# xmindflow/deformableLKA

Hardware: AMD Instinct MI355X
Metric: 3D D-LKA fwd+bwd volumes/sec (64x128x128, b2) (higher is better)
Workload: dtype f32; 1 GPU; 3D D-LKA Former Synapse 64x128x128 patch: fwd+bwd of its 21 D-LKA attention blocks (6x(32,32^3)+6x(64,16^3)+6x(128,8^3)+3x(256,4^3)) + grad all-reduce + SGD update; batch_per_gpu=2, global_batch=2, parallelism=dp1, block_params=15390693, hipgraph=True, weight_gradients_on_side_stream=True, allreduce_overlap=False, allreduce_split_block=0

## Files before the change

deformablelka_amd/_lib.py:

```python
from __future__ import annotations

import ctypes
import os
from ctypes import POINTER, c_char_p, c_int, c_int32, c_int64, c_size_t, c_void_p

import torch

_HERE = os.path.dirname(os.path.abspath(__file__))
LIB_PATH = os.path.join(_HERE, "_lib", "libdlka_hip.so")

DLKA_F32, DLKA_BF16, DLKA_F64 = 0, 1, 2
DLKA_TILES_MAX_T, DLKA_TILES_K_MAX = 64, 32
DLKA_TILES_IDENTITY, DLKA_TILES_SOFTMAX, DLKA_TILES_SIGMOID = 0, 1, 2
LKA3D_SYNAPSE, LKA3D_ACDC = 0, 1
DLKA_SEG_LOSS_K_MAX = 32
DLKA_SEG_LOSS_NNUNET, DLKA_SEG_LOSS_DICE2D = 0, 1
DLKA_LABEL_F32, DLKA_LABEL_I64 = 0, 1
DLKA_SD_K_MAX = 32
DLKA_SD_U8, DLKA_SD_I16, DLKA_SD_I32, DLKA_SD_I64 = 0, 1, 2, 3
DLKA_CC_K_MAX, DLKA_CC_IDS_MAX = 32, 64
DLKA_CC_SUMMARY = 1 + 2 * DLKA_CC_K_MAX
DLKA_RESAMPLE_SPLINE_PAD = 12
DLKA_SPLINE_REFLECT, DLKA_SPLINE_MIRROR = 0, 1
DLKA_AUG_I16 = 3
# ... 38 lines not shown
class SegLossDesc(ctypes.Structure):
    _fields_ = [("B", c_int32), ("K", c_int32), ("N", c_int64), ("dtype", c_int32), ("label_dtype", c_int32), ("mode", c_int32),
                ("batch_dice", c_int32), ("do_bg", c_int32), ("smooth", ctypes.c_float), ("weight_ce", ctypes.c_float),
                ("weight_dice", ctypes.c_float), ("class_weight", ctypes.c_float * DLKA_SEG_LOSS_K_MAX)]


class SurfaceDistDesc(ctypes.Structure):
    _fields_ = [("rank", c_int32), ("connectivity", c_int32), ("label_dtype", c_int32), ("K", c_int32), ("mask_mode", c_int32),
                ("ext", c_int64 * 3), ("spacing", ctypes.c_double * 3), ("class_id", c_int64 * DLKA_SD_K_MAX)]


class ConnCompDesc(ctypes.Structure):
    _fields_ = [("rank", c_int32), ("connectivity", c_int32), ("label_dtype", c_int32), ("K", c_int32), ("mask_mode", c_int32),
                ("n_ids", c_int32), ("has_min", c_int32), ("ext", c_int64 * 3), ("class_id", c_int64 * DLKA_CC_IDS_MAX),
                ("entry_of", c_int32 * DLKA_CC_IDS_MAX), ("min_count", c_int64 * DLKA_CC_K_MAX)]


class ResampleDesc(ctypes.Structure):
    _fields_ = [("C", c_int32), ("dtype", c_int32), ("taps", c_int32 * 3), ("in_", c_int64 * 3), ("out", c_int64 * 3)]


class AugmentDesc(ctypes.Structure):
    _fields_ = [("B", c_int32), ("C", c_int32), ("dtype", c_int32), ("order", c_int32), ("mode", c_int32), ("pad", c_int32),
                ("src", c_int64 * 3), ("out", c_int64 * 3), ("cval", ctypes.c_double)]


class PrepDesc(ctypes.Structure):
    _fields_ = [("rank", c_int32), ("C", c_int32), ("seg_channels", c_int32), ("nan_to_zero", c_int32), ("nonzero_label", c_int32),
                ("ext", c_int64 * 3), ("lo", c_int64 * 3), ("hi", c_int64 * 3)]


class Zoom2dDesc(ctypes.Structure):
    _fields_ = [("in_dtype", c_int32), ("out_dtype", c_int32), ("taps", c_int32), ("normalize", c_int32), ("N", c_int64),
                ("in_", c_int64 * 2), ("out", c_int64 * 2), ("mean", ctypes.c_float), ("std", ctypes.c_float)]


class OptimDesc(ctypes.Structure):
    _fields_ = [("n_tensors", c_int32), ("dtype", c_int32), ("nesterov", c_int32), ("has_momentum", c_int32), ("clip", c_int32),
                ("momentum", ctypes.c_float), ("weight_decay", ctypes.c_float), ("max_norm", ctypes.c_float), ("lr_index", c_int32)]


_G = POINTER(ConvGeom)
_SD = POINTER(SegLossDesc)
_SDD = POINTER(SurfaceDistDesc)
_CCD = POINTER(ConnCompDesc)
_RSD = POINTER(ResampleDesc)
_AGD = POINTER(AugmentDesc)
_PPD = POINTER(PrepDesc)
_ZMD = POINTER(Zoom2dDesc)
_OPD = POINTER(OptimDesc)
_PTRS, _I64S = POINTER(c_void_p), POINTER(c_int64)
SIGNATURES = {
    "dlka_abi_version": (c_int, []),
    "dlka_status_string": (c_char_p, [c_int]),
    "dlka_conv_out_size": (c_int, [c_int] * 5),
    "dlka_deform_conv3d_forward_workspace": (c_size_t, [_G, c_int]),
    "dlka_deform_conv3d_forward": (c_int, [c_void_p] * 6 + [c_size_t, _G, c_int, c_void_p]),
    "dlka_deform_conv3d_backward_workspace": (c_size_t, [_G, c_int]),
    "dlka_deform_conv3d_backward": (c_int, [c_void_p] * 9 + [c_size_t, _G, c_int, c_void_p]),
    "dlka_deform_conv3d_sample_index": (c_int, [c_void_p] * 3 + [_G, c_int, c_void_p]),
    "dlka_deform_conv3d_sample_index_path": (c_int, [c_void_p] * 3 + [_G, c_int, c_int, c_void_p]),
    "dlka_deform_conv2d_forward_workspace": (c_size_t, [_G, c_int]),
    "dlka_deform_conv2d_forward": (c_int, [c_void_p] * 6 + [c_size_t, _G, c_int, c_void_p]),
    "dlka_deform_conv2d_backward_workspace": (c_size_t, [_G, c_int]),
    "dlka_deform_conv2d_backward": (c_int, [c_void_p] * 9 + [c_size_t, _G, c_int, c_void_p]),
    "dlka_conv3d_forward_workspace": (c_size_t, [_G, c_int]),
    "dlka_conv3d_forward": (c_int, [c_void_p] * 5 + [c_size_t, _G, c_int, c_void_p]),
    "dlka_conv3d_backward_workspace": (c_size_t, [_G, c_int]),
    "dlka_conv3d_backward": (c_int, [c_void_p] * 7 + [c_size_t, _G, c_int, c_void_p]),
    "dlka_gelu_forward": (c_int, [c_void_p, c_void_p, c_int64, c_int, c_void_p]),
    "dlka_gelu_backward": (c_int, [c_void_p] * 3 + [c_int64, c_int, c_void_p]),
    "dlka_mul_forward": (c_int, [c_void_p] * 3 + [c_int64, c_int, c_void_p]),
    "dlka_mul_backward": (c_int, [c_void_p] * 5 + [c_int64, c_int, c_void_p]),
    "dlka_add_forward": (c_int, [c_void_p] * 3 + [c_int64, c_int, c_void_p]),
    "dlka_lka3d_saved_bytes": (c_size_t, [c_int] * 6),
    "dlka_lka3d_workspace_bytes": (c_size_t, [c_int] * 6),
    "dlka_lka3d_attention_forward": (c_int, [c_void_p, POINTER(Lka3dPtrs), c_void_p, c_void_p, c_size_t, c_void_p, c_size_t]
                                     + [c_int] * 6 + [c_void_p]),
    "dlka_lka3d_attention_backward": (c_int, [c_void_p, POINTER(Lka3dPtrs), c_void_p, c_void_p, c_size_t, c_void_p,
                                              POINTER(Lka3dPtrs), c_void_p, c_size_t] + [c_int] * 6 + [c_void_p]),
    "dlka_lka2d_saved_bytes": (c_size_t, [c_int] * 5),
    "dlka_lka2d_workspace_bytes": (c_size_t, [c_int] * 5),
    "dlka_lka2d_attention_forward": (c_int, [c_void_p, POINTER(Lka2dPtrs), c_void_p, c_void_p, c_size_t, c_void_p, c_size_t]
                                     + [c_int] * 5 + [c_void_p]),
    "dlka_lka2d_attention_backward": (c_int, [c_void_p, POINTER(Lka2dPtrs), c_void_p, c_void_p, c_size_t, c_void_p,
                                              POINTER(Lka2dPtrs), c_void_p, c_size_t] + [c_int] * 5 + [c_void_p]),
    "dlka_lka2d_force_general": (c_int, [c_int]),
    "dlka_lka2d_saved_offsets": (c_int, [c_int] * 5 + [POINTER(c_size_t), POINTER(c_int)]),
    "dlka_conv3d_cl_workspace": (c_size_t, [_G, c_int, c_int]),
    "dlka_conv3d_forward_cl": (c_int, [c_void_p] * 4 + [c_int, c_void_p, c_size_t, _G, c_int, c_void_p]),
    "dlka_conv3d_backward_cl": (c_int, [c_void_p] * 3 + [c_int] + [c_void_p] * 4 + [c_size_t, _G, c_int, c_void_p]),
    "dlka_deform_conv3d_cl_workspace": (c_size_t, [_G, c_int, c_int]),
    "dlka_deform_conv3d_forward_cl": (c_int, [c_void_p] * 6 + [c_size_t, _G, c_int, c_void_p]),
    "dlka_deform_conv3d_backward_cl": (c_int, [c_void_p] * 9 + [c_size_t, _G, c_int, c_void_p]),
    "dlka_ncdhw_to_ndhwc": (c_int, [c_void_p, c_void_p, c_int, c_int, c_int, c_int, c_void_p]),
    "dlka_ndhwc_to_ncdhw": (c_int, [c_void_p, c_void_p, c_int, c_int, c_int, c_int, c_void_p]),
    "dlka_lka3d_tokens_supported": (c_int, [c_int] * 6),
    "dlka_lka3d_tokens_saved_bytes": (c_size_t, [c_int] * 6),
    "dlka_lka3d_tokens_workspace_bytes": (c_size_t, [c_int] * 6),
    "dlka_lka3d_attention_tokens_forward": (c_int, [c_void_p, POINTER(Lka3dPtrs), c_void_p, c_void_p, c_size_t, c_void_p, c_size_t]
                                            + [c_int] * 6 + [c_void_p]),
    "dlka_lka3d_attention_tokens_forward_prepared": (c_int, [c_void_p, POINTER(Lka3dPtrs), c_void_p, c_void_p, c_size_t, c_void_p, c_size_t]
                                                     + [c_int] * 6 + [c_void_p]),
    "dlka_lka3d_tokens_prepare_plan_bytes": (c_size_t, [c_int]),
    "dlka_lka3d_tokens_prepare_plan": (c_int, [c_int, POINTER(Lka3dPtrs), POINTER(c_void_p), POINTER(c_size_t), POINTER(c_int), c_int, c_void_p, c_size_t]),
    "dlka_lka3d_tokens_prepare_run": (c_int, [c_void_p, c_void_p, c_int, c_void_p]),
    "dlka_lka3d_tokens_prepare_run_range": (c_int, [c_void_p, c_void_p, c_int, c_int, c_int, c_void_p]),
    "dlka_lka3d_tokens_partials_bytes_v": (c_size_t, [c_int] * 7),
    "dlka_wgrad_finalize_plan_bytes": (c_size_t, [c_int]),
    "dlka_wgrad_finalize_plan_init": (c_int, [c_void_p, c_size_t, c_int]),
    "dlka_lka3d_attention_tokens_backward_deferred_v": (c_int, [c_void_p, POINTER(Lka3dPtrs), c_void_p, c_void_p, c_size_t, c_void_p,
                                                               POINTER(Lka3dPtrs), c_void_p, c_size_t, c_void_p, c_size_t, c_void_p, c_int,
                                                               c_int, c_int, c_int, c_int, c_int, c_int, c_int, c_void_p]),
    "dlka_lka3d_attention_tokens_backward_phase_v": (c_int, [c_void_p, POINTER(Lka3dPtrs), c_void_p, c_void_p, c_size_t, c_void_p,
                                                            POINTER(Lka3dPtrs), c_void_p, c_size_t, c_void_p, c_size_t, c_void_p, c_int, c_int,
                                                            c_int, c_int, c_int, c_int, c_int, c_int, c_int, c_void_p]),
    "dlka_wgrad_finalize_plan_seal": (c_int, [c_void_p]),
    "dlka_wgrad_finalize_run_slot": (c_int, [c_void_p, c_int, c_void_p]),
    "dlka_wgrad_finalize_run": (c_int, [c_void_p, c_void_p, c_int, c_int, c_void_p]),
    "dlka_lka3d_attention_tokens_backward": (c_int, [c_void_p, POINTER(Lka3dPtrs), c_void_p, c_void_p, c_size_t, c_void_p,
                                                     POINTER(Lka3dPtrs), c_void_p, c_size_t] + [c_int] * 6 + [c_void_p]),
    "dlka_layernorm_tokens_forward": (c_int, [c_void_p, c_int] + [c_void_p] * 6 + [c_int] * 3 + [ctypes.c_float, c_int, c_void_p]),
    "dlka_layernorm_tokens_backward": (c_int, [c_void_p] * 9 + [c_int] * 4 + [c_void_p]),
    "dlka_scale_residual_forward": (c_int, [c_void_p] * 4 + [c_int64, c_int, c_int, c_void_p]),
    "dlka_scale_residual_backward": (c_int, [c_void_p] * 5 + [c_int64, c_int, c_int, c_void_p]),
    "dlka_batchnorm_cl_forward": (c_int, [c_void_p] * 5 + [c_int] + [c_void_p] * 2 + [c_int64, c_int, ctypes.c_float, ctypes.c_float, c_int, c_void_p]),
    "dlka_batchnorm_cl_backward": (c_int, [c_void_p] * 5 + [c_int] + [c_void_p] * 5 + [c_int64, c_int, ctypes.c_float, c_int, c_void_p]),
    "dlka_channel_scale": (c_int, [c_void_p] * 3 + [c_int, c_int64, c_int, c_int, c_void_p]),
    "dlka_batchnorm_planar_forward": (c_int, [c_void_p] * 6 + [c_int, c_int, c_int64, ctypes.c_float, c_void_p]),
    "dlka_batchnorm_planar_backward": (c_int, [c_void_p] * 8 + [c_int, c_int, c_int64, c_void_p]),
    "dlka_pointwise_planar_forward": (c_int, [c_void_p] * 4 + [c_int, c_int, c_int, c_int64, c_void_p]),
    "dlka_pointwise_planar_backward": (c_int, [c_void_p] * 6 + [c_int, c_int, c_int, c_int64, c_void_p]),
    "dlka_tblock3d_supported": (c_int, [c_int] * 6),
    "dlka_tblock3d_saved_bytes": (c_size_t, [c_int] * 6),
    "dlka_tblock3d_workspace_bytes": (c_size_t, [c_int] * 6),
    "dlka_tblock3d_forward": (c_int, [c_void_p, c_int, POINTER(TBlock3dPtrs), POINTER(Lka3dPtrs), c_void_p, c_int, c_void_p, c_void_p, c_void_p, c_size_t,
                                      c_void_p, c_size_t] + [c_int] * 5 + [ctypes.c_float, ctypes.c_float, c_int, c_void_p]),
    "dlka_tblock3d_backward": (c_int, [POINTER(TBlock3dPtrs), POINTER(Lka3dPtrs), c_void_p, c_int, c_void_p, c_void_p, c_void_p, c_size_t, c_void_p,
                                       POINTER(TBlock3dPtrs), POINTER(Lka3dPtrs), c_void_p, c_size_t] + [c_int] * 6 + [c_void_p]),
    "dlka_deform_conv2d_sample_index_path": (c_int, [c_void_p] * 3 + [_G, c_int, c_int, c_void_p]),
    "dlka_deform_dwconv2d_cl_workspace": (c_size_t, [_G, c_int, c_int]),
    "dlka_deform_dwconv2d_forward_cl": (c_int, [c_void_p] * 5 + [c_size_t, _G, c_int, c_void_p]),
    "dlka_deform_dwconv2d_backward_cl": (c_int, [c_void_p] * 8 + [c_size_t, _G, c_int, c_void_p]),
    "dlka_lka3d_force_wgrad_gather": (c_int, [c_int]),
    "dlka_fork_stats": (c_int, [c_int, POINTER(ctypes.c_int64), POINTER(ctypes.c_int64)]),
    "dlka_env_refresh": (None, []),
    "dlka_dwconv_lds_launch_count": (ctypes.c_long, []),
    "dlka_conv_brick_launch_count": (ctypes.c_long, []),
    "dlka_dwpair_launch_count": (ctypes.c_long, []),
    "dlka_pw_chain_launch_count": (ctypes.c_long, []),
    "dlka_dwconv_2p_launch_count": (ctypes.c_long, []),
    "dlka_conv_kw_launch_count": (ctypes.c_long, []),
    "dlka_conv_kw_applies": (c_int, [c_int] * 8),
    "dlka_lka3d_tokens_supported_v": (c_int, [c_int] * 7),
    "dlka_lka3d_tokens_saved_bytes_v": (c_size_t, [c_int] * 7),
    "dlka_lka3d_tokens_workspace_bytes_v": (c_size_t, [c_int] * 7),
    "dlka_lka3d_attention_tokens_forward_v": (c_int, [c_void_p, POINTER(Lka3dPtrs), c_void_p, c_void_p, c_size_t, c_void_p, c_size_t]
                                              + [c_int] * 7 + [c_void_p]),
    "dlka_lka3d_attention_tokens_backward_v": (c_int, [c_void_p, POINTER(Lka3dPtrs), c_void_p, c_void_p, c_size_t, c_void_p,
                                                       POINTER(Lka3dPtrs), c_void_p, c_size_t] + [c_int] * 7 + [c_void_p]),
    "dlka_lka3d_tokens_saved_offsets_v": (c_int, [c_int] * 7 + [POINTER(c_size_t)]),
    "dlka_tblock3d_saved_offsets_v": (c_int, [c_int] * 7 + [POINTER(c_size_t)]),
    "dlka_tblock3d_saved_activations_v": (c_int, [c_int] * 7 + [POINTER(c_size_t)]),
    "dlka_tblock3d_supported_v": (c_int, [c_int] * 7),
    "dlka_tblock3d_saved_bytes_v": (c_size_t, [c_int] * 7),
    "dlka_tblock3d_workspace_bytes_v": (c_size_t, [c_int] * 7),
    "dlka_tblock3d_forward_v": (c_int, [c_void_p, c_int, POINTER(TBlock3dPtrs), POINTER(Lka3dPtrs), c_void_p, c_int, c_void_p, c_void_p, c_void_p, c_size_t,
                                        c_void_p, c_size_t] + [c_int] * 5 + [ctypes.c_float, ctypes.c_float, c_int, c_int, c_void_p]),
    "dlka_tblock3d_backward_v": (c_int, [POINTER(TBlock3dPtrs), POINTER(Lka3dPtrs), c_void_p, c_int, c_void_p, c_void_p, c_void_p, c_size_t, c_void_p,
                                         POINTER(TBlock3dPtrs), POINTER(Lka3dPtrs), c_void_p, c_size_t] + [c_int] * 7 + [c_void_p]),
    "dlka_tblock3d_backward_phase_v": (c_int, [POINTER(TBlock3dPtrs), POINTER(Lka3dPtrs), c_void_p, c_int, c_void_p, c_void_p, c_void_p, c_size_t, c_void_p,
                                         POINTER(TBlock3dPtrs), POINTER(Lka3dPtrs), c_void_p, c_size_t] + [c_int] * 8 + [c_void_p]),
    "dlka_tiles_gather": (c_int, [c_void_p] + [c_int] * 4 + [POINTER(c_int), c_int, POINTER(c_int)] + [c_int] * 7 + [ctypes.c_float, c_void_p, c_void_p]),
    "dlka_tiles_blend": (c_int, [c_void_p, c_int, c_int, c_int, ctypes.c_float] + [c_void_p] * 3 + [c_int] * 3
                         + [POINTER(c_int), c_int, POINTER(c_int)] + [c_int] * 4 + [c_void_p]),
    "dlka_tiles_finalize": (c_int, [c_void_p] * 2 + [c_int] * 10 + [c_void_p] * 3),
    "dlka_tiles_launch_count": (ctypes.c_long, []),
    "dlka_seg_loss_workspace_bytes": (c_size_t, [_SD]),
    "dlka_seg_loss_forward": (c_int, [c_void_p, c_void_p, _SD, c_void_p, c_size_t] + [c_void_p] * 5),
    "dlka_seg_loss_backward": (c_int, [c_void_p, c_void_p, _SD] + [c_void_p] * 4),
    "dlka_seg_eval_counts": (c_int, [c_void_p, c_void_p, _SD, c_void_p, c_size_t, c_void_p, c_void_p]),
    "dlka_seg_loss_launch_count": (ctypes.c_long, []),
    "dlka_sd_stats_workspace_bytes": (c_size_t, [_SDD]),
    "dlka_sd_label_stats": (c_int, [c_void_p, c_void_p, _SDD, c_void_p, c_size_t, c_void_p, c_void_p]),
    "dlka_sd_distance_cells": (c_int64, [_SDD, POINTER(c_int64)]),
    "dlka_sd_distances": (c_int, [c_void_p, c_void_p, _SDD, POINTER(c_int64), c_void_p, c_size_t, c_void_p, c_int64, c_void_p]),
    "dlka_sd_launch_count": (ctypes.c_long, []),
    "dlka_cc_workspace_bytes": (c_size_t, [_CCD]),
    "dlka_cc_components": (c_int, [c_void_p, _CCD, c_void_p, c_size_t, c_void_p, c_void_p, c_void_p, c_void_p]),
    "dlka_cc_component_table": (c_int, [_CCD, c_void_p, c_size_t, c_int64, c_void_p, c_void_p, c_void_p]),
    "dlka_cc_launch_count": (ctypes.c_long, []),
    "dlka_resample_argmax": (c_int, [c_void_p, c_void_p, _RSD, c_void_p, c_void_p, c_void_p, c_void_p]),
    "dlka_resample_linear": (c_int, [c_void_p, c_void_p, _RSD, c_void_p, c_void_p, c_void_p]),
    "dlka_resample_labels": (c_int, [c_void_p, c_void_p, _RSD, c_void_p, c_void_p, c_int, c_void_p]),
    "dlka_resample_spline_eval": (c_int, [c_void_p, c_void_p, _RSD, c_void_p, c_void_p, c_void_p, c_void_p, c_int, c_void_p]),
    "dlka_resample_launch_count": (ctypes.c_long, []),
    "dlka_spline_pad": (c_int, [c_void_p, c_void_p, c_int, POINTER(c_int64), POINTER(c_int64), c_void_p]),
    "dlka_spline_prefilter": (c_int, [c_void_p, POINTER(c_int64), c_int, c_int, c_void_p]),
    "dlka_augment_spatial": (c_int, [c_void_p, c_void_p, c_void_p, _AGD, c_void_p, c_void_p, c_void_p]),
    "dlka_augment_spatial_labels": (c_int, [c_void_p, c_void_p, _AGD, c_void_p, c_void_p, c_void_p]),
    "dlka_augment_spatial2d": (c_int, [c_void_p, c_void_p, c_void_p, _AGD, c_void_p, c_void_p, c_void_p]),
    "dlka_augment_spatial2d_labels": (c_int, [c_void_p, c_void_p, _AGD, c_void_p, c_void_p, c_void_p]),
    "dlka_augment_gaussian": (c_int, [c_void_p, c_void_p, c_int, c_int64, POINTER(c_int64), c_int, c_void_p, c_void_p, c_void_p]),
    "dlka_augment_stats_workspace_bytes": (c_size_t, [c_int64, c_int64]),
    "dlka_augment_channel_stats": (c_int, [c_void_p, c_void_p, c_void_p, c_size_t, c_int, c_int64, c_int64, c_void_p]),
    "dlka_augment_pointwise": (c_int, [c_void_p, c_void_p, c_void_p, c_int, c_int64, c_int64, POINTER(c_int64)] + [c_void_p] * 5),
    "dlka_augment_launch_count": (ctypes.c_long, []),
    "dlka_prep_background": (c_int, [c_void_p, _PPD, c_void_p, c_void_p]),
    "dlka_prep_fill_workspace_bytes": (c_size_t, [_PPD]),
    "dlka_prep_fill_bbox": (c_int, [c_void_p, c_void_p, _PPD, c_void_p, c_size_t, c_void_p, c_void_p, c_void_p]),
    "dlka_prep_mask_bbox": (c_int, [c_void_p, _PPD, c_void_p, c_void_p]),
    "dlka_prep_crop": (c_int, [c_void_p, c_void_p, c_void_p, _PPD, c_void_p, c_void_p, c_void_p]),
    "dlka_prep_stats_workspace_bytes": (c_size_t, [_PPD]),
    "dlka_prep_channel_stats": (c_int, [c_void_p, c_void_p, _PPD, c_void_p, c_void_p, c_size_t, c_void_p]),
    "dlka_prep_normalize": (c_int, [c_void_p, c_void_p, _PPD, c_void_p, c_void_p, c_void_p]),
    "dlka_prep_launch_count": (ctypes.c_long, []),
    "dlka_zoom2d_spline": (c_int, [c_void_p, c_void_p, _ZMD, c_void_p, c_void_p, c_void_p]),
    "dlka_zoom2d_nearest": (c_int, [c_void_p, c_void_p, _ZMD, c_int, c_void_p, c_void_p]),
    "dlka_zoom2d_argmax": (c_int, [c_void_p, c_void_p, _ZMD, c_int, c_void_p, c_void_p]),
    "dlka_zoom2d_launch_count": (ctypes.c_long, []),
    "dlka_optim_workspace_bytes": (c_size_t, [_I64S, c_int64]),
    "dlka_optim_grad_norm": (c_int, [_PTRS, _I64S, c_int64, c_int, c_void_p, c_size_t, c_void_p, c_void_p]),
    "dlka_optim_scale": (c_int, [_PTRS, _I64S, c_int64, c_int, c_void_p, ctypes.c_float, c_void_p]),
    "dlka_optim_sgd_step": (c_int, [_PTRS, _PTRS, _PTRS, _I64S, _OPD, c_void_p, c_void_p, c_void_p]),
    "dlka_optim_launch_count": (ctypes.c_long, []),
    "dlka_trace_start": (c_int, [c_int, c_void_p]),
    "dlka_trace_mark": (c_int, [c_void_p]),
    "dlka_trace_stop": (c_int, []),
    "dlka_trace_count": (c_int, []),
    "dlka_trace_get": (c_int, [c_int, ctypes.c_char_p, c_size_t, POINTER(ctypes.c_float)]),
}


def bind(cdll: ctypes.CDLL) -> ctypes.CDLL:
    for name, (res, args) in SIGNATURES.items():
        fn = getattr(cdll, name)
        fn.restype = res
        fn.argtypes = args
    if cdll.dlka_abi_version() != 1:
        raise RuntimeError("libdlka ABI version mismatch")
    return cdll


_lib = None
_test_backend = False


def get_lib() -> ctypes.CDLL:
    global _lib
    if _lib is None:
        if not os.path.exists(LIB_PATH):
            raise RuntimeError(
                f"deformablelka_amd: {LIB_PATH} is missing. Build it with `python -c 'import __graft_entry__ as g; g.build()'` "
                "or `make -C deformablelka_amd/csrc` (hipcc, --offload-arch=gfx950). There is no CPU/PyTorch fallback.")
        _lib = bind(ctypes.CDLL(LIB_PATH))
    return _lib


def _set_backend_for_tests(cdll) -> None:
    global _lib, _test_backend
    _lib = bind(cdll) if cdll is not None else None
    _test_backend = cdll is not None


def check(rc: int, what: str) -> None:
    if rc != 0:
        msg = get_lib().dlka_status_string(rc).decode()
        raise RuntimeError(f"{what}: {msg} (dlka status {rc})")


def dtype_code(t: torch.Tensor, allow_f64: bool = False) -> int:
    if t.dtype == torch.float32:
        return DLKA_F32
    if t.dtype == torch.bfloat16:
        return DLKA_BF16
    if t.dtype == torch.float64 and allow_f64:
        return DLKA_F64
    raise RuntimeError(f"deformablelka_amd supports float32 and bfloat16 tensors (float64: the general deform_conv / conv3d operators only), got {t.dtype}")


def require_device(*tensors) -> None:
    for t in tensors:
        if t is None:
            continue
        if _test_backend:
            if t.device.type != "cpu":
                raise RuntimeError("test backend wants CPU tensors")
        elif not t.is_cuda:
            raise RuntimeError("deformablelka_amd: tensors must live on an AMD GPU (cuda/HIP device); "
                               "the operator is not implemented on the CPU")


def stream_ptr(t: torch.Tensor):
    if _test_backend:
        return None
    if t.device.index is not None and t.device.index != torch.cuda.current_device():
        raise RuntimeError(f"deformablelka_amd: tensor on {t.device} but the current device is cuda:{torch.cuda.current_device()} — "
                           f"call under torch.cuda.device({t.device.index})")
    return c_void_p(torch.cuda.current_stream(t.device).cuda_stream)


def ptr(t):
    return c_void_p(0) if t is None else c_void_p(t.data_ptr())


def scratch(nbytes: int, like: torch.Tensor) -> torch.Tensor:
# ... 2 lines not shown
```

deformablelka_amd/csrc/capi_lka3d_tokens.h:

```cpp
#pragma once
#include "cl_host.h"

namespace dlka {

inline SameConv block_conv(int B, int C, int Cout, int D, int H, int W, int k, int pad, int dil, int group, int act_bf16 = 0)
{
    SameConv s;
    s.act_bf16 = act_bf16;
    s.B = B; s.D = D; s.H = H; s.W = W; s.N = D * H * W; s.M = B * s.N; s.Cin = C; s.Cout = Cout; s.group = group;
    s.kd = s.kh = s.kw = k; s.pd = s.ph = s.pw = pad; s.dd = s.dh = s.dw = dil; s.K = k * k * k;
    return s;
}

struct DwPairCfg { int k0[3], p0[3], d0[3], k1[3], p1[3], d1[3]; };
inline bool dw_pair_cfg(int variant, int C, DwPairCfg &c)
{
    auto set = [](int *dst, int a, int b, int cc) { dst[0] = a; dst[1] = b; dst[2] = cc; };
    if (variant == DLKA_LKA3D_SYNAPSE) {
        set(c.k0, 5, 5, 5); set(c.p0, 2, 2, 2); set(c.d0, 1, 1, 1); set(c.k1, 7, 7, 7); set(c.p1, 9, 9, 9); set(c.d1, 3, 3, 3);
        return true;
    }
    if (variant != DLKA_LKA3D_ACDC) return false;
    if (C == 32 || C == 64) { set(c.k0, 5, 5, 5); set(c.p0, 2, 2, 2); set(c.d0, 1, 1, 1); set(c.k1, 5, 7, 7); set(c.p1, 6, 9, 9); set(c.d1, 3, 3, 3); }
    else if (C == 128) { set(c.k0, 5, 5, 5); set(c.p0, 2, 2, 2); set(c.d0, 1, 1, 1); set(c.k1, 3, 5, 5); set(c.p1, 1, 6, 6); set(c.d1, 1, 3, 3); }
    else if (C == 256) { set(c.k0, 3, 3, 3); set(c.p0, 1, 1, 1); set(c.d0, 1, 1, 1); set(c.k1, 3, 3, 3); set(c.p1, 1, 1, 1); set(c.d1, 1, 1, 1); }
    else return false;
    return true;
}
inline SameConv dw_conv(int B, int C, int D, int H, int W, const int *k, const int *p, const int *d, int act_bf16)
{
    SameConv s;
    s.act_bf16 = act_bf16;
    s.B = B; s.D = D; s.H = H; s.W = W; s.N = D * H * W; s.M = B * s.N; s.Cin = C; s.Cout = C; s.group = C;
    s.kd = k[0]; s.kh = k[1]; s.kw = k[2]; s.pd = p[0]; s.ph = p[1]; s.pw = p[2]; s.dd = d[0]; s.dh = d[1]; s.dw = d[2]; s.K = k[0] * k[1] * k[2];
    return s;
}

struct TokPartials { float *p2, *c1, *p1, *off, *dcn, *stage5, *stage7; };

struct TokGeoms {
    SameConv pw, dw5, dw7, offc, dcn;
    SameConv dw5_f, dw7_f, offc_f, pw_f;
    size_t E, Off, GOff;
    size_t SB;
    size_t part_bytes;
    TokGeoms(int B, int C, int D, int H, int W, int dtype = DLKA_F32, int variant = DLKA_LKA3D_SYNAPSE)
    {
        const int bf = dtype == DLKA_BF16 ? 1 : 0;
        SB = bf ? 2 : 4;
        DwPairCfg dc;
        if (!dw_pair_cfg(variant, C, dc)) dw_pair_cfg(DLKA_LKA3D_SYNAPSE, C, dc);
        pw = block_conv(B, C, C, D, H, W, 1, 0, 1, 1, bf);
        dw5 = dw_conv(B, C, D, H, W, dc.k0, dc.p0, dc.d0, bf);
        dw7 = dw_conv(B, C, D, H, W, dc.k1, dc.p1, dc.d1, bf);
        offc = block_conv(B, C, 81, D, H, W, 3, 1, 1, 1, bf);
        dcn = block_conv(B, C, C, D, H, W, 3, 1, 1, 1, bf);
        dw5_f = dw_conv(B, C, D, H, W, dc.k0, dc.p0, dc.d0, 0);
        dw7_f = dw_conv(B, C, D, H, W, dc.k1, dc.p1, dc.d1, 0);
        offc_f = block_conv(B, C, 81, D, H, W, 3, 1, 1, 1, 0);
        pw_f = block_conv(B, C, C, D, H, W, 1, 0, 1, 1, 0);
        E = (size_t)B * C * D * H * W;
        Off = (size_t)B * 81 * D * H * W;
        GOff = (size_t)B * 96 * D * H * W;
        part_bytes = carved_bytes([&](Carver &m) { carve_partials(m); });
    }
    size_t wp_floats() const
    {
        size_t m = dense_wp_floats(offc);
        if (dense_wp_floats(dcn) > m) m = dense_wp_floats(dcn);
        if ((size_t)dw7.K * dw7.Cin > m) m = (size_t)dw7.K * dw7.Cin;
        return m;
    }
    size_t scratch_floats() const { return deform_scratch_floats(dcn); }
    size_t blk_floats() const
    {
        const size_t a5 = cl_dwconv_blk_floats(dw5.B, dw5.Cin, dw5.D, dw5.H, dw5.W, dw5.dw), a7 = cl_dwconv_blk_floats(dw7.B, dw7.Cin, dw7.D, dw7.H, dw7.W, dw7.dw);
        return ((a5 > a7 ? a5 : a7) + 63) & ~(size_t)63;
    }
    size_t samp_capacity_floats() const
    {
        const size_t n = (size_t)dcn.K * dcn.M * dcn.Cin;
        return (n * SB < ((size_t)1 << 31)) ? n * SB / 4 : 0;
    }
    size_t pw_floats() const { return (size_t)pw.Cin * pw.Cin; }
    size_t offc_floats() const { return dense_wp_floats(offc); }
    size_t dcn_floats() const { return dense_wp_floats(dcn); }
    size_t dw5_floats() const { return (size_t)dw5.K * dw5.Cin; }
    size_t dw7_floats() const { return (size_t)dw7.K * dw7.Cin; }
    size_t prep_floats() const { return 6 * pw_floats() + 2 * offc_floats() + 3 * dcn_floats() + 2 * dw5_floats() + 2 * dw7_floats() + 17 * 64; }
    size_t part_pw() const { return (cl_wgrad_part_floats_mode(pw.M, 1, pw.Cin, pw.Cin, 0) + 63) & ~(size_t)63; }
    size_t part_off() const { return (cl_wgrad_part_floats_mode(pw.M, 27, 81, pw.Cin, 0) + 63) & ~(size_t)63; }
    size_t part_dcn() const { return (cl_wgrad_part_floats_mode(pw.M, 27, pw.Cin, pw.Cin, 1) + 63) & ~(size_t)63; }
    size_t stage_dw() const { return (size_t)(dw5.K + 1 + dw7.K + 1) * pw.Cin; }
    TokPartials carve_partials(Carver &pc) const
    {
        TokPartials P;
        P.p2 = (float *)pc.take(part_pw() * 4); P.c1 = (float *)pc.take(part_pw() * 4); P.p1 = (float *)pc.take(part_pw() * 4);
        P.off = (float *)pc.take(part_off() * 4);
        P.dcn = (float *)pc.take(part_dcn() * 4);
        P.stage5 = (float *)pc.take(stage_dw() * 4);
        P.stage7 = P.stage5 ? P.stage5 + (size_t)(dw5.K + 1) * pw.Cin : nullptr;
        return P;
    }
};

struct TokPrep {
    float *pw_f[3], *pw_b[3];
    float *off_f, *off_b, *dcn_f, *dcn_b, *dw5_f, *dw5_b, *dw7_f, *dw7_b;
    float *dcn_b16;
};

struct TokSaved {
    float *h, *a, *t1, *t, *off, *f, *g1;
    float *prep;
    float *m;
};
inline TokSaved carve_tok_saved(Carver &sv, const TokGeoms &G)
{
    const size_t act = G.E * G.SB;
    TokSaved S;
    S.h = (float *)sv.take(act); S.a = (float *)sv.take(act); S.t1 = (float *)sv.take(act); S.t = (float *)sv.take(act);
    S.off = (float *)sv.take(G.Off * 4);
    S.f = (float *)sv.take(act); S.g1 = (float *)sv.take(act);
    S.prep = (float *)sv.take(G.prep_floats() * 4);
    S.m = (float *)sv.take(act);
    return S;
}
inline size_t tok_saved_bytes(const TokGeoms &G) { return carved_bytes([&](Carver &m) { carve_tok_saved(m, G); }); }

inline void carve_tok_blk(Carver &cv, const TokGeoms &G, float *&blkA, float *&blkB)
{
    const bool want_blk = cl_dwconv_lds_mode() != 0;
    blkA = (float *)cv.take_opt(G.blk_floats() * 4, want_blk);
    blkB = (float *)cv.take_opt(G.blk_floats() * 4, want_blk && cv.got(blkA));
    if (!blkB) blkA = nullptr;
}

struct TokBwdWs {
    float *wp_reserve;
    float *part;
    float *gg1, *ga1, *gf, *gta, *gt, *gt1, *ga2, *gh;
    float *goff, *scratch;
    float *samp;
    float *blkA, *blkB;
    float *padt;
};
inline TokBwdWs carve_tok_bwd_ws(Carver &cv, const TokGeoms &G)
{
    TokBwdWs W;
    W.wp_reserve = (float *)cv.take(G.wp_floats() * 4);
    W.part = (float *)cv.take(G.part_bytes);
    float **grad[8] = {&W.gg1, &W.ga1, &W.gf, &W.gta, &W.gt, &W.gt1, &W.ga2, &W.gh};
    for (float **g : grad) *g = (float *)cv.take(G.E * 4);
    W.goff = (float *)cv.take(G.GOff * 4);
    W.scratch = (float *)cv.take(G.scratch_floats() * 4);
    W.samp = G.samp_capacity_floats() ? (float *)cv.take(G.samp_capacity_floats() * 4) : nullptr;
    carve_tok_blk(cv, G, W.blkA, W.blkB);
    const size_t pad = dense_wgrad_pad_bytes(G.offc);
    W.padt = (float *)cv.take_opt(pad, pad != 0);
    return W;
}

struct TokFwdWs {
    float *wp_reserve, *part_reserve, *gg1_reserve;
    float *a32, *t1_32, *t_32;
    float *blkA, *blkB;
};
inline TokFwdWs carve_tok_fwd_ws(Carver &cv, const TokGeoms &G)
{
    TokFwdWs W;
    W.wp_reserve = (float *)cv.take(G.wp_floats() * 4);
    W.part_reserve = (float *)cv.take(G.part_bytes);
    W.gg1_reserve = (float *)cv.take(G.E * 4);
    W.a32 = (float *)cv.take(G.E * 4); W.t1_32 = (float *)cv.take(G.E * 4); W.t_32 = (float *)cv.take(G.E * 4);
    carve_tok_blk(cv, G, W.blkA, W.blkB);
    return W;
}

struct TokWsTail {
    void *reserve;
    float *slab;
};
inline TokWsTail carve_tok_ws_tail(Carver &cv, const TokGeoms &G)
{
    cv.skip_to(carved_bytes([&](Carver &m) { carve_tok_bwd_ws(m, G); }));
    TokWsTail T;
    T.reserve = cv.take(4096);
    T.slab = deform_fwd_slab_floats(G.dcn) ? (float *)cv.take(deform_fwd_slab_floats(G.dcn) * 4) : nullptr;
    return T;
}
inline size_t tok_workspace_bytes(const TokGeoms &G)
{
    return carved_bytes([&](Carver &m) { carve_tok_fwd_ws(m, G); carve_tok_ws_tail(m, G); });
}

bool tokens_supported(int B, int C, int D, int H, int W, int variant = DLKA_LKA3D_SYNAPSE);
int carve_prep(const TokGeoms &G, float *base, TokPrep &t, const dlka_lka3d_params *p, hipStream_t st, bool fill, const ZeroBatch *zb = nullptr,
               PrepBatch *collect = nullptr, bool append = false);
constexpr int FIN_JOBS_PER_BLOCK = 8;
int tokens_forward_impl(const void *x_, const dlka_lka3d_params *p, void *y_, void *saved, size_t saved_bytes, void *workspace,
                        size_t workspace_bytes, int B, int C, int D, int H, int W, int dtype, void *stream, bool prepared,
                        int variant = DLKA_LKA3D_SYNAPSE, const float *x_f32 = nullptr);
int tokens_backward_impl(const void *x_, const dlka_lka3d_params *p, const void *gy_, const void *saved, size_t saved_bytes, void *gx_,
                         const dlka_lka3d_grads *gr, void *workspace, size_t workspace_bytes, int B, int C, int D, int H, int W, int dtype, int variant,
                         void *stream, void *partials, size_t partials_bytes, FinalizeJob *jobs_out, int *njobs_out, int phase = 0,
                         const FinalizeBatch *extra = nullptr);
}
```

deformablelka_amd/csrc/capi_lka3d_tokens.hip:

```cpp
#include "capi_lka3d_tokens.h"
#include "cl_fork.h"

using namespace dlka;

namespace dlka {

int carve_prep(const TokGeoms &G, float *base, TokPrep &t, const dlka_lka3d_params *p, hipStream_t st, bool fill, const ZeroBatch *zb,
               PrepBatch *collect, bool append)
{
    float *q = base;
    auto take = [&](size_t n) { float *r = q; q += (n + 63) & ~(size_t)63; return r; };
    for (int k = 0; k < 3; ++k) { t.pw_f[k] = take(G.pw_floats()); t.pw_b[k] = take(G.pw_floats()); }
    t.off_f = take(G.offc_floats()); t.off_b = take(G.offc_floats());
    t.dcn_f = take(G.dcn_floats()); t.dcn_b = take(G.dcn_floats());
    t.dw5_f = take(G.dw5_floats()); t.dw5_b = take(G.dw5_floats());
    t.dw7_f = take(G.dw7_floats()); t.dw7_b = take(G.dw7_floats());
    t.dcn_b16 = take(G.dcn_floats());
    if (!fill) return DLKA_OK;
    PrepBatch pb;
    if (collect && append) pb = *collect;
    else memset(&pb, 0, sizeof(pb));
    if (pb.njobs + 15 + (zb ? zb->n : 0) > PREP_MAX_JOBS) return DLKA_ERR_WORKSPACE;
    const int C = G.pw.Cin;
    const void *pw_w[3] = {p->proj_1_w, p->conv1_w, p->proj_2_w};
    for (int k = 0; k < 3; ++k) {
        add_job(pb, pw_w[k], t.pw_f[k], C, C, 1, C, C, 0);
        add_job(pb, pw_w[k], t.pw_b[k], C, C, 1, C, C, 1);
    }
    add_job(pb, p->offset_w, t.off_f, 81, C, 27, C, 96, split_mode_flag(use_split(G.offc_f, true)));
    add_job(pb, p->offset_w, t.off_b, 81, C, 27, 96, C, use_split(G.offc, false) ? 9 : 1);
    add_job(pb, p->deform_w, t.dcn_f, C, C, 27, C, C, (G.dcn.act_bf16 && deform_b16()) ? 8 : 0);
    add_job(pb, p->deform_w, t.dcn_b, C, C, 27, C, C, 2);
    if (deform_b16()) add_job(pb, p->deform_w, t.dcn_b16, C, C, 27, C, C, 2 | 8);
    add_job(pb, p->conv0_w, t.dw5_f, C, C, G.dw5.K, 0, 0, 3);
    add_job(pb, p->conv0_w, t.dw5_b, C, C, G.dw5.K, 0, 0, 4);
    add_job(pb, p->conv_spatial_w, t.dw7_f, C, C, G.dw7.K, 0, 0, 3);
    add_job(pb, p->conv_spatial_w, t.dw7_b, C, C, G.dw7.K, 0, 0, 4);
    if (zb && pb.njobs + zb->n > PREP_MAX_JOBS) return DLKA_ERR_WORKSPACE;
    if (zb)
        for (int r = 0; r < zb->n; ++r) {
            PrepJob &j = pb.j[pb.njobs++];
            memset(&j, 0, sizeof(j));
            j.dst = zb->p[r]; j.n = zb->cnt[r]; j.mode = 5;
            pb.total += j.n;
        }
    if (collect) { *collect = pb; return DLKA_OK; }
    return launch_cl_prep_batch(pb, st);
}

bool tokens_supported(int B, int C, int D, int H, int W, int variant)
{
    if (B <= 0 || D <= 0 || H <= 0 || W <= 0) return false;
    if (!(C == 32 || C == 64 || C == 128 || C == 256)) return false;
    if ((long)B * D * H * W > (1l << 28)) return false;
    DwPairCfg dc;
    if (!dw_pair_cfg(variant, C, dc)) return false;
    return dw_supported(dw_conv(B, C, D, H, W, dc.k0, dc.p0, dc.d0, 0)) && dw_supported(dw_conv(B, C, D, H, W, dc.k1, dc.p1, dc.d1, 0));
}

}

extern "C" {

int dlka_lka3d_tokens_supported_v(int B, int C, int D, int H, int W, int dtype, int variant)
{
    return ((dtype == DLKA_F32 || dtype == DLKA_BF16) && tokens_supported(B, C, D, H, W, variant)) ? 1 : 0;
}
int dlka_lka3d_tokens_supported(int B, int C, int D, int H, int W, int dtype) { return dlka_lka3d_tokens_supported_v(B, C, D, H, W, dtype, DLKA_LKA3D_SYNAPSE); }

size_t dlka_lka3d_tokens_saved_bytes_v(int B, int C, int D, int H, int W, int dtype, int variant)
{
    if (!dlka_lka3d_tokens_supported_v(B, C, D, H, W, dtype, variant)) return 0;
    return tok_saved_bytes(TokGeoms(B, C, D, H, W, dtype, variant));
}
size_t dlka_lka3d_tokens_saved_bytes(int B, int C, int D, int H, int W, int dtype) { return dlka_lka3d_tokens_saved_bytes_v(B, C, D, H, W, dtype, DLKA_LKA3D_SYNAPSE); }

size_t dlka_lka3d_tokens_workspace_bytes(int B, int C, int D, int H, int W, int dtype) { return dlka_lka3d_tokens_workspace_bytes_v(B, C, D, H, W, dtype, DLKA_LKA3D_SYNAPSE); }
size_t dlka_lka3d_tokens_workspace_bytes_v(int B, int C, int D, int H, int W, int dtype, int variant)
{
    if (!dlka_lka3d_tokens_supported_v(B, C, D, H, W, dtype, variant)) return 0;
    return tok_workspace_bytes(TokGeoms(B, C, D, H, W, dtype, variant));
}

}

int dlka::tokens_forward_impl(const void *x_, const dlka_lka3d_params *p, void *y_, void *saved, size_t saved_bytes, void *workspace,
                              size_t workspace_bytes, int B, int C, int D, int H, int W, int dtype, void *stream, bool prepared,
                              int variant, const float *x_f32)
{
    if (!x_ || !p || !y_ || !saved || !workspace) return DLKA_ERR_NULL;
    const void *const *pp = (const void *const *)p;
    for (size_t k = 0; k < sizeof(*p) / sizeof(void *); ++k) if (!pp[k]) return DLKA_ERR_NULL;
    if (!dlka_lka3d_tokens_supported_v(B, C, D, H, W, dtype, variant)) return DLKA_ERR_UNSUPPORTED;
    hipStream_t st = (hipStream_t)stream;
    TokGeoms G(B, C, D, H, W, dtype, variant);
    Carver sv(saved, saved_bytes), cv(workspace, workspace_bytes);
    const TokSaved S = carve_tok_saved(sv, G);
    const TokFwdWs Wf = carve_tok_fwd_ws(cv, G);
    if (!sv.ok() || !cv.ok()) return DLKA_ERR_WORKSPACE;
    TokWsTail Wt = {nullptr, nullptr};
    if (deform_fwd_slab_floats(G.dcn)) Wt = carve_tok_ws_tail(cv, G);
    if (!cv.ok()) return DLKA_ERR_WORKSPACE;
    float *h = S.h, *a = S.a, *t1 = S.t1, *t = S.t, *off = S.off, *f = S.f, *g1 = S.g1, *prep = S.prep, *m = S.m;
    float *a32 = Wf.a32, *t1_32 = Wf.t1_32, *t_32 = Wf.t_32, *blkA = Wf.blkA, *blkB = Wf.blkB, *slab = Wt.slab;
    const bool bf = dtype == DLKA_BF16;
    const float *x = (const float *)x_;
    float *y = (float *)y_;
    const float *N0 = nullptr;
    ZeroBatch zb;
    memset(&zb, 0, sizeof(zb));
    if (dense_forward_splits(G.offc_f, 0) > 1) zb.add(off, G.Off);
    if (dense_forward_splits(G.pw, 3) > 1) zb.add(y, G.E);
    TokPrep PW;
    const ZeroBatch *ride = nullptr;
    if (prepared) {
        DLKA_TRY(carve_prep(G, prep, PW, p, st, false));
        if (zb.n) ride = &zb;
    } else {
        DLKA_TRY(carve_prep(G, prep, PW, p, st, true, &zb));
    }
    if (bf && x_f32) {
        DLKA_TRY(dense_forward(G.pw_f, x_f32, N0, (const float *)p->proj_1_b, t_32, 0, PW.pw_f[0], 1, nullptr, a32, st, false, ride));
        ride = nullptr;
        DLKA_TRY(dense_forward(G.pw, x, N0, (const float *)p->proj_1_b, h, 0, PW.pw_f[0], 1, nullptr, a, st));
    } else
        DLKA_TRY(dense_forward(G.pw, x, N0, (const float *)p->proj_1_b, h, 0, PW.pw_f[0], 1, nullptr, a, st, false, ride, bf ? a32 : nullptr));
    const float *a_in = bf ? a32 : a;
    float *t1_out = bf ? t1_32 : t1, *t_out = bf ? t_32 : t;
    bool chained = false;
    DwBlk bk5, bk7;
    bk5.blk = blkA; bk5.blk_floats = G.blk_floats(); bk5.chain = &G.dw7_f; bk5.chain_blk = blkB; bk5.chained = &chained;
    const int pair = dw_pair(G.dw5_f, G.dw7_f, a_in, PW.dw5_f, (const float *)p->conv0_b, t1_out, bf ? t1 : nullptr, PW.dw7_f, (const float *)p->conv_spatial_b, t_out,
                             bf ? t : nullptr, nullptr, nullptr, st);
    if (pair != DLKA_ERR_UNSUPPORTED) DLKA_TRY(pair);
    else {
        DLKA_TRY(dw_forward(G.dw5_f, a_in, N0, (const float *)p->conv0_b, t1_out, PW.dw5_f, 0, st, nullptr, nullptr, bf ? t1 : nullptr, &bk5));
        bk7.blk = blkB; bk7.blk_floats = G.blk_floats(); bk7.in_blocked = chained;
        DLKA_TRY(dw_forward(G.dw7_f, t1_out, N0, (const float *)p->conv_spatial_b, t_out, PW.dw7_f, 0, st, nullptr, nullptr, bf ? t : nullptr, &bk7));
    }
    DLKA_TRY(dense_forward(G.offc_f, t_out, N0, (const float *)p->offset_b, off, 1, PW.off_f, 0, nullptr, nullptr, st, true));
    DLKA_TRY(deform_forward(G.dcn, t, off, N0, (const float *)p->deform_b, f, PW.dcn_f, st, slab));
    const int prc = pointwise_pair(G.pw, 0, f, PW.pw_f[1], (const float *)p->conv1_b, PW.pw_f[2], (const float *)p->proj_2_b, a, x, g1, m, y, st);
    if (prc != DLKA_ERR_UNSUPPORTED) return prc;
    DLKA_TRY(dense_forward(G.pw, f, N0, (const float *)p->conv1_b, g1, 0, PW.pw_f[1], 2, a, m, st));
    DLKA_TRY(dense_forward(G.pw, m, N0, (const float *)p->proj_2_b, y, 0, PW.pw_f[2], 3, x, nullptr, st, true));
    return DLKA_OK;
}

extern "C" {

int dlka_lka3d_attention_tokens_forward(const void *x, const dlka_lka3d_params *p, void *y, void *saved, size_t saved_bytes, void *workspace,
                                        size_t workspace_bytes, int B, int C, int D, int H, int W, int dtype, void *stream)
{
    return tokens_forward_impl(x, p, y, saved, saved_bytes, workspace, workspace_bytes, B, C, D, H, W, dtype, stream, false);
}

int dlka_lka3d_attention_tokens_forward_v(const void *x, const dlka_lka3d_params *p, void *y, void *saved, size_t saved_bytes, void *workspace,
                                          size_t workspace_bytes, int B, int C, int D, int H, int W, int dtype, int variant, void *stream)
{
    return tokens_forward_impl(x, p, y, saved, saved_bytes, workspace, workspace_bytes, B, C, D, H, W, dtype, stream, false, variant);
}

int dlka_lka3d_attention_tokens_forward_prepared(const void *x, const dlka_lka3d_params *p, void *y, void *saved, size_t saved_bytes, void *workspace,
                                                 size_t workspace_bytes, int B, int C, int D, int H, int W, int dtype, void *stream)
{
    return tokens_forward_impl(x, p, y, saved, saved_bytes, workspace, workspace_bytes, B, C, D, H, W, dtype, stream, true);
}

namespace {
constexpr int PLAN_JOBS_PER_BLOCK = 16;
struct PlanHeader { int njobs, nblocks, pad0, pad1; };
size_t plan_first_off() { return sizeof(PlanHeader); }
size_t plan_blkjob_off(int nb) { return sizeof(PlanHeader) + ((size_t)nb * PLAN_JOBS_PER_BLOCK + 1) * sizeof(int); }
size_t plan_jobs_off(int nb) { return align256(plan_blkjob_off(nb) + (size_t)(nb + 1) * sizeof(int)); }
}

size_t dlka_lka3d_tokens_prepare_plan_bytes(int nblocks)
{
    if (nblocks <= 0) return 0;
    return plan_jobs_off(nblocks) + (size_t)nblocks * PLAN_JOBS_PER_BLOCK * sizeof(PrepJob);
}

int dlka_lka3d_tokens_prepare_plan(int nblocks, const dlka_lka3d_params *params, void *const *saved, const size_t *saved_bytes, const int *dims5,
                                   int dtype, void *plan_host, size_t plan_bytes)
{
    if (!params || !saved || !saved_bytes || !dims5 || !plan_host) return DLKA_ERR_NULL;
    if (nblocks <= 0 || plan_bytes < dlka_lka3d_tokens_prepare_plan_bytes(nblocks)) return DLKA_ERR_WORKSPACE;
    unsigned char *base = (unsigned char *)plan_host;
    PlanHeader *hd = (PlanHeader *)base;
    int *first = (int *)(base + plan_first_off());
    PrepJob *jobs = (PrepJob *)(base + plan_jobs_off(nblocks));
    int *blkjob = (int *)(base + plan_blkjob_off(nblocks));
    int nj = 0, nb = 0;
    for (int k = 0; k < nblocks; ++k) {
        blkjob[k] = nj;
        const int B = dims5[5 * k], C = dims5[5 * k + 1], D = dims5[5 * k + 2], H = dims5[5 * k + 3], W = dims5[5 * k + 4];
        if (!dlka_lka3d_tokens_supported(B, C, D, H, W, dtype)) return DLKA_ERR_UNSUPPORTED;
        TokGeoms G(B, C, D, H, W, dtype);
        Carver sv(saved[k], saved_bytes[k]);
        const TokSaved S = carve_tok_saved(sv, G);
        if (!S.prep) return DLKA_ERR_WORKSPACE;
        TokPrep PW;
        PrepBatch pb;
        DLKA_TRY(carve_prep(G, S.prep, PW, &params[k], nullptr, true, nullptr, &pb));
        if (pb.njobs > PLAN_JOBS_PER_BLOCK) return DLKA_ERR_UNSUPPORTED;
        for (int j = 0; j < pb.njobs; ++j) {
            first[nj] = nb;
            jobs[nj] = pb.j[j];
            nb += cl_prep_table_blocks(pb.j[j]);
            ++nj;
        }
    }
    blkjob[nblocks] = nj;
    first[nj] = nb;
    hd->njobs = nj; hd->nblocks = nb; hd->pad0 = hd->pad1 = 0;
    return DLKA_OK;
}

int dlka_lka3d_tokens_prepare_run_range(const void *plan_device, const void *plan_host, int nblocks, int block_lo, int block_hi, void *stream)
{
    if (!plan_device || !plan_host) return DLKA_ERR_NULL;
    if (block_lo < 0 || block_hi > nblocks || block_lo >= block_hi) return DLKA_ERR_SHAPE;
    const unsigned char *hst = (const unsigned char *)plan_host;
    const int *first = (const int *)(hst + plan_first_off()), *blkjob = (const int *)(hst + plan_blkjob_off(nblocks));
    const int jlo = blkjob[block_lo], jhi = blkjob[block_hi];
    const unsigned char *dev = (const unsigned char *)plan_device;
    return launch_cl_prep_table((const PrepJob *)(dev + plan_jobs_off(nblocks)), (const int *)(dev + plan_first_off()), jlo, jhi, first[jhi] - first[jlo],
                                (hipStream_t)stream);
}

int dlka_lka3d_tokens_prepare_run(const void *plan_device, const void *plan_host, int nblocks, void *stream)
{
    return dlka_lka3d_tokens_prepare_run_range(plan_device, plan_host, nblocks, 0, nblocks, stream);
}

int dlka_lka3d_attention_tokens_backward(const void *x_, const dlka_lka3d_params *p, const void *gy_, const void *saved, size_t saved_bytes,
                                         void *gx_, const dlka_lka3d_grads *gr, void *workspace, size_t workspace_bytes, int B, int C,
                                         int D, int H, int W, int dtype, void *stream)
{
    return dlka_lka3d_attention_tokens_backward_v(x_, p, gy_, saved, saved_bytes, gx_, gr, workspace, workspace_bytes, B, C, D, H, W, dtype, DLKA_LKA3D_SYNAPSE, stream);
}

namespace {
struct FinPlanHeader { int nblocks, sealed, pad0, pad1; long total_blocks; long pad2; };
size_t fin_first_off() { return sizeof(FinPlanHeader); }
size_t fin_jobs_off(int nb) { return align256(sizeof(FinPlanHeader) + (size_t)(nb + 1) * sizeof(int)); }
}

size_t dlka_lka3d_tokens_partials_bytes_v(int B, int C, int D, int H, int W, int dtype, int variant)
{
    if (!dlka_lka3d_tokens_supported_v(B, C, D, H, W, dtype, variant)) return 0;
    return TokGeoms(B, C, D, H, W, dtype, variant).part_bytes;
}

size_t dlka_wgrad_finalize_plan_bytes(int nblocks)
{
    if (nblocks <= 0) return 0;
    return fin_jobs_off(nblocks) + (size_t)nblocks * FIN_JOBS_PER_BLOCK * sizeof(FinalizeJob);
}

int dlka_wgrad_finalize_plan_init(void *plan_host, size_t plan_bytes, int nblocks)
{
    if (!plan_host) return DLKA_ERR_NULL;
    if (nblocks <= 0 || plan_bytes < dlka_wgrad_finalize_plan_bytes(nblocks)) return DLKA_ERR_WORKSPACE;
    memset(plan_host, 0, dlka_wgrad_finalize_plan_bytes(nblocks));
    ((FinPlanHeader *)plan_host)->nblocks = nblocks;
    return DLKA_OK;
}

int dlka_lka3d_attention_tokens_backward_deferred_v(const void *x, const dlka_lka3d_params *p, const void *grad_y, const void *saved, size_t saved_bytes,
                                                    void *grad_x, const dlka_lka3d_grads *grads, void *workspace, size_t workspace_bytes, void *partials,
                                                    size_t partials_bytes, void *plan_host, int plan_slot, int B, int C, int D, int H, int W, int dtype,
                                                    int variant, void *stream)
{
    if (!partials) return DLKA_ERR_NULL;
    FinalizeJob jobs[FIN_JOBS_PER_BLOCK];
    int nj = 0;
    DLKA_TRY(tokens_backward_impl(x, p, grad_y, saved, saved_bytes, grad_x, grads, workspace, workspace_bytes, B, C, D, H, W, dtype, variant, stream, partials,
                                  partials_bytes, jobs, &nj));
    if (plan_host) {
        FinPlanHeader *hd = (FinPlanHeader *)plan_host;
        if (plan_slot < 0 || plan_slot >= hd->nblocks || hd->sealed) return DLKA_ERR_SHAPE;
        int *first = (int *)((unsigned char *)plan_host + fin_first_off());
        FinalizeJob *all = (FinalizeJob *)((unsigned char *)plan_host + fin_jobs_off(hd->nblocks));
        for (int j = 0; j < nj; ++j) all[plan_slot * FIN_JOBS_PER_BLOCK + j] = jobs[j];
        first[plan_slot] = nj;
    }
    return DLKA_OK;
}

int dlka_lka3d_attention_tokens_backward_phase_v(const void *x, const dlka_lka3d_params *p, const void *grad_y, const void *saved, size_t saved_bytes,
                                                 void *grad_x, const dlka_lka3d_grads *grads, void *workspace, size_t workspace_bytes, void *partials,
                                                 size_t partials_bytes, void *plan_host, int plan_slot, int phase, int B, int C, int D, int H, int W, int dtype,
                                                 int variant, void *stream)
{
    if (!partials) return DLKA_ERR_NULL;
    if (phase != 1 && phase != 2) return DLKA_ERR_SHAPE;
    FinalizeJob jobs[FIN_JOBS_PER_BLOCK];
    int nj = 0;
    DLKA_TRY(tokens_backward_impl(x, p, grad_y, saved, saved_bytes, grad_x, grads, workspace, workspace_bytes, B, C, D, H, W, dtype, variant, stream, partials,
                                  partials_bytes, jobs, &nj, phase));
    if (plan_host && phase == 2) {
        FinPlanHeader *hd = (FinPlanHeader *)plan_host;
        if (plan_slot < 0 || plan_slot >= hd->nblocks || hd->sealed) return DLKA_ERR_SHAPE;
        int *first = (int *)((unsigned char *)plan_host + fin_first_off());
        FinalizeJob *all = (FinalizeJob *)((unsigned char *)plan_host + fin_jobs_off(hd->nblocks));
        for (int j = 0; j < nj; ++j) all[plan_slot * FIN_JOBS_PER_BLOCK + j] = jobs[j];
        first[plan_slot] = nj;
    }
    return DLKA_OK;
}

int dlka_wgrad_finalize_run_slot(const void *plan_host, int plan_slot, void *stream)
{
    if (!plan_host) return DLKA_ERR_NULL;
    const FinPlanHeader *hd = (const FinPlanHeader *)plan_host;
    if (hd->sealed || plan_slot < 0 || plan_slot >= hd->nblocks) return DLKA_ERR_SHAPE;
    const int *first = (const int *)((const unsigned char *)plan_host + fin_first_off());
    const FinalizeJob *all = (const FinalizeJob *)((const unsigned char *)plan_host + fin_jobs_off(hd->nblocks));
    const int cnt = first[plan_slot];
    if (cnt <= 0 || cnt > FIN_JOBS_PER_BLOCK) return DLKA_ERR_SHAPE;
    FinalizeBatch fb;
    memset(&fb, 0, sizeof(fb));
    for (int j = 0; j < cnt; ++j) fb.j[j] = all[plan_slot * FIN_JOBS_PER_BLOCK + j];
    fb.njobs = cnt;
    return launch_cl_wgrad_finalize(fb, (hipStream_t)stream);
}

int dlka_wgrad_finalize_plan_seal(void *plan_host)
{
    if (!plan_host) return DLKA_ERR_NULL;
    FinPlanHeader *hd = (FinPlanHeader *)plan_host;
    if (hd->sealed) return DLKA_OK;
    const int nb = hd->nblocks;
    int *first = (int *)((unsigned char *)plan_host + fin_first_off());
    FinalizeJob *all = (FinalizeJob *)((unsigned char *)plan_host + fin_jobs_off(nb));
    int nj = 0;
    long blk = 0;
    for (int k = 0; k < nb; ++k) {
        const int cnt = first[k];
        if (cnt <= 0 || cnt > FIN_JOBS_PER_BLOCK) return DLKA_ERR_SHAPE;
        first[k] = nj;
        for (int j = 0; j < cnt; ++j) {
            FinalizeJob jb = all[k * FIN_JOBS_PER_BLOCK + j];
            jb.block0 = blk;
            blk += cl_wgrad_finalize_plan_job(jb);
            all[nj++] = jb;
        }
    }
    first[nb] = nj;
    hd->total_blocks = blk;
    hd->sealed = 1;
    return DLKA_OK;
}

int dlka_wgrad_finalize_run(const void *plan_device, const void *plan_host, int block_lo, int block_hi, void *stream)
{
    if (!plan_device || !plan_host) return DLKA_ERR_NULL;
    const FinPlanHeader *hd = (const FinPlanHeader *)plan_host;
    if (!hd->sealed || block_lo < 0 || block_hi > hd->nblocks || block_lo >= block_hi) return DLKA_ERR_SHAPE;
    const int *first = (const int *)((const unsigned char *)plan_host + fin_first_off());
    const FinalizeJob *all_h = (const FinalizeJob *)((const unsigned char *)plan_host + fin_jobs_off(hd->nblocks));
    const int jlo = first[block_lo], jhi = first[block_hi];
    const long b_lo = all_h[jlo].block0;
    const long b_hi = block_hi == hd->nblocks ? hd->total_blocks : all_h[jhi].block0;
    const FinalizeJob *all_d = (const FinalizeJob *)((const unsigned char *)plan_device + fin_jobs_off(hd->nblocks));
    return launch_cl_wgrad_finalize_table(all_d, jlo, jhi, b_hi - b_lo, (hipStream_t)stream);
}

int dlka_lka3d_attention_tokens_backward_v(const void *x_, const dlka_lka3d_params *p, const void *gy_, const void *saved, size_t saved_bytes,
                                           void *gx_, const dlka_lka3d_grads *gr, void *workspace, size_t workspace_bytes, int B, int C,
                                           int D, int H, int W, int dtype, int variant, void *stream)
{
    return tokens_backward_impl(x_, p, gy_, saved, saved_bytes, gx_, gr, workspace, workspace_bytes, B, C, D, H, W, dtype, variant, stream, nullptr, 0, nullptr,
                                nullptr);
}

}

int dlka::tokens_backward_impl(const void *x_, const dlka_lka3d_params *p, const void *gy_, const void *saved, size_t saved_bytes, void *gx_,
                         const dlka_lka3d_grads *gr, void *workspace, size_t workspace_bytes, int B, int C, int D, int H, int W, int dtype, int variant,
                         void *stream, void *partials, size_t partials_bytes, FinalizeJob *jobs_out, int *njobs_out, int phase, const FinalizeBatch *extra)
{
    if (!x_ || !p || !gy_ || !saved || !gx_ || !gr || !workspace) return DLKA_ERR_NULL;
    if (phase < 0 || phase > 2) return DLKA_ERR_SHAPE;
    const void *const *pp = (const void *const *)p;
    for (size_t k = 0; k < sizeof(*p) / sizeof(void *); ++k) if (!pp[k]) return DLKA_ERR_NULL;
    void *const *gp = (void *const *)gr;
    for (size_t k = 0; k < sizeof(*gr) / sizeof(void *); ++k) if (!gp[k]) return DLKA_ERR_NULL;
    if (!dlka_lka3d_tokens_supported_v(B, C, D, H, W, dtype, variant)) return DLKA_ERR_UNSUPPORTED;
    hipStream_t st = (hipStream_t)stream;
    TokGeoms G(B, C, D, H, W, dtype, variant);
    const bool bf = dtype == DLKA_BF16;
    Carver sv(saved, saved_bytes), cv(workspace, workspace_bytes);
    const TokSaved S = carve_tok_saved(sv, G);
    const TokBwdWs Wb = carve_tok_bwd_ws(cv, G);
    if (!sv.ok() || !cv.ok()) return DLKA_ERR_WORKSPACE;
    Carver pc(partials ? partials : Wb.part, partials ? partials_bytes : G.part_bytes);
    const TokPartials P = G.carve_partials(pc);
    if (!pc.ok()) return DLKA_ERR_WORKSPACE;
    const float *h = S.h, *a = S.a, *t1 = S.t1, *t = S.t, *off = S.off, *f = S.f, *g1 = S.g1, *m = S.m;
    float *prep = S.prep;
    float *gg1 = Wb.gg1, *ga1 = Wb.ga1, *gf = Wb.gf, *gta = Wb.gta, *gt = Wb.gt, *gt1 = Wb.gt1, *ga2 = Wb.ga2, *gh = Wb.gh;
    float *goff = Wb.goff, *scratch = Wb.scratch, *blkA = Wb.blkA, *blkB = Wb.blkB, *padt = Wb.padt;
    float *samp = wgrad_gather() ? nullptr : Wb.samp;
    const float *x = (const float *)x_, *gy = (const float *)gy_;
    float *gx = (float *)gx_;
    const float *N0 = nullptr;
    TokPrep PW;
    DLKA_TRY(carve_prep(G, prep, PW, p, st, false));
    float *part_p2 = P.p2, *part_c1 = P.c1, *part_p1 = P.p1, *part_off = P.off, *part_dcn = P.dcn, *stage5 = P.stage5, *stage7 = P.stage7;
    FinalizeBatch fb;
    memset(&fb, 0, sizeof(fb));

    const bool want_gx_fork = phase != 2 && gx_fork_wanted((long)G.dcn.M, phase);
    ForkLease lease(st, want_gx_fork);
    ZeroBatch zb;
    memset(&zb, 0, sizeof(zb));
    zb.add(stage5, G.stage_dw());
    zb.add(gta, G.E);
    int goff_cpad = 0;
    {
        DeformBwdArgs da;
        fill_deform_bwd(da, G.dcn);
        const bool fp32_goff = bf || getenv("DLKA_GOFF_PACKED") == nullptr;
        const bool sliced = cl_deform_goff_ccsplit(da) > 1;
        if (sliced) zb.add(goff, G.Off);
        else if (!fp32_goff && use_split(G.offc, false) == 2 && (G.offc.N & 15) == 0) goff_cpad = 96;
    }
    if (dense_backward_data_splits(G.pw, 0) > 1) zb.add(gf, G.E);
    if (dense_backward_data_splits(G.offc, 3) > 1) zb.add(bf ? ga2 : gt, G.E);
    if (dense_backward_data_splits(G.pw, 3) > 1) zb.add(gx, G.E);
    float *samp_max = (samp && !bf) ? samp + (size_t)G.dcn.K * G.dcn.M * G.dcn.Cin / 2 : nullptr;
    zb.add(samp_max, 1);
    if (zb.overflow) return DLKA_ERR_WORKSPACE;

#define DLKA_P1(call) do { if (phase != 2) DLKA_TRY(call); } while (0)
#define DLKA_P2(call) do { if (phase != 1) DLKA_TRY(call); } while (0)
    if (phase != 2) {
        const int prc = dense_backward_data_splits(G.pw, 0) > 1 ? DLKA_ERR_UNSUPPORTED
                                                                : pointwise_pair(G.pw, 1, gy, PW.pw_b[2], nullptr, PW.pw_b[1], nullptr, a, g1, gg1, ga1, gf, st, &zb);
        if (prc != DLKA_ERR_UNSUPPORTED) DLKA_TRY(prc);
        else {
            DLKA_TRY(dense_backward_data(G.pw, gy, 0, N0, gg1, PW.pw_b[2], 4, a, st, g1, ga1, false, false, false, nullptr, &zb));
            DLKA_TRY(dense_backward_data(G.pw, gg1, 0, N0, gf, PW.pw_b[1], 0, nullptr, st, nullptr, nullptr, true));
        }
    }
    if (!samp)
        DLKA_P2(deform_backward(G.dcn, t, off, N0, gf, nullptr, nullptr, (float *)gr->deform_w, (float *)gr->deform_b, PW.dcn_b, part_dcn, scratch, st,
                                &fb.j[fb.njobs++]));
    bool gx_forked = false;
    if (want_gx_fork && lease.ok()) {
        DLKA_TRY(lease.fork(1));
        DLKA_TRY(deform_backward(G.dcn, t, off, N0, gf, gta, nullptr, nullptr, nullptr, PW.dcn_b, nullptr, scratch, lease.stream(1), nullptr, true, false, 0, nullptr, PW.dcn_b16));
        gx_forked = true;
    }
    DLKA_P1(deform_backward(G.dcn, t, off, N0, gf, nullptr, goff, nullptr, nullptr, PW.dcn_b, nullptr, scratch, st, nullptr, false, true, goff_cpad, samp, PW.dcn_b16, samp_max != nullptr));
    if (samp)
        DLKA_P2(deform_backward(G.dcn, t, off, N0, gf, nullptr, nullptr, (float *)gr->deform_w, (float *)gr->deform_b, PW.dcn_b, part_dcn, scratch, st,
                                &fb.j[fb.njobs++], false, false, 0, samp));
    DLKA_P2(dense_backward_weight(G.offc, t, goff, 1, (float *)gr->offset_w, (float *)gr->offset_b, part_off, st, &fb.j[fb.njobs++], goff_cpad, padt));
    if (gx_forked) DLKA_TRY(lease.join(1));
    else
        DLKA_P1(deform_backward(G.dcn, t, off, N0, gf, gta, nullptr, nullptr, nullptr, PW.dcn_b, nullptr, scratch, st, nullptr, true, false, 0, nullptr, PW.dcn_b16));
    DLKA_P1(dense_backward_data(G.offc, goff, 1, N0, gt, PW.off_b, 3, gta, st, nullptr, nullptr, true, goff_cpad != 0, true, ga2));
    DLKA_P2(dw_backward_weight(G.dw7, t1, gt, (float *)gr->conv_spatial_w, (float *)gr->conv_spatial_b, stage7, st, &fb.j[fb.njobs++]));
    bool chained = false;
    DwBlk bk7, bk5;
    bk7.blk = blkA; bk7.blk_floats = G.blk_floats(); bk7.chain = &G.dw5; bk7.chain_blk = blkB; bk7.chained = &chained;
    int pair = DLKA_ERR_UNSUPPORTED;
    if (phase != 2) pair = dw_pair(G.dw7, G.dw5, gt, PW.dw7_b, nullptr, gt1, nullptr, PW.dw5_b, nullptr, gh, nullptr, h, ga1, st);
    if (pair != DLKA_ERR_UNSUPPORTED) DLKA_TRY(pair);
    else DLKA_P1(dw_forward(G.dw7, gt, N0, nullptr, gt1, PW.dw7_b, 1, st, nullptr, nullptr, nullptr, &bk7));
    DLKA_P2(dw_backward_weight(G.dw5, a, gt1, (float *)gr->conv0_w, (float *)gr->conv0_b, stage5, st, &fb.j[fb.njobs++]));
    bk5.blk = blkB; bk5.blk_floats = G.blk_floats(); bk5.in_blocked = chained;
    if (pair == DLKA_ERR_UNSUPPORTED) DLKA_P1(dw_forward(G.dw5, gt1, N0, nullptr, gh, PW.dw5_b, 1, st, h, ga1, nullptr, &bk5));
    if (phase != 1) {
        WgradArgs jobs[3];
        fill_pw_wgrad(jobs[0], G.pw, m, gy, part_p2);
        fill_pw_wgrad(jobs[1], G.pw, f, gg1, part_c1);
        fill_pw_wgrad(jobs[2], G.pw, x, gh, part_p1);
        float *const gws[3] = {(float *)gr->proj_2_w, (float *)gr->conv1_w, (float *)gr->proj_1_w};
        float *const gbs[3] = {(float *)gr->proj_2_b, (float *)gr->conv1_b, (float *)gr->proj_1_b};
        DLKA_TRY(launch_cl_wgrad_pw3(jobs, gws, gbs, st, &fb.j[fb.njobs]));
        fb.njobs += 3;
    }
    if (partials) {
        if (fb.njobs > FIN_JOBS_PER_BLOCK || !jobs_out || !njobs_out) return DLKA_ERR_UNSUPPORTED;
        for (int k = 0; k < fb.njobs; ++k) jobs_out[k] = fb.j[k];
        *njobs_out = fb.njobs;
    } else {
        if (phase != 0) return DLKA_ERR_UNSUPPORTED;
        if (extra) {
            if (fb.njobs + extra->njobs > (int)(sizeof(fb.j) / sizeof(fb.j[0]))) return DLKA_ERR_UNSUPPORTED;
            for (int k = 0; k < extra->njobs; ++k) fb.j[fb.njobs++] = extra->j[k];
        }
        DLKA_TRY(launch_cl_wgrad_finalize(fb, st));
    }
    DLKA_P1(dense_backward_data(G.pw, gh, 0, N0, gx, PW.pw_b[0], 3, gy, st, nullptr, nullptr, true));
#undef DLKA_P1
#undef DLKA_P2
    return DLKA_OK;
}

extern "C" {

int dlka_lka3d_tokens_saved_offsets_v(int B, int C, int D, int H, int W, int dtype, int variant, size_t *byte_offset)
{
    if (!byte_offset) return DLKA_ERR_NULL;
    if (!dlka_lka3d_tokens_supported_v(B, C, D, H, W, dtype, variant)) return DLKA_ERR_UNSUPPORTED;
    Carver sv = Carver::probing();
    *byte_offset = sv.offset_of(carve_tok_saved(sv, TokGeoms(B, C, D, H, W, dtype, variant)).off);
    return DLKA_OK;
}

}
```

deformablelka_amd/csrc/cl_args.h:

```cpp
#pragma once
#include "dlka_common.h"

namespace dlka {

struct ZeroBatch {
    int n;
    float *p[8];
    long cnt[8];
    unsigned block0[9];
    bool overflow;
    void add(float *ptr, size_t floats) { if (!ptr || !floats) return; if (n >= 8) { overflow = true; return; } p[n] = ptr; cnt[n] = (long)floats; ++n; }
};

__device__ __forceinline__ void zero_batch_block(const ZeroBatch &b, unsigned zb, int tid, int nthreads)
{
    if (zb >= b.block0[b.n]) return;
    int r = 0;
    while (r + 1 < b.n && zb >= b.block0[r + 1]) ++r;
    float *p = b.p[r];
    const long n = b.cnt[r], base = (long)(zb - b.block0[r]) * 4096;
    for (int k = tid; k < 1024; k += nthreads) {
        const long i = base + (long)k * 4;
        if (i + 3 < n) *reinterpret_cast<f32x4 *>(p + i) = f32x4{0.f, 0.f, 0.f, 0.f};
        else for (long j = i; j < n && j < base + 4096; ++j) p[j] = 0.f;
    }
}

struct IgemmArgs {
    const float *in;
    const float *off;
    const float *wp;
    const float *bias;
    const float *aux;
    const float *aux2;
    float *out;
    float *out2;
    float *out2_f32;
    int B, D, H, W, N, M;
    int Cin, CinReal, CinP, Cout, NP;
    int kd, kh, kw, pd, ph, pw, dd, dh, dw, K;
    int units_per_split;
    int split_bf16;
    int xcd_nx;
    int out_zeroed;
    int a_packed;
    int act_bf16;
    int aux_f32;
    ZeroBatch zero;
    int zero_xblocks;
    int epi;
};

struct PwPairArgs {
    const float *in, *wp1, *bias1, *wp2, *bias2, *a, *b;
    float *out1, *out1b, *out2;
    int M, C, bwd, act_bf16;
    ZeroBatch zero;
    int zero_blocks;
};

struct WgradArgs {
    const float *g;
    const float *in;
    const float *off;
    const float *samp;
    int samp_f16;
    int samp_b16mfma;
    float *part;
    float *bpart;
    int B, D, H, W, N, M;
    int Cin, Cout, CoutP;
    int kd, kh, kw, pd, ph, pw, dd, dh, dw, K;
    int rows_per_chunk;
    int act_bf16;
    int CT;
    int w16;
    int no_win3;
    int xcd_ny, xcd_nz, xcd_total;
    int g_cpad;
    const float *pad;
    int DP, HP, WP;
};

struct DwArgs {
    const float *in;
    const float *wp;
    const float *bias;
    float *out;
    float *out_lo;
    int xcd_nx;
    const float *gelu_x;
    const float *gelu_add;
    int B, D, H, W, C;
    int act_bf16;
    int kd, kh, pd, ph, pw, dd, dh;
    float *blk;
    size_t blk_floats;
    int in_blocked;
    float *out_blk;
    int out_blk_dil;
};

struct DwPairArgs {
    const float *in;
    const float *wpA, *wpB;
    const float *biasA, *biasB;
    float *outA, *outB;
    float *outA_lo, *outB_lo;
    const float *gelu_x, *gelu_add;
    int B, D, H, W, C;
    int kA, dA, pA, KA;
    int kB, dB, pB, KB;
    int act_bf16;
};

struct DwArgs2d {
    const float *in;
    const float *off;
    const float *wp;
    const float *g;
    float *out;
    float *out_lo;
    float *gx;
    float *goff;
    float *part;
    int B, H, W, C, kh, kw, ph, pw, dh, dw;
    int act_bf16;
};

struct DwWgradArgs {
    const float *g;
    const float *in;
    float *gwp;
    float *gb;
    int B, D, H, W, C;
    int kd, kh, pd, ph, pw, dd, dh;
    int rows_per_block;
    int act_bf16;
    int xcd_nx;
};

struct PrepJob {
    const float *src;
    float *dst;
    int Cout, Cin, K, KP, NP;
    int mode;
    long n;
};
constexpr int PREP_MAX_JOBS = 32;
struct PrepBatch {
    PrepJob j[PREP_MAX_JOBS];
    int njobs;
    long total;
    int first[PREP_MAX_JOBS + 1];
};

struct FinalizeJob {
    const float *part;
    const float *bpart;
    float *gw, *gb;
    int chunks, K, CoutP, Cout, Cin;
    int kind;
    int tr;
    long n;
    long block0;
};
struct FinalizeBatch {
    FinalizeJob j[12];
    int njobs;
    long nblocks;
};

struct DeformBwdArgs {
    const float *in;
    const float *off;
    const float *g;
    const float *wp;
    const float *wp16;
    float *gx;
    float *goff;
    float *samp;
    int B, D, H, W, N, M;
    int C, Cout, CoutP;
    int kd, kh, kw, pd, ph, pw, dd, dh, dw, K;
    int cc_per_block;
    int xcd_nx;
    int gx_zeroed;
    int goff_zeroed;
    int act_bf16;
    int samp_f16;
    int samp_max_zeroed;
    int goff_cpad;
};

}
```

deformablelka_amd/csrc/cl_conv_kw.hip:

```cpp
#include <stdlib.h>

#include <atomic>

#include "cl_arow.h"
#include "dlka_kernels.h"

namespace dlka {

std::atomic<long> g_conv_kw_launches{0};

template <int AMODE, int OMODE, int SPLIT, int KW, int NT, typename T>
__global__ __launch_bounds__(64 * KW) void cl_conv_kw_kernel(IgemmArgs p)
{
    constexpr bool A16 = AMODE == 0 && sizeof(T) == 2;
    constexpr int UF = SPLIT == 3 ? 48 : 32;
    constexpr int NB = 2 * SPLIT * NT;
    constexpr int RS = 65;
    constexpr bool LF = AMODE == 0 && sizeof(T) == 4;
    constexpr int AROW = 36;
    constexpr int WSM = (LF && 32 * AROW > 16 * RS) ? 32 * AROW : 16 * RS;
    __shared__ __attribute__((aligned(16))) float Red[KW][WSM];
    const int tid = threadIdx.x, lane = tid & 63, wave = tid >> 6;
    const int i = lane & 31, h = lane >> 5;
    const int mbase = blockIdx.x * 32;
    const int m = mbase + i;
    const bool row_ok = m < p.M;
    const int b = row_ok ? m / p.N : 0;
    const int v = row_ok ? m - b * p.N : 0;
    const int w0 = v % p.W, h0 = (v / p.W) % p.H, d0 = v / (p.W * p.H);
    const int n0 = blockIdx.z * (32 * NT);

    f32x16 acc[NT];
#pragma unroll
    for (int t = 0; t < NT; ++t)
#pragma unroll
        for (int r = 0; r < 16; ++r) acc[t][r] = 0.f;

    const int nchunk = p.CinP / 32;
    const int units = p.K * nchunk;
    const int ups = (units + KW - 1) / KW;
    const int unit_lo = wave * ups;
    const int unit_hi = min(units, unit_lo + ups);
    const BufRsrc rin = make_rsrc(p.in, AMODE == 2 ? (size_t)p.B * p.CinReal * p.N * 4 : (size_t)p.M * p.Cin * sizeof(T));
    const BufRsrc rw = make_rsrc(p.wp, (size_t)units * UF * p.NP * 4);
    const unsigned unit_bytes = (unsigned)(UF * p.NP) * 4u, seg_bytes = (unsigned)p.NP * 16u;
    const unsigned blane = (unsigned)(h * p.NP + n0 + i) * 16u;

    ARow<AMODE, T> arow;
    float abuf[2][16];
    f32x4 bbuf[2][NB];
    const int rg = lane >> 3, pc = lane & 7;
    unsigned lf_ro[4] = {DLKA_OOB, DLKA_OOB, DLKA_OOB, DLKA_OOB};
    int lf_tap = -1;
    auto issue = [&](int unit, float *ad, f32x4 *bd) {
        int ck;
        const int tap = divmod_fast(unit, nchunk, ck);
        if (LF) {
            if (tap != lf_tap) {
                lf_tap = tap;
                int ti, tj, tk;
                tap_decode(tap, p.kw, p.kh, ti, tj, tk);
                const int zd = d0 + ti * p.dd - p.pd, zh = h0 + tj * p.dh - p.ph, zw = w0 + tk * p.dw - p.pw;
                const bool ok = row_ok & ((unsigned)zd < (unsigned)p.D) & ((unsigned)zh < (unsigned)p.H) & ((unsigned)zw < (unsigned)p.W);
                const unsigned mine = !ok ? DLKA_OOB : (unsigned)((b * p.N + (zd * p.H + zh) * p.W + zw) * p.Cin) * 4u;
#pragma unroll
                for (int e = 0; e < 4; ++e) lf_ro[e] = (unsigned)__shfl((int)mine, 8 * e + rg);
            }
            const unsigned cb = (unsigned)(ck * 32 + 4 * pc) * 4u;
#pragma unroll
            for (int e = 0; e < 4; ++e) {
                const f32x4 t = buf_load_f32x4(rin, lf_ro[e] == DLKA_OOB ? DLKA_OOB : lf_ro[e] + cb);
                ad[4 * e] = t[0]; ad[4 * e + 1] = t[1]; ad[4 * e + 2] = t[2]; ad[4 * e + 3] = t[3];
            }
        } else
        arow.fetch(p, rin, tap, ck, h, row_ok, b, v, d0, h0, w0, ad);
        const unsigned ub = (unsigned)unit * unit_bytes + blane;
#pragma unroll
        for (int part = 0; part < SPLIT; ++part)
#pragma unroll
            for (int mf = 0; mf < 2; ++mf)
#pragma unroll
                for (int t = 0; t < NT; ++t) bd[(part * 2 + mf) * NT + t] = buf_load_f32x4(rw, ub + (unsigned)((part * 2 + mf) * 2) * seg_bytes + (unsigned)t * 512u);
    };
    auto compute = [&](const float *a_raw, const f32x4 *b_cur) {
        float a_lf[16];
        if (LF) {
            float *At = Red[wave];
            wave_sync();
#pragma unroll
            for (int e = 0; e < 4; ++e) *reinterpret_cast<f32x4 *>(At + (8 * e + rg) * AROW + 4 * pc) = f32x4{a_raw[4 * e], a_raw[4 * e + 1], a_raw[4 * e + 2], a_raw[4 * e + 3]};
            wave_sync();
#pragma unroll
            for (int e = 0; e < 4; ++e) {
                const f32x4 t = *reinterpret_cast<const f32x4 *>(At + i * AROW + 16 * h + 4 * e);
                a_lf[4 * e] = t[0]; a_lf[4 * e + 1] = t[1]; a_lf[4 * e + 2] = t[2]; a_lf[4 * e + 3] = t[3];
            }
        }
        const float *a_cur = LF ? a_lf : a_raw;
#pragma unroll
        for (int mf = 0; mf < 2; ++mf) {
            if (SPLIT == 3) {
                bf16x8 ahi, amid, alo;
                split3_bf16x8(a_cur + 8 * mf, ahi, amid, alo);
#pragma unroll
                for (int t = 0; t < NT; ++t) {
                    const bf16x8 bhi = __builtin_bit_cast(bf16x8, b_cur[(0 * 2 + mf) * NT + t]), bmid = __builtin_bit_cast(bf16x8, b_cur[(1 * 2 + mf) * NT + t]),
                                 blo = __builtin_bit_cast(bf16x8, b_cur[(2 * 2 + mf) * NT + t]);
                    acc[t] = mfma_32x32x16_bf16(alo, bhi, acc[t]);
                    acc[t] = mfma_32x32x16_bf16(ahi, blo, acc[t]);
                    acc[t] = mfma_32x32x16_bf16(amid, bmid, acc[t]);
                    acc[t] = mfma_32x32x16_bf16(amid, bhi, acc[t]);
                    acc[t] = mfma_32x32x16_bf16(ahi, bmid, acc[t]);
                    acc[t] = mfma_32x32x16_bf16(ahi, bhi, acc[t]);
                }
            } else {
                bf16x8 ahi, alo;
                if (A16) ahi = alo = bf16x8_from_words(a_cur + 4 * mf);
                else if (AMODE == 2 && p.a_packed) unpack_split2x8(a_cur + 8 * mf, ahi, alo);
                else split_bf16x8(a_cur + 8 * mf, ahi, alo);
#pragma unroll
                for (int t = 0; t < NT; ++t) {
                    const bf16x8 bhi = __builtin_bit_cast(bf16x8, b_cur[(0 * 2 + mf) * NT + t]), blo = __builtin_bit_cast(bf16x8, b_cur[(1 * 2 + mf) * NT + t]);
                    if (!A16) acc[t] = mfma_32x32x16_bf16(alo, bhi, acc[t]);
                    acc[t] = mfma_32x32x16_bf16(ahi, blo, acc[t]);
                    acc[t] = mfma_32x32x16_bf16(ahi, bhi, acc[t]);
                }
            }
        }
    };
    if (unit_lo < unit_hi) issue(unit_lo, abuf[0], bbuf[0]);
    for (int unit = unit_lo; unit < unit_hi; unit += 2) {
        if (unit + 1 < unit_hi) issue(unit + 1, abuf[1], bbuf[1]);
        compute(abuf[0], bbuf[0]);
        if (unit + 1 < unit_hi) {
            if (unit + 2 < unit_hi) issue(unit + 2, abuf[0], bbuf[0]);
            compute(abuf[1], bbuf[1]);
        }
    }

    float *mine = Red[wave];
    wave_sync();
#pragma unroll
    for (int t = 0; t < NT; ++t) {
        if (t) __syncthreads();
#pragma unroll
        for (int r = 0; r < 16; ++r) mine[r * RS + lane] = acc[t][r];
        __syncthreads();
        for (int e = tid; e < 32 * 32; e += 64 * KW) {
            const int row = OMODE == 1 ? (e & 31) : (e >> 5), col = OMODE == 1 ? (e >> 5) : (e & 31);
            const int hh = (row >> 2) & 1, rr = (row & 3) + 4 * (row >> 3);
            float val = 0.f;
#pragma unroll
            for (int w = 0; w < KW; ++w) val += Red[w][rr * RS + col + 32 * hh];
            const int mr = mbase + row, n = n0 + 32 * t + col;
            if (mr >= p.M || n >= p.Cout) continue;
            if (p.bias) val += p.bias[n];
            if (OMODE == 1) {
                const int bb = mr / p.N, vv = mr - bb * p.N;
                p.out[((long)bb * p.Cout + n) * p.N + vv] = val;
            } else {
                const long o = (long)mr * p.Cout + n;
                if (p.epi == 3) val += (sizeof(T) == 2 && p.aux_f32) ? p.aux[o] : act_load1(reinterpret_cast<const T *>(p.aux), o);
                act_store1(reinterpret_cast<T *>(p.out), o, val);
            }
        }
    }
}

bool cl_conv_kw_applies(int amode, int omode, int split_bf16, int K, int epi, int NP, bool act_bf16, bool volume)
{
    static const bool off = [] { const char *e = getenv("DLKA_CONV_KW"); return e && e[0] == '0'; }();
    if (off || !volume || K <= 1 || (epi != 0 && epi != 3) || NP % 32) return false;
    if (epi == 3 && omode == 1) return false;
    if (act_bf16) return split_bf16 == 2 && ((amode == 0 && omode == 1) || (amode == 2 && omode == 0));
    if (split_bf16 == 3) return amode == 0 && (omode == 0 || omode == 1);
    if (split_bf16 == 2) return (amode == 0 && (omode == 0 || omode == 1)) || (amode == 2 && omode == 0);
    return false;
}

int launch_cl_conv_kw(int amode, int omode, const IgemmArgs &a, hipStream_t st)
{
    if (!cl_conv_kw_applies(amode, omode, a.split_bf16, a.K, a.epi, a.NP, a.act_bf16 != 0, a.D > 1)) return DLKA_ERR_UNSUPPORTED;
    if ((long)a.K * (a.CinP / 32) * (a.split_bf16 == 3 ? 48 : 32) * a.NP * 4 >= (1l << 31)) return DLKA_ERR_UNSUPPORTED;
    const int nt_total = a.NP / 32, row_tiles = cdiv(a.M, 32);
    int nt = 1;
    for (int c = 4; c > 1; --c)
        if (nt_total % c == 0 && (long)row_tiles * (nt_total / c) * 4 >= 2048) { nt = c; break; }
    const int tiles = row_tiles * (nt_total / nt);
    const int kw = (nt > 1 || tiles * 4 >= 1024) ? 4 : 8;
    dim3 grid(row_tiles, 1, nt_total / nt), block(64 * kw);
    auto go = [&](auto am, auto om, auto sp, auto t) {
        dispatch_int<4, 1, 2, 3>(nt, [&](auto n) { dispatch_bool(kw == 8, [&](auto w8) {
            if constexpr (!DLKA_V(w8) || DLKA_V(n) == 1) {
                auto k = cl_conv_kw_kernel<DLKA_V(am), DLKA_V(om), DLKA_V(sp), DLKA_V(w8) ? 8 : 4, DLKA_V(n), DLKA_T(t)>;
                DLKA_LAUNCH(k, grid, block, 0, st, a);
            }
        }); });
    };
    constexpr int_c<0> c0; constexpr int_c<1> c1; constexpr int_c<2> c2; constexpr int_c<3> c3;
    if (a.act_bf16) {
        if (amode == 0) go(c0, c1, c2, type_tag<bf16_t>{});
        else go(c2, c0, c2, type_tag<bf16_t>{});
    } else if (a.split_bf16 == 3) {
        if (omode == 1) go(c0, c1, c3, type_tag<float>{});
        else go(c0, c0, c3, type_tag<float>{});
    } else {
        if (amode == 0 && omode == 0) go(c0, c0, c2, type_tag<float>{});
        else if (amode == 0) go(c0, c1, c2, type_tag<float>{});
        else go(c2, c0, c2, type_tag<float>{});
    }
    DLKA_CHECK_LAUNCH();
    g_conv_kw_launches.fetch_add(1, std::memory_order_relaxed);
    return DLKA_OK;
}

}

extern "C" long dlka_conv_kw_launch_count(void) { return dlka::g_conv_kw_launches.load(std::memory_order_relaxed); }
extern "C" int dlka_conv_kw_applies(int amode, int omode, int split_bf16, int K, int epi, int NP, int act_bf16, int volume)
{
    return dlka::cl_conv_kw_applies(amode, omode, split_bf16, K, epi, NP, act_bf16 != 0, volume != 0) ? 1 : 0;
}
```

deformablelka_amd/csrc/cl_host.h:

```cpp
#pragma once
#include <stdint.h>
#include <stdlib.h>

#include "cl_args.h"
#include "dlka_kernels.h"

namespace dlka {

inline size_t align256(size_t n) { return (n + 255) & ~(size_t)255; }

struct Carver {
    uintptr_t base;
    size_t cap, used;
    bool measure;
    Carver(const void *p, size_t n) : base((uintptr_t)p), cap(n), used(0), measure(false) {}
    static Carver measuring() { Carver c(nullptr, ~(size_t)0); c.measure = true; return c; }
    static Carver probing() { return Carver((const void *)(uintptr_t)256, ~(size_t)0 >> 1); }
    void *take(size_t n)
    {
        n = align256(n);
        if (measure) { used += n; return nullptr; }
        if (!base || used + n > cap) { used = cap + 1; return nullptr; }
        void *r = (void *)(base + used);
        used += n;
        return r;
    }
    void *take_opt(size_t n, bool want)
    {
        n = align256(n);
        if (!want) return nullptr;
        if (measure) { used += n; return nullptr; }
        if (!base || used > cap || used + n > cap) return nullptr;
        void *r = (void *)(base + used);
        used += n;
        return r;
    }
    bool got(const void *p) const { return measure || p != nullptr; }
    void skip_to(size_t n)
    {
        if (!measure && n > cap) used = cap + 1;
        else if (n > used) used = n;
    }
    size_t offset_of(const void *field) const { return (size_t)((uintptr_t)field - base); }
    bool ok() const { return used <= cap; }
};

template <typename Carve>
size_t carved_bytes(Carve carve)
{
    Carver m = Carver::measuring();
    carve(m);
    return m.used;
}

#define DLKA_TRY(expr)                  \
    do {                                \
        int rc_ = (expr);               \
        if (rc_ != DLKA_OK) return rc_; \
    } while (0)

struct SameConv {
    int B, D, H, W, N, M, Cin, Cout, group;
    int kd, kh, kw, pd, ph, pw, dd, dh, dw, K;
    int act_bf16;
};

struct ForkEnv {
    bool gx_rows_set;
    long gx_rows;
    int lka2d_fork;
    bool wgrad_pad;
    bool dwpair;
    bool prep_tiled;
};
ForkEnv fork_env();

struct DwBlk {
    float *blk = nullptr;
    size_t blk_floats = 0;
    bool in_blocked = false;
    const SameConv *chain = nullptr;
    float *chain_blk = nullptr;
    bool *chained = nullptr;
};

int make_same_conv(const dlka_conv_geom *c, SameConv &s);
bool nt_ok(int np);
bool is_depthwise(const SameConv &s);
bool dw_supported(const SameConv &s);
bool dense_fwd_supported(const SameConv &s);
int use_split(const SameConv &s, bool forward);
inline int split_mode_flag(int terms) { return terms == 3 ? 16 : (terms == 2 ? 8 : 0); }
int dense_forward_splits(const SameConv &s, int epi);
int dense_backward_data_splits(const SameConv &s, int epi, int gout_planar = -1);
int dense_forward(const SameConv &s, const float *x, const float *w, const float *bias, float *out, int out_planar, float *wp,
                  int epi, const float *aux, float *out2, hipStream_t st, bool zeroed = false, const ZeroBatch *ride = nullptr, float *out2_f32 = nullptr);
int dense_backward_data(const SameConv &s, const float *gout, int gout_planar, const float *w, float *gx, float *wp, int epi,
                        const float *aux, hipStream_t st, const float *aux2 = nullptr, float *out2 = nullptr, bool zeroed = false, bool g_packed = false,
                        bool aux_f32 = false, float *acc32 = nullptr, const ZeroBatch *ride = nullptr);
size_t dense_wp_floats(const SameConv &s);
size_t dense_wgrad_pad_bytes(const SameConv &s);
int dense_backward_weight(const SameConv &s, const float *x, const float *gout, int gout_planar, float *gw, float *gb, float *part, hipStream_t st,
                          FinalizeJob *defer = nullptr, int g_cpad = 0, float *padbuf = nullptr);
void fill_pw_wgrad(WgradArgs &a, const SameConv &s, const float *x, const float *gout, float *part);
int dw_forward(const SameConv &s, const float *x, const float *w, const float *bias, float *out, float *wp, int flip, hipStream_t st,
               const float *gelu_x = nullptr, const float *gelu_add = nullptr, float *out_lo = nullptr, const DwBlk *bk = nullptr);
int dw_pair(const SameConv &sa, const SameConv &sb, const float *x, const float *wpA, const float *biasA, float *outA, float *outA_lo, const float *wpB, const float *biasB,
            float *outB, float *outB_lo, const float *gelu_x, const float *gelu_add, hipStream_t st);
int dw_backward_weight(const SameConv &s, const float *x, const float *gout, float *gw, float *gb, float *gwp, hipStream_t st, FinalizeJob *defer = nullptr);
bool deform_b16();
bool deform_supported(const SameConv &s);
size_t deform_fwd_slab_floats(const SameConv &s);
int deform_forward(const SameConv &s, const float *x, const float *off, const float *w, const float *bias, float *out, float *wp, hipStream_t st,
                   float *slab = nullptr, bool b16_cores = true);
void fill_deform_bwd(DeformBwdArgs &a, const SameConv &s);
size_t deform_scratch_floats(const SameConv &s);
int deform_backward(const SameConv &s, const float *x, const float *off, const float *w, const float *gout, float *gx, float *goff,
                    float *gw, float *gb, float *wp, float *part, float *scratch, hipStream_t st, FinalizeJob *defer = nullptr, bool gx_zeroed = false,
                    bool goff_zeroed = false, int goff_cpad = 0, float *samp = nullptr, const float *wp16 = nullptr, bool samp_max_zeroed = false);
int pointwise_pair(const SameConv &s, int bwd, const float *in, const float *wp1, const float *bias1, const float *wp2, const float *bias2,
                   const float *a, const float *b, float *out1, float *out1b, float *out2, hipStream_t st, const ZeroBatch *ride = nullptr);
bool wgrad_gather();
void add_job(PrepBatch &pb, const void *src, float *dst, int Cout, int Cin, int K, int KP, int NP, int mode);
}
```

deformablelka_amd/csrc/cl_host_ops.hip:

```cpp
#include <atomic>
#include <mutex>

#include "cl_host.h"

namespace dlka {

int make_same_conv(const dlka_conv_geom *c, SameConv &s)
{
    if (!c) return DLKA_ERR_NULL;
    if (c->B <= 0 || c->C <= 0 || c->D <= 0 || c->H <= 0 || c->W <= 0 || c->Cout <= 0) return DLKA_ERR_SHAPE;
    if (c->kd <= 0 || c->kh <= 0 || c->kw <= 0 || c->dd <= 0 || c->dh <= 0 || c->dw <= 0) return DLKA_ERR_SHAPE;
    if (c->group <= 0 || c->C % c->group || c->Cout % c->group) return DLKA_ERR_GROUP;
    if (c->sd != 1 || c->sh != 1 || c->sw != 1) return DLKA_ERR_UNSUPPORTED;
    if (dlka_conv_out_size(c->D, c->pd, c->dd, c->kd, 1) != c->D || dlka_conv_out_size(c->H, c->ph, c->dh, c->kh, 1) != c->H ||
        dlka_conv_out_size(c->W, c->pw, c->dw, c->kw, 1) != c->W)
        return DLKA_ERR_UNSUPPORTED;
    const long N = (long)c->D * c->H * c->W;
    if (N > (1l << 30) || (long)c->B * N > (1l << 30)) return DLKA_ERR_SHAPE;
    s.B = c->B; s.D = c->D; s.H = c->H; s.W = c->W; s.N = (int)N; s.M = (int)(c->B * N);
    s.Cin = c->C; s.Cout = c->Cout; s.group = c->group;
    s.kd = c->kd; s.kh = c->kh; s.kw = c->kw; s.pd = c->pd; s.ph = c->ph; s.pw = c->pw;
    s.dd = c->dd; s.dh = c->dh; s.dw = c->dw; s.K = c->kd * c->kh * c->kw;
    s.act_bf16 = 0;
    return DLKA_OK;
}

bool nt_ok(int np) { const int nt = np / 32; return nt == 1 || nt == 2 || nt == 3 || nt == 4 || nt == 8; }
bool is_depthwise(const SameConv &s) { return s.group == s.Cin && s.Cin == s.Cout; }
bool dw_supported(const SameConv &s)
{
    const bool kshape = (s.kw == 5 && s.dw == 1) || (s.kw == 7 && s.dw == 3) || (s.kw == 3 && s.dw == 1) || (s.kw == 5 && s.dw == 3) ||
                        (s.kw == 7 && s.dw == 1);
    const int cpb = s.Cin < 256 ? s.Cin : 256;
    return kshape && s.Cin % 32 == 0 && 256 % cpb == 0 && s.Cin % cpb == 0;
}
bool dense_fwd_supported(const SameConv &s) { return s.group == 1 && s.Cin % 32 == 0 && nt_ok(round_up(s.Cout, 32)); }

int use_split(const SameConv &s, bool forward)
{
    static const bool exact = getenv("DLKA_EXACT_FP32") != nullptr;
    static const int fwd = getenv("DLKA_SPLIT_FORWARD") ? atoi(getenv("DLKA_SPLIT_FORWARD")) : 3;
    if (s.act_bf16) return s.K > 1 ? 2 : 0;
    if (exact || s.K <= 1) return 0;
    if (!forward) return 2;
    return (fwd == 2 || fwd == 3) ? fwd : 0;
}

template <class Args> static void copy_geom(Args &a, const SameConv &s)
{
    a.B = s.B; a.D = s.D; a.H = s.H; a.W = s.W; a.N = s.N; a.M = s.M;
    a.kd = s.kd; a.kh = s.kh; a.kw = s.kw; a.pd = s.pd; a.ph = s.ph; a.pw = s.pw; a.dd = s.dd; a.dh = s.dh; a.dw = s.dw; a.K = s.K;
}

static void fill_igemm(IgemmArgs &a, const SameConv &s)
{
    memset(&a, 0, sizeof(a));
    copy_geom(a, s);
    a.act_bf16 = s.act_bf16;
}

static int deform_forward_splits(const SameConv &s) { return cl_igemm_pick_splits(s.M, s.K * (s.Cin / 32), 0, s.K); }
int dense_forward_splits(const SameConv &s, int epi)
{
    const int sp = cl_igemm_pick_splits(s.M, s.K * (s.Cin / 32), epi, s.K);
    if (sp > 1 && cl_conv_kw_applies(0, s.act_bf16 ? 1 : 0, use_split(s, true), s.K, epi, round_up(s.Cout, 32), s.act_bf16 != 0, s.D > 1)) return 1;
    return sp;
}
int dense_backward_data_splits(const SameConv &s, int epi, int gout_planar)
{
    const int sp = cl_igemm_pick_splits(s.M, s.K * (round_up(s.Cout, 32) / 32), epi, s.K);
    const int amode = gout_planar < 0 ? (s.act_bf16 ? 2 : 0) : (gout_planar ? 2 : 0);
    if (sp > 1 && cl_conv_kw_applies(amode, 0, use_split(s, false), s.K, epi, s.Cin, s.act_bf16 != 0, s.D > 1)) return 1;
    return sp;
}

int dense_forward(const SameConv &s, const float *x, const float *w, const float *bias, float *out, int out_planar, float *wp,
                  int epi, const float *aux, float *out2, hipStream_t st, bool zeroed, const ZeroBatch *ride, float *out2_f32)
{
    const int NP = round_up(s.Cout, 32);
    const int split = use_split(s, true);
    if (w) DLKA_TRY(launch_cl_prep_weight(w, wp, s.Cout, s.Cin, s.K, s.Cin, NP, split_mode_flag(split), st));
    IgemmArgs a;
    fill_igemm(a, s);
    a.split_bf16 = split;
    a.in = x; a.wp = wp; a.bias = bias; a.out = out; a.out2 = out2; a.aux = aux; a.epi = epi; a.out_zeroed = zeroed ? 1 : 0;
    a.Cin = s.Cin; a.CinReal = s.Cin; a.CinP = s.Cin; a.Cout = s.Cout; a.NP = NP;
    if (ride) a.zero = *ride;
    int splits = dense_forward_splits(s, epi);
    if (out_planar && cl_conv_brick3_supported(a)) splits = 1;
    if (out2_f32) {
        if (!(s.act_bf16 && epi == 1 && s.K == 1 && splits == 1 && !split && !out_planar)) return DLKA_ERR_UNSUPPORTED;
        a.out2_f32 = out2_f32;
    }
    return launch_cl_igemm(0, out_planar ? 1 : 0, a, splits, st);
}

int dense_backward_data(const SameConv &s, const float *gout, int gout_planar, const float *w, float *gx, float *wp, int epi,
                        const float *aux, hipStream_t st, const float *aux2, float *out2, bool zeroed, bool g_packed,
                        bool aux_f32, float *acc32, const ZeroBatch *ride)
{
    const int KP = round_up(s.Cout, 32), NP = s.Cin;
    if (!(nt_ok(NP) || NP == 192 || NP == 384) || s.Cin % 32) return DLKA_ERR_UNSUPPORTED;
    if (!gout_planar && s.Cout % 32) return DLKA_ERR_UNSUPPORTED;
    const int split = use_split(s, false);
    if (w) DLKA_TRY(launch_cl_prep_weight(w, wp, s.Cout, s.Cin, s.K, KP, NP, 1 | split_mode_flag(split), st));
    IgemmArgs a;
    fill_igemm(a, s);
    a.split_bf16 = split;
    a.pd = s.dd * (s.kd - 1) - s.pd; a.ph = s.dh * (s.kh - 1) - s.ph; a.pw = s.dw * (s.kw - 1) - s.pw;
    a.in = gout; a.wp = wp; a.bias = nullptr; a.out = gx; a.aux = aux; a.aux2 = aux2; a.out2 = out2; a.epi = epi; a.out_zeroed = zeroed ? 1 : 0;
    a.Cin = s.Cout; a.CinReal = s.Cout; a.CinP = KP; a.Cout = s.Cin; a.NP = NP;
    if (g_packed) {
        if (!gout_planar || split != 2) return DLKA_ERR_UNSUPPORTED;
        a.a_packed = 1; a.CinReal = KP;
    }
    a.aux_f32 = aux_f32 ? 1 : 0;
    if (ride) a.zero = *ride;
    int splits = dense_backward_data_splits(s, epi, gout_planar);
    const int bsplit = gout_planar ? cl_conv_brick_split(a) : 0;
    bool brick_only = false;
    if (bsplit == 1) splits = 1;
    else if (bsplit > 1 && splits <= 1) { splits = 2; brick_only = true; }
    if (s.act_bf16 && splits > 1) {
        if (!acc32) return DLKA_ERR_WORKSPACE;
        if (brick_only) DLKA_TRY(launch_zero(acc32, (size_t)s.M * s.Cin * 4, st));
        a.out = acc32; a.out_zeroed = 1;
        DLKA_TRY(launch_cl_igemm(gout_planar ? 2 : 0, 0, a, splits, st));
        return launch_cast_from_f32<bf16_t>(acc32, reinterpret_cast<bf16_t *>(gx), (long)s.M * s.Cin, st);
    }
    if (brick_only) {
        DLKA_TRY(launch_zero(gx, (size_t)s.M * s.Cin * 4, st));
        a.out_zeroed = 1;
    }
    return launch_cl_igemm(gout_planar ? 2 : 0, 0, a, splits, st);
}

size_t dense_wp_floats(const SameConv &s) { return (size_t)s.K * round_up(s.Cin, 32) * round_up(s.Cout, 32) * (s.K > 1 ? 3 : 2) / 2; }

static std::mutex g_fork_env_mu;
static ForkEnv g_fork_env;
static std::atomic<int> g_fork_env_loaded{0};
static void fork_env_load()
{
    std::lock_guard<std::mutex> lk(g_fork_env_mu);
    ForkEnv e;
    const char *r = getenv("DLKA_GX_FORK_MIN_ROWS");
    e.gx_rows_set = r != nullptr;
    e.gx_rows = r ? atol(r) : 0;
    const char *f = getenv("DLKA_LKA2D_FORK");
    e.lka2d_fork = !f ? 2 : f[0] == '0' ? 0 : f[0] == '1' ? 1 : 2;
    auto off = [](const char *name) { const char *v = getenv(name); return v && v[0] == '0'; };
    e.wgrad_pad = !off("DLKA_WGRAD_PAD");
    e.dwpair = !off("DLKA_DWPAIR");
    e.prep_tiled = !off("DLKA_PREP_TILED");
    g_fork_env = e;
    g_fork_env_loaded.store(1, std::memory_order_release);
}
ForkEnv fork_env()
{
    if (!g_fork_env_loaded.load(std::memory_order_acquire)) fork_env_load();
    std::lock_guard<std::mutex> lk(g_fork_env_mu);
    return g_fork_env;
}

size_t dense_wgrad_pad_bytes(const SameConv &s)
{
    if (!fork_env().wgrad_pad || s.K <= 1 || s.group != 1) return 0;
    const size_t n = cl_wgrad_pad_bytes(s.B, s.D, s.H, s.W, s.Cin, s.kd, s.kh, s.kw, s.dd, s.dh, s.dw, s.act_bf16);
    return n < ((size_t)1 << 31) ? align256(n) : 0;
}
int dense_backward_weight(const SameConv &s, const float *x, const float *gout, int gout_planar, float *gw, float *gb, float *part, hipStream_t st,
                          FinalizeJob *defer, int g_cpad, float *padbuf)
{
    if (s.Cin % 32) return DLKA_ERR_UNSUPPORTED;
    if (s.K != 1 && s.K > 7 * 64) return DLKA_ERR_UNSUPPORTED;
    WgradArgs a;
    memset(&a, 0, sizeof(a));
    a.g = gout; a.in = x; a.part = part;
    copy_geom(a, s);
    a.Cin = s.Cin; a.Cout = s.Cout;
    if (s.K == 1 && gout_planar) return DLKA_ERR_UNSUPPORTED;
    if (g_cpad && (!gout_planar || s.K == 1)) return DLKA_ERR_UNSUPPORTED;
    a.g_cpad = g_cpad;
    a.act_bf16 = s.act_bf16;
    a.pad = (padbuf && gout_planar && !g_cpad && dense_wgrad_pad_bytes(s)) ? padbuf : nullptr;
    return launch_cl_wgrad<float>(0, gout_planar ? 1 : 0, a, gw, gb, st, defer);
}

void fill_pw_wgrad(WgradArgs &a, const SameConv &s, const float *x, const float *gout, float *part)
{
    memset(&a, 0, sizeof(a));
    a.g = gout; a.in = x; a.part = part;
    copy_geom(a, s);
    a.Cin = s.Cin; a.Cout = s.Cout;
    a.act_bf16 = s.act_bf16;
}

static void fill_dw_args(DwArgs &a, const SameConv &s, int flip)
{
    memset(&a, 0, sizeof(a));
    a.B = s.B; a.D = s.D; a.H = s.H; a.W = s.W; a.C = s.Cin;
    a.act_bf16 = s.act_bf16; a.xcd_nx = 0;
    a.kd = s.kd; a.kh = s.kh; a.dd = s.dd; a.dh = s.dh;
    if (flip) { a.pd = s.dd * (s.kd - 1) - s.pd; a.ph = s.dh * (s.kh - 1) - s.ph; a.pw = s.dw * (s.kw - 1) - s.pw; }
    else { a.pd = s.pd; a.ph = s.ph; a.pw = s.pw; }
}

int dw_forward(const SameConv &s, const float *x, const float *w, const float *bias, float *out, float *wp, int flip, hipStream_t st,
               const float *gelu_x, const float *gelu_add, float *out_lo, const DwBlk *bk)
{
    if (w) DLKA_TRY(launch_cl_dw_prep_weight(w, wp, s.Cin, s.K, flip, st));
    if (out_lo && s.act_bf16) return DLKA_ERR_UNSUPPORTED;
    DwArgs a;
    fill_dw_args(a, s, flip);
    a.in = x; a.wp = wp; a.bias = bias; a.out = out; a.out_lo = out_lo; a.gelu_x = gelu_x; a.gelu_add = gelu_add;
    if (bk && bk->blk) {
        a.blk = bk->blk; a.blk_floats = bk->blk_floats; a.in_blocked = bk->in_blocked ? 1 : 0;
        if (bk->chained) *bk->chained = false;
        if (bk->chain && bk->chain_blk && cl_dwconv_lds_selected(a, s.kw, s.dw)) {
            DwArgs n;
            fill_dw_args(n, *bk->chain, flip);
            n.blk = bk->chain_blk; n.blk_floats = bk->blk_floats;
            if (cl_dwconv_lds_selected(n, bk->chain->kw, bk->chain->dw)) {
                a.out_blk = bk->chain_blk; a.out_blk_dil = bk->chain->dw;
                if (bk->chained) *bk->chained = true;
            }
        }
    }
    return launch_cl_dwconv(a, s.kw, s.dw, st);
}

static int dwpair_mode()
{
    return fork_env().dwpair ? 1 : 0;
}

int dw_pair(const SameConv &sa, const SameConv &sb, const float *x, const float *wpA, const float *biasA, float *outA, float *outA_lo, const float *wpB, const float *biasB,
            float *outB, float *outB_lo, const float *gelu_x, const float *gelu_add, hipStream_t st)
{
    if (!dwpair_mode()) return DLKA_ERR_UNSUPPORTED;
    auto cubic = [](const SameConv &s) { return s.kd == s.kw && s.kh == s.kw && s.dd == s.dw && s.dh == s.dw && s.pd == s.pw && s.ph == s.pw; };
    if (!cubic(sa) || !cubic(sb) || sa.act_bf16 != sb.act_bf16 || sa.Cin != sb.Cin) return DLKA_ERR_UNSUPPORTED;
    DwPairArgs a;
    memset(&a, 0, sizeof(a));
    a.in = x; a.wpA = wpA; a.wpB = wpB; a.biasA = biasA; a.biasB = biasB; a.outA = outA; a.outB = outB; a.outA_lo = outA_lo; a.outB_lo = outB_lo;
    a.gelu_x = gelu_x; a.gelu_add = gelu_add;
    a.B = sa.B; a.D = sa.D; a.H = sa.H; a.W = sa.W; a.C = sa.Cin;
    a.kA = sa.kw; a.dA = sa.dw; a.pA = sa.pw; a.KA = sa.K;
    a.kB = sb.kw; a.dB = sb.dw; a.pB = sb.pw; a.KB = sb.K;
    a.act_bf16 = sa.act_bf16;
    return launch_cl_dwpair_small(a, st);
}

int dw_backward_weight(const SameConv &s, const float *x, const float *gout, float *gw, float *gb, float *gwp, hipStream_t st, FinalizeJob *defer)
{
    DwWgradArgs a;
    memset(&a, 0, sizeof(a));
    a.g = gout; a.in = x; a.gwp = gwp; a.gb = defer ? gwp + (size_t)s.K * s.Cin : gb;
    a.B = s.B; a.D = s.D; a.H = s.H; a.W = s.W; a.C = s.Cin;
    a.kd = s.kd; a.kh = s.kh; a.pd = s.pd; a.ph = s.ph; a.pw = s.pw; a.dd = s.dd; a.dh = s.dh;
    a.act_bf16 = s.act_bf16;
    if (defer) {
        DLKA_TRY(launch_cl_dwconv_wgrad(a, s.kw, s.dw, st, false));
        memset(defer, 0, sizeof(*defer));
        defer->part = gwp; defer->gw = gw; defer->gb = gb; defer->K = s.K; defer->Cin = s.Cin; defer->kind = 1; defer->chunks = 1;
        defer->n = (long)s.K * s.Cin + s.Cin;
        return DLKA_OK;
    }
    DLKA_TRY(launch_cl_dwconv_wgrad(a, s.kw, s.dw, st));
    return launch_cl_dw_unprep<float>(gwp, gw, s.Cin, s.K, st);
}

bool deform_b16()
{
    static const bool on = [] { const char *e = getenv("DLKA_DEFORM_B16"); return !(e && e[0] == '0') && getenv("DLKA_EXACT_FP32") == nullptr; }();
    return on;
}

bool deform_supported(const SameConv &s) { return s.group == 1 && s.Cin % 32 == 0 && s.Cout % 32 == 0 && nt_ok(s.Cout) && nt_ok(s.Cin); }

static int deform_fwd_actual_splits(const SameConv &s) { return cl_deform_fwd_actual_splits(s.K, s.Cin, deform_forward_splits(s)); }
size_t deform_fwd_slab_floats(const SameConv &s)
{
    const int sp = deform_fwd_actual_splits(s);
    return sp > 1 ? (size_t)sp * s.M * s.Cout : 0;
}
int deform_forward(const SameConv &s, const float *x, const float *off, const float *w, const float *bias, float *out, float *wp, hipStream_t st,
                   float *slab, bool b16_cores)
{
    const int b16 = (s.act_bf16 && b16_cores && deform_b16()) ? 1 : 0;
    if (w) DLKA_TRY(launch_cl_prep_weight(w, wp, s.Cout, s.Cin, s.K, s.Cin, s.Cout, b16 ? 8 : 0, st));
    IgemmArgs a;
    fill_igemm(a, s);
    a.split_bf16 = b16 ? 2 : 0;
    a.in = x; a.off = off; a.wp = wp; a.bias = bias; a.out = out; a.epi = 0; a.out_zeroed = 0;
    a.Cin = s.Cin; a.CinReal = s.Cin; a.CinP = s.Cin; a.Cout = s.Cout; a.NP = s.Cout;
    const int splits = deform_fwd_actual_splits(s);
    if (splits > 1) {
        if (!slab) return DLKA_ERR_WORKSPACE;
        a.out = slab;
        const int rc = launch_cl_deform_fwd(a, splits, st);
        if (rc == DLKA_OK) return launch_cl_slab_reduce(slab, splits, (long)s.M * s.Cout, out, s.act_bf16, st);
        if (rc != DLKA_ERR_UNSUPPORTED || s.act_bf16) return rc;
        a.out = out;
        return launch_cl_igemm(1, 0, a, splits, st);
    }
    const int rc = launch_cl_deform_fwd(a, 1, st);
    if (rc != DLKA_ERR_UNSUPPORTED || s.act_bf16) return rc;
    return launch_cl_igemm(1, 0, a, 1, st);
}

void fill_deform_bwd(DeformBwdArgs &a, const SameConv &s)
{
    memset(&a, 0, sizeof(a));
    copy_geom(a, s);
    a.C = s.Cin; a.Cout = s.Cout; a.CoutP = s.Cout;
    a.act_bf16 = s.act_bf16;
}

size_t deform_scratch_floats(const SameConv &s)
{
    DeformBwdArgs a;
    fill_deform_bwd(a, s);
    return cl_deform_bwd2_scratch_floats(a);
}

static bool samp_f16(const SameConv &s)
{
    static const bool on = [] { const char *e = getenv("DLKA_SAMP_F16"); return !(e && e[0] == '0') && getenv("DLKA_EXACT_FP32") == nullptr; }();
    return on && !s.act_bf16;
}

int deform_backward(const SameConv &s, const float *x, const float *off, const float *w, const float *gout, float *gx, float *goff,
                    float *gw, float *gb, float *wp, float *part, float *scratch, hipStream_t st, FinalizeJob *defer, bool gx_zeroed,
                    bool goff_zeroed, int goff_cpad, float *samp, const float *wp16, bool samp_max_zeroed)
{
    if (gx || goff) {
        if (w) DLKA_TRY(launch_cl_prep_weight(w, wp, s.Cout, s.Cin, s.K, s.Cout, s.Cin, 2, st));
        DeformBwdArgs a;
        fill_deform_bwd(a, s);
        a.in = x; a.off = off; a.g = gout; a.wp = wp; a.gx = gx; a.goff = goff; a.gx_zeroed = gx_zeroed ? 1 : 0; a.goff_zeroed = goff_zeroed ? 1 : 0; a.goff_cpad = goff_cpad;
        a.samp = goff ? samp : nullptr;
        a.samp_f16 = (a.samp && samp_f16(s)) ? 1 : 0;
        a.samp_max_zeroed = samp_max_zeroed ? 1 : 0;
        a.wp16 = deform_b16() ? wp16 : nullptr;
        DLKA_TRY(launch_cl_deform_bwd2(a, scratch, st));
    }
    if (gw) {
        WgradArgs a;
        memset(&a, 0, sizeof(a));
        a.g = gout; a.in = x; a.off = off; a.part = part; a.samp = samp;
        a.samp_f16 = (samp && samp_f16(s)) ? 1 : 0;
        {
            static const bool b16 = [] { const char *e = getenv("DLKA_SAMP_B16MFMA"); return !(e && e[0] == '0'); }();
            a.samp_b16mfma = (a.samp_f16 && b16) ? 1 : 0;
        }
        copy_geom(a, s);
        a.Cin = s.Cin; a.Cout = s.Cout;
        a.act_bf16 = s.act_bf16;
        DLKA_TRY(launch_cl_wgrad<float>(1, 0, a, gw, gb, st, defer));
    } else if (gb) {
        if (s.act_bf16) return DLKA_ERR_UNSUPPORTED;
        DLKA_TRY(launch_cl_colsum(gout, gb, s.M, s.Cout, st));
    }
    return DLKA_OK;
}

int pointwise_pair(const SameConv &s, int bwd, const float *in, const float *wp1, const float *bias1, const float *wp2, const float *bias2,
                   const float *a, const float *b, float *out1, float *out1b, float *out2, hipStream_t st, const ZeroBatch *ride)
{
    const bool unfused = getenv("DLKA_PW_UNFUSED") != nullptr;
    if (unfused || s.Cin != s.Cout || s.K != 1) return DLKA_ERR_UNSUPPORTED;
    PwPairArgs pa;
    memset(&pa, 0, sizeof(pa));
    pa.in = in; pa.wp1 = wp1; pa.bias1 = bias1; pa.wp2 = wp2; pa.bias2 = bias2; pa.a = a; pa.b = b;
    pa.out1 = out1; pa.out1b = out1b; pa.out2 = out2; pa.M = s.M; pa.C = s.Cin; pa.bwd = bwd; pa.act_bf16 = s.act_bf16;
    if (ride) pa.zero = *ride;
    return s.Cin == 32 ? launch_cl_pointwise_pair(pa, st) : launch_cl_pointwise_chain(pa, st);
}

static std::atomic<int> g_wgrad_gather{-1};
bool wgrad_gather()
{
    int v = g_wgrad_gather.load(std::memory_order_acquire);
    if (v < 0) {
        int want = getenv("DLKA_WGRAD_GATHER") != nullptr ? 1 : 0;
        if (g_wgrad_gather.compare_exchange_strong(v, want, std::memory_order_acq_rel)) v = want;
    }
    return v != 0;
}

void add_job(PrepBatch &pb, const void *src, float *dst, int Cout, int Cin, int K, int KP, int NP, int mode)
{
    PrepJob &j = pb.j[pb.njobs++];
    j.src = (const float *)src; j.dst = dst; j.Cout = Cout; j.Cin = Cin; j.K = K; j.KP = KP; j.NP = NP; j.mode = mode;
    if (!fork_env().prep_tiled && (mode & 7) <= 2) j.mode |= 32;
    j.n = (mode == 3 || mode == 4) ? (long)Cin * K : (long)K * KP * NP;
    pb.total += j.n;
}

}

using namespace dlka;

extern "C" {

void dlka_env_refresh(void)
{
    fork_env_load();
}

int dlka_lka3d_force_wgrad_gather(int on)
{
    const int old = wgrad_gather() ? 1 : 0;
    g_wgrad_gather.store(on ? 1 : 0, std::memory_order_release);
    return old;
}

}
```

deformablelka_amd/csrc/dlka_kernels.h:

```cpp
#pragma once
#include "cl_args.h"
#include "dlka_common.h"

namespace dlka {

int deform_pick_cob(int Og);
int deform_fwd_wt_floats(const Geom &g);
template <typename T>
int launch_relayout_weight(const T *w, float *wt, int group, int Og, int Cg, int K, int OgP, hipStream_t st);
template <typename T, int NOFF>
int launch_deform_fwd(const T *x, const T *off, const T *w, const T *bias, T *out, float *wt, const Geom &g, hipStream_t st);
template <typename T, int NOFF>
int launch_deform_bwd_input_offset(const T *x, const T *off, const float *wt, int OgP, const T *gout,
                                   float *gx32, T *goff, const Geom &g, hipStream_t st);
template <typename T, int NOFF>
int launch_deform_bwd_weight(const T *x, const T *off, const T *gout, float *gw32, const Geom &g, hipStream_t st);
template <typename T>
int launch_bias_grad(const T *gout, T *gb, int B, int Cout, int No, hipStream_t st);
template <typename T>
int launch_cast_from_f32(const float *src, T *dst, long n, hipStream_t st);
template <typename T>
int launch_sample_index(const T *off, int32_t *idx, uint8_t *mask, const Geom &g, int path, hipStream_t st);
template <typename T>
int launch_sample_index2(const T *off, int32_t *idx, uint8_t *mask, const Geom &g, int path, hipStream_t st);

template <int NOFF> int launch_deform_fwd_f64(const double *x, const double *off, const double *w, const double *bias, double *out, const Geom &g, hipStream_t st);
template <int NOFF> int launch_deform_bwd_f64(const double *x, const double *off, const double *w, const double *gout, double *gx, double *goff, double *gw, double *gb,
                                              const Geom &g, hipStream_t st);
int launch_conv_fwd_f64(const double *x, const double *w, const double *bias, double *out, const Geom &g, hipStream_t st);
int launch_conv_bwd_f64(const double *x, const double *w, const double *gout, double *gx, double *gw, double *gb, const Geom &g, hipStream_t st);

int conv_fwd_wt_floats(const Geom &g);
int conv_bwd_wb_floats(const Geom &g);
template <typename T>
int launch_conv_fwd(const T *x, const T *w, const T *bias, T *out, float *wt, const Geom &g, hipStream_t st);
template <typename T>
int launch_conv_bwd_data(const T *gout, const T *w, T *gx, float *wb, const Geom &g, hipStream_t st);
size_t conv_bwd_weight_part_floats(const Geom &g, size_t elem_bytes);
template <typename T>
int launch_conv_bwd_weight(const T *x, const T *gout, float *gw32, const Geom &g, hipStream_t st, float *part = nullptr);

int launch_zero(void *ptr, size_t bytes, hipStream_t st);
struct ZeroBatch;
int launch_zero_batch(ZeroBatch &b, hipStream_t st);
template <typename T> int launch_gelu_fwd(const T *x, T *y, long n, hipStream_t st);
template <typename T> int launch_gelu_bwd(const T *x, const T *gy, T *gx, long n, hipStream_t st);
template <typename T> int launch_mul_fwd(const T *a, const T *b, T *y, long n, hipStream_t st);
template <typename T> int launch_mul_bwd(const T *a, const T *b, const T *gy, T *ga, T *gb, long n, hipStream_t st);
template <typename T> int launch_add_fwd(const T *a, const T *b, T *y, long n, hipStream_t st);
template <typename T> int launch_gelu_bwd_sum(const T *x, const T *g1, const T *g2, T *gx, long n, hipStream_t st);

int launch_cl_prep_weight(const float *w, float *wp, int Cout, int Cin, int K, int KP, int NP, int mode, hipStream_t st);
int launch_cl_prep_batch(const PrepBatch &b, hipStream_t st);
int cl_prep_table_blocks(const PrepJob &j);
int launch_cl_prep_table(const PrepJob *jobs_dev, const int *first_dev, int job_lo, int job_hi, int nblocks, hipStream_t st);
int cl_igemm_pick_splits(int M, int units, int epi, int K);
int launch_cl_pointwise(const IgemmArgs &a, hipStream_t st);
int launch_cl_pointwise_pair(const PwPairArgs &a, hipStream_t st);
int launch_cl_pointwise_chain(const PwPairArgs &a, hipStream_t st);
int launch_cl_conv_wave(int amode, int omode, const IgemmArgs &a, int splits, hipStream_t st);
bool cl_conv_kw_applies(int amode, int omode, int split_bf16, int K, int epi, int NP, bool act_bf16, bool volume);
int launch_cl_conv_kw(int amode, int omode, const IgemmArgs &a, hipStream_t st);
bool cl_conv_brick_supported(const IgemmArgs &a);
int cl_conv_brick_split(const IgemmArgs &a);
bool cl_conv_brick3_supported(const IgemmArgs &a);
int launch_cl_conv_brick3(const IgemmArgs &a, hipStream_t st);
int launch_cl_conv_brick(const IgemmArgs &a, hipStream_t st);
int launch_cl_igemm(int amode, int omode, IgemmArgs a, int splits, hipStream_t st);
int launch_cl_deform_fwd(IgemmArgs a, int splits, hipStream_t st);
int cl_deform_fwd_actual_splits(int K, int CinP, int splits);
int launch_cl_slab_reduce(const float *slab, int S, long n, void *out, int out_bf16, hipStream_t st);
int cl_wgrad_pick_chunks(int M, int K, int Cout, int Cin, int amode);
size_t cl_wgrad_part_floats(int M, int K, int Cout, int Cin);
size_t cl_wgrad_pad_bytes(int B, int D, int H, int W, int Cin, int kd, int kh, int kw, int dd, int dh, int dw, int act_bf16);
template <typename T> int launch_cl_wgrad(int amode, int gmode, WgradArgs a, T *gw, T *gb, hipStream_t st, FinalizeJob *defer = nullptr);
size_t cl_wgrad_part_floats_mode(int M, int K, int Cout, int Cin, int amode);
int launch_cl_wgrad_finalize(FinalizeBatch &b, hipStream_t st);
int launch_pl_bn_forward(const float *x, const float *w, const float *b, float *stats, float *y, float *scratch, int B, int C, long N, float eps, hipStream_t st);
int launch_pl_bn_backward(const float *g, const float *x, const float *w, const float *stats, float *gx, float *gw, float *gb, float *scratch, int B, int C,
                          long N, hipStream_t st);
int launch_pl_pw_forward(const float *x, const float *w, const float *bias, float *y, int B, int CI, int CO, long N, hipStream_t st);
int launch_pl_pw_backward(const float *x, const float *w, const float *g, float *gx, float *gw, float *gb, int B, int CI, int CO, long N, hipStream_t st);
long cl_wgrad_finalize_plan_job(FinalizeJob &j);
int launch_cl_wgrad_finalize_table(const FinalizeJob *jobs_device, int job_lo, int job_hi, long nblocks, hipStream_t st);
int launch_cl_wgrad_pw3(const WgradArgs *jobs, float *const *gw, float *const *gb, hipStream_t st, FinalizeJob *defer);
int launch_cl_colsum(const float *g, float *gb32, int M, int Cout, hipStream_t st);
int launch_cl_dw_prep_weight(const float *w, float *wp, int C, int K, int flip, hipStream_t st);
int launch_cl_dwconv(const DwArgs &a, int kw, int dil_w, hipStream_t st);
bool cl_dwpair_small_supported(const DwPairArgs &a);
int launch_cl_dwpair_small(const DwPairArgs &a, hipStream_t st);
int launch_cl_dwconv_lds(const DwArgs &a, int kw, int dil_w, hipStream_t st);
bool cl_dwconv_lds_selected(const DwArgs &a, int kw, int dil_w);
int cl_dwconv_lds_mode();
size_t cl_dwconv_blk_floats(int B, int C, int D, int H, int W, int dil);
int launch_cl_dwconv_wgrad(DwWgradArgs a, int kw, int dil_w, hipStream_t st, bool zero_init = true);
template <typename T> int launch_cl_dw_unprep(const float *gwp, T *gw, int C, int K, hipStream_t st);
int launch_cl_transpose(const float *src, float *dst, int B, int C, int N, int to_cl, hipStream_t st, int bf16 = 0);
size_t cl_deform_bwd2_scratch_floats(const DeformBwdArgs &a);
int launch_cl_deform_bwd2(const DeformBwdArgs &a, float *scratch, hipStream_t st);
int cl_deform_goff_ccsplit(const DeformBwdArgs &a);

int cl_ddw2d_supported(int C);
size_t cl_ddw2d_part_floats(int M, int K, int C);
int launch_cl_ddw2d_fwd(const DwArgs2d &d, hipStream_t st);
int launch_cl_ddw2d_bwd(const DwArgs2d &d, float *gw, hipStream_t st, hipStream_t gx_st = nullptr);
int lka2d_cl_supported(int B, int C, int H, int W, int dtype);
size_t lka2d_cl_saved_bytes(int B, int C, int H, int W, int dtype);
int lka2d_cl_saved_offsets(int B, int C, int H, int W, int dtype, size_t byte_offsets[2], int *elem_bytes);
size_t lka2d_cl_workspace_bytes(int B, int C, int H, int W, int dtype);
int lka2d_cl_forward(const void *x, const dlka_lka2d_params *p, void *y, void *saved, size_t saved_bytes, void *workspace, size_t workspace_bytes, int B,
                     int C, int H, int W, int dtype, hipStream_t st);
int lka2d_cl_backward(const void *x, const dlka_lka2d_params *p, const void *gy, const void *saved, size_t saved_bytes, void *gx, const dlka_lka2d_grads *gr,
                      void *workspace, size_t workspace_bytes, int B, int C, int H, int W, int dtype, hipStream_t st);

int launch_cl_layernorm_fwd(const float *x, int x_planar, const float *pos, const float *w, const float *b, float *xt, float *xn, float *stats, int B, int N,
                            int C, float eps, hipStream_t st, int lo = 0, float *xn32 = nullptr);
int launch_cl_layernorm_bwd(const float *g, const float *g_res, const float *xt, const float *stats, const float *w, float *gxt, float *gw, float *gb,
                            float *gpos, int B, int N, int C, hipStream_t st, bool zeroed = false, int lo = 0);
int launch_cl_scale_residual_fwd(const float *xt, const float *e, const float *gamma, float *out, long M, int C, hipStream_t st, int lo = 0);
int launch_cl_scale_residual_bwd(const float *g, const float *e, const float *gamma, float *ge, float *ggamma, long M, int C, hipStream_t st, bool zeroed = false, int lo = 0);
int launch_cl_bn_stats(const float *x, float *sums, float *stats, long M, int C, float eps, hipStream_t st, bool zeroed = false, float *det_part = nullptr, size_t det_floats = 0);
int launch_cl_bn_apply(const float *x, const float *res, const float *w, const float *b, const float *stats, const float *mask, float *y, long M, long N, int C,
                       float slope, hipStream_t st);
int launch_cl_bn_bwd(const float *g, const float *gmask, const float *x, const float *y, const float *w, const float *stats, float *sums, float *gx, float *gres,
                     const float *gres_add, float *gw, float *gb, long M, long N, int C, float slope, int training, hipStream_t st, bool zeroed = false);
int launch_cl_channel_scale(const float *x, const float *mask, float *y, int B, long N, int C, hipStream_t st);

}
```

deformablelka_amd/ops.py:

```python
from __future__ import annotations

import ctypes
import math
from ctypes import byref
from typing import Optional, Sequence, Tuple

import numpy as np
import torch

from . import _lib as L


def _triple(v) -> Tuple[int, int, int]:
    if isinstance(v, int):
        return (v, v, v)
    v = tuple(int(x) for x in v)
    if len(v) != 3:
        raise ValueError(f"expected an int or a 3-tuple, got {v}")
    return v


def _pair(v) -> Tuple[int, int]:
    if isinstance(v, int):
        return (v, v)
# ... 321 lines not shown
    Cout = weight.shape[0]
    y = torch.empty((B, Cout) + tuple(x.shape[2:]), dtype=torch.float32, device=x.device)
    L.check(L.get_lib().dlka_pointwise_planar_forward(L.ptr(x), L.ptr(weight), L.ptr(bias), L.ptr(y), B, Cin, Cout, x[0, 0].numel(), L.stream_ptr(x)),
            "pointwise_planar_forward")
    return y


def pointwise_planar_backward(x, weight, g, need=(True, True, True)):
    L.require_device(x, weight, g)
    B, Cin = x.shape[:2]
    Cout = weight.shape[0]
    gx = torch.empty_like(x) if need[0] else None
    gw = torch.empty_like(weight) if need[1] else None
    gb = torch.empty(Cout, dtype=torch.float32, device=x.device) if (need[1] and need[2]) else None
    if need[0] or need[1]:
        L.check(L.get_lib().dlka_pointwise_planar_backward(L.ptr(x), L.ptr(weight), L.ptr(g), L.ptr(gx), L.ptr(gw), L.ptr(gb), B, Cin, Cout, x[0, 0].numel(),
                                                           L.stream_ptr(x)), "pointwise_planar_backward")
    if need[2] and gb is None:
        gb = g.sum(dim=[0] + list(range(2, g.dim())))
    return gx, gw, gb


def _ptr_struct(cls, fields, tensors):
    st = cls()
    for n, t in zip(fields, tensors):
        setattr(st, n, t.data_ptr())
    return st


def lka3d_attention_forward(x, params: Sequence[torch.Tensor]):
    L.require_device(x, *params)
    x = x.contiguous()
    params = [t.contiguous() for t in params]
    B, C, D, H, W = (int(v) for v in x.shape)
    lib = L.get_lib()
    dt = L.dtype_code(x)
    sb, wb = lib.dlka_lka3d_saved_bytes(B, C, D, H, W, dt), lib.dlka_lka3d_workspace_bytes(B, C, D, H, W, dt)
    if sb == 0:
        L.check(-4, "lka3d_attention_forward")
    saved, ws = L.scratch(sb, x), L.scratch(wb, x)
    y = torch.empty_like(x)
    ps = _ptr_struct(L.Lka3dPtrs, L.LKA3D_FIELDS, params)
    rc = lib.dlka_lka3d_attention_forward(L.ptr(x), byref(ps), L.ptr(y), L.ptr(saved), sb, L.ptr(ws), wb, B, C, D, H, W, dt,
                                          L.stream_ptr(x))
    L.check(rc, "lka3d_attention_forward")
    return y, saved


def lka3d_attention_backward(x, params, grad_y, saved):
    L.require_device(x, grad_y, saved, *params)
    x, grad_y = x.contiguous(), grad_y.contiguous()
    params = [t.contiguous() for t in params]
    B, C, D, H, W = (int(v) for v in x.shape)
    lib = L.get_lib()
    dt = L.dtype_code(x)
    wb = lib.dlka_lka3d_workspace_bytes(B, C, D, H, W, dt)
    ws = L.scratch(wb, x)
    gx = torch.empty_like(x)
    grads = [torch.empty_like(t) for t in params]
    ps = _ptr_struct(L.Lka3dPtrs, L.LKA3D_FIELDS, params)
    gs = _ptr_struct(L.Lka3dPtrs, L.LKA3D_FIELDS, grads)
    rc = lib.dlka_lka3d_attention_backward(L.ptr(x), byref(ps), L.ptr(grad_y), L.ptr(saved), saved.numel(), L.ptr(gx), byref(gs),
                                           L.ptr(ws), wb, B, C, D, H, W, dt, L.stream_ptr(x))
    L.check(rc, "lka3d_attention_backward")
    return gx, grads


def lka2d_bf16_supported(C: int) -> bool:
    return C % 32 == 0 and C // 32 in (1, 2, 3, 4, 6, 8, 12)


def _lka2d_params(x, params):
    if x.dtype == torch.bfloat16:
        if not lka2d_bf16_supported(int(x.shape[1])):
            raise RuntimeError(f"deformable_LKA_Attention with bfloat16 activations needs C / 32 in {{1,2,3,4,6,8,12}}, got C={int(x.shape[1])}")
        return [_fp32_param(t) for t in params]
    return [t.contiguous() for t in params]


def lka2d_attention_forward(x, params: Sequence[torch.Tensor]):
    L.require_device(x, *params)
    x = x.contiguous()
    params = _lka2d_params(x, params)
    B, C, H, W = (int(v) for v in x.shape)
    lib = L.get_lib()
    dt = L.dtype_code(x)
    sb, wb = lib.dlka_lka2d_saved_bytes(B, C, H, W, dt), lib.dlka_lka2d_workspace_bytes(B, C, H, W, dt)
    if sb == 0:
        L.check(-4, "lka2d_attention_forward")
    saved, ws = L.scratch(sb, x), L.scratch(wb, x)
    y = torch.empty_like(x)
    ps = _ptr_struct(L.Lka2dPtrs, L.LKA2D_FIELDS, params)
    rc = lib.dlka_lka2d_attention_forward(L.ptr(x), byref(ps), L.ptr(y), L.ptr(saved), sb, L.ptr(ws), wb, B, C, H, W, dt,
                                          L.stream_ptr(x))
    L.check(rc, "lka2d_attention_forward")
    return y, saved


def lka2d_saved_offsets(saved, x):
    B, C, H, W = (int(v) for v in x.shape)
    lib = L.get_lib()
    offs = (ctypes.c_size_t * 2)()
    eb = ctypes.c_int(0)
    L.check(lib.dlka_lka2d_saved_offsets(B, C, H, W, L.dtype_code(x), offs, byref(eb)), "lka2d_saved_offsets")
    dt = torch.float32 if eb.value == 4 else torch.bfloat16
    out = []
    for o, ch in zip(offs, (50, 98)):
        n = B * ch * H * W * eb.value
        out.append(saved[int(o):int(o) + n].view(dt).view(B, ch, H, W))
    return out


def lka2d_attention_backward(x, params, grad_y, saved):
    L.require_device(x, grad_y, saved, *params)
    x, grad_y = x.contiguous(), grad_y.to(x.dtype).contiguous()
    params = _lka2d_params(x, params)
    B, C, H, W = (int(v) for v in x.shape)
    lib = L.get_lib()
    dt = L.dtype_code(x)
    wb = lib.dlka_lka2d_workspace_bytes(B, C, H, W, dt)
    ws = L.scratch(wb, x)
    gx = torch.empty_like(x)
    grads = [torch.empty_like(t) for t in params]
    ps = _ptr_struct(L.Lka2dPtrs, L.LKA2D_FIELDS, params)
    gs = _ptr_struct(L.Lka2dPtrs, L.LKA2D_FIELDS, grads)
    rc = lib.dlka_lka2d_attention_backward(L.ptr(x), byref(ps), L.ptr(grad_y), L.ptr(saved), saved.numel(), L.ptr(gx), byref(gs),
                                           L.ptr(ws), wb, B, C, H, W, dt, L.stream_ptr(x))
    L.check(rc, "lka2d_attention_backward")
    return gx, grads


def _geom_cl(x_shape, cout, k, p, d, group, dg=1):
    B, D, H, W, C = (int(v) for v in x_shape)
    return L.ConvGeom(B, C, D, H, W, int(cout), *k, 1, 1, 1, *p, *d, int(group), int(dg), 64)


def conv3d_forward_cl(x, weight, bias=None, padding=0, dilation=1, groups=1, out_planar=False):
    L.require_device(x, weight, bias)
    p, d = _triple(padding), _triple(dilation)
    x, weight = x.contiguous(), weight.contiguous()
    bias = None if bias is None else bias.contiguous()
    g = _geom_cl(x.shape, weight.shape[0], tuple(weight.shape[2:5]), p, d, groups)
    lib = L.get_lib()
    dt = L.dtype_code(x)
    B, D, H, W, _ = x.shape
    shape = (B, g.Cout, D, H, W) if out_planar else (B, D, H, W, g.Cout)
    out = torch.empty(shape, dtype=x.dtype, device=x.device)
    wsb = lib.dlka_conv3d_cl_workspace(byref(g), dt, 0)
    ws = L.scratch(wsb, x)
    rc = lib.dlka_conv3d_forward_cl(L.ptr(x), L.ptr(weight), L.ptr(bias), L.ptr(out), int(out_planar), L.ptr(ws), wsb, byref(g), dt,
                                    L.stream_ptr(x))
    L.check(rc, "conv3d_forward_cl")
    return out


def conv3d_backward_cl(x, weight, grad_out, padding=0, dilation=1, groups=1, grad_out_planar=False, need=(True, True, True)):
    L.require_device(x, weight, grad_out)
    p, d = _triple(padding), _triple(dilation)
    x, weight, grad_out = x.contiguous(), weight.contiguous(), grad_out.contiguous()
    g = _geom_cl(x.shape, weight.shape[0], tuple(weight.shape[2:5]), p, d, groups)
    lib = L.get_lib()
    dt = L.dtype_code(x)
    if not any(need):
        return None, None, None
    gi = torch.empty_like(x) if need[0] else None
    gw = torch.empty_like(weight) if need[1] else None
    gb = torch.empty((g.Cout,), dtype=x.dtype, device=x.device) if need[2] else None
    wsb = lib.dlka_conv3d_cl_workspace(byref(g), dt, 1)
    ws = L.scratch(wsb, x)
    rc = lib.dlka_conv3d_backward_cl(L.ptr(x), L.ptr(weight), L.ptr(grad_out), int(grad_out_planar), L.ptr(gi), L.ptr(gw), L.ptr(gb),
                                     L.ptr(ws), wsb, byref(g), dt, L.stream_ptr(x))
    L.check(rc, "conv3d_backward_cl")
    return gi, gw, gb


def deform_cl_grad_dtype(x):
    return torch.float32 if x.dtype == torch.bfloat16 else x.dtype


def _deform_cl_fp32_operands(x, **named):
    for name, t in named.items():
        if t is not None and t.dtype != (torch.float32 if x.dtype == torch.bfloat16 else x.dtype):
            raise RuntimeError(f"channels-last deformable conv: {name} must be float32 (bfloat16 is the storage of x / out / grad_out only); got {t.dtype}")


def deform_conv3d_forward_cl(x, offset, weight, bias, padding=1, dilation=1):
    L.require_device(x, offset, weight, bias)
    _deform_cl_fp32_operands(x, offset=offset, weight=weight, bias=bias)
    p, d = _triple(padding), _triple(dilation)
    x, offset, weight, bias = x.contiguous(), offset.contiguous(), weight.contiguous(), bias.contiguous()
    g = _geom_cl(x.shape, weight.shape[0], tuple(weight.shape[2:5]), p, d, 1)
    lib = L.get_lib()
    dt = L.dtype_code(x)
    B, D, H, W, _ = x.shape
    out = torch.empty((B, D, H, W, g.Cout), dtype=x.dtype, device=x.device)
    wsb = lib.dlka_deform_conv3d_cl_workspace(byref(g), dt, 0)
    ws = L.scratch(wsb, x)
    rc = lib.dlka_deform_conv3d_forward_cl(L.ptr(x), L.ptr(offset), L.ptr(weight), L.ptr(bias), L.ptr(out), L.ptr(ws), wsb, byref(g), dt,
                                           L.stream_ptr(x))
    L.check(rc, "deform_conv3d_forward_cl")
    return out


def deform_conv3d_backward_cl(x, offset, weight, grad_out, padding=1, dilation=1, need=(True, True, True, True)):
    L.require_device(x, offset, weight, grad_out)
    _deform_cl_fp32_operands(x, offset=offset, weight=weight)
    if grad_out.dtype != x.dtype:
        raise RuntimeError(f"channels-last deformable conv: grad_out must have x's dtype ({x.dtype}), got {grad_out.dtype}")
    p, d = _triple(padding), _triple(dilation)
    x, offset, weight, grad_out = x.contiguous(), offset.contiguous(), weight.contiguous(), grad_out.contiguous()
    g = _geom_cl(x.shape, weight.shape[0], tuple(weight.shape[2:5]), p, d, 1)
    lib = L.get_lib()
    dt = L.dtype_code(x)
    if not any(need):
        return None, None, None, None
    gdt = deform_cl_grad_dtype(x)
    gi = torch.empty(x.shape, dtype=gdt, device=x.device) if need[0] else None
    go = torch.empty(offset.shape, dtype=gdt, device=x.device) if need[1] else None
    gw = torch.empty(weight.shape, dtype=gdt, device=x.device) if need[2] else None
    gb = torch.empty((g.Cout,), dtype=gdt, device=x.device) if need[3] else None
    wsb = lib.dlka_deform_conv3d_cl_workspace(byref(g), dt, 1)
    ws = L.scratch(wsb, x)
    rc = lib.dlka_deform_conv3d_backward_cl(L.ptr(x), L.ptr(offset), L.ptr(weight), L.ptr(grad_out), L.ptr(gi), L.ptr(go), L.ptr(gw),
                                            L.ptr(gb), L.ptr(ws), wsb, byref(g), dt, L.stream_ptr(x))
    L.check(rc, "deform_conv3d_backward_cl")
    return gi, go, gw, gb


def lka3d_tokens_supported(x, B, C, D, H, W, variant=0) -> bool:
    dt = x if isinstance(x, torch.dtype) else x.dtype
    if dt not in (torch.float32, torch.bfloat16):
        return False
    return bool(L.get_lib().dlka_lka3d_tokens_supported_v(B, C, D, H, W, L.DLKA_F32 if dt == torch.float32 else L.DLKA_BF16, int(variant)))


def autocast_activation_dtype(x):
    try:
        on = torch.is_autocast_enabled(x.device.type)
        dt = torch.get_autocast_dtype(x.device.type) if on else None
    except (TypeError, RuntimeError):
        return x.dtype
    return torch.bfloat16 if (on and dt == torch.bfloat16 and x.dtype in (torch.float32, torch.bfloat16)) else x.dtype



def _fp32_param(t):
    if t.dtype != torch.float32:
        raise RuntimeError(f"the token-layout D-LKA block keeps its parameters in float32 (bf16 is an ACTIVATION dtype); got {t.dtype}")
    return t.contiguous()


def lka3d_attention_tokens_forward(x, params, dims, variant=0):
    L.require_device(x, *params)
    x = x.contiguous()
    params = [_fp32_param(t) for t in params]
    B, N, C = (int(v) for v in x.shape)
    D, H, W = (int(v) for v in dims)
    assert N == D * H * W
    lib = L.get_lib()
    dt = L.dtype_code(x)
    v = int(variant)
    sb, wb = lib.dlka_lka3d_tokens_saved_bytes_v(B, C, D, H, W, dt, v), lib.dlka_lka3d_tokens_workspace_bytes_v(B, C, D, H, W, dt, v)
    if sb == 0:
        L.check(-8, "lka3d_attention_tokens_forward")
    saved, ws = L.scratch(sb, x), L.scratch(wb, x)
    y = torch.empty_like(x)
    ps = _ptr_struct(L.Lka3dPtrs, L.LKA3D_FIELDS, params)
    rc = lib.dlka_lka3d_attention_tokens_forward_v(L.ptr(x), byref(ps), L.ptr(y), L.ptr(saved), sb, L.ptr(ws), wb, B, C, D, H, W, dt, v,
                                                   L.stream_ptr(x))
    L.check(rc, "lka3d_attention_tokens_forward")
    return y, saved


def lka3d_tokens_saved_offsets(saved, B, C, dims, act_dtype=torch.float32, variant=0):
    D, H, W = (int(v) for v in dims)
    off = ctypes.c_size_t(0)
    dt = L.DLKA_F32 if act_dtype == torch.float32 else L.DLKA_BF16
    lib = L.get_lib()
    if lib.dlka_lka3d_tokens_saved_offsets_v(B, C, D, H, W, dt, int(variant), byref(off)) != 0:
        sb = 4 if act_dtype == torch.float32 else 2
        off = ctypes.c_size_t(4 * ((B * C * D * H * W * sb + 255) & ~255))
    o = int(off.value)
    return saved[o:o + B * 81 * D * H * W * 4].view(torch.float32).view(B, 81, D, H, W)


def tblock3d_saved_offsets(saved, B, C, dims, variant=0, lka_bf16=False):
    D, H, W = (int(v) for v in dims)
    off = ctypes.c_size_t(0)
    L.check(L.get_lib().dlka_tblock3d_saved_offsets_v(B, C, D, H, W, L.DLKA_BF16 if lka_bf16 else L.DLKA_F32, int(variant), byref(off)), "tblock3d_saved_offsets")
    o = int(off.value)
    return saved[o:o + B * 81 * D * H * W * 4].view(torch.float32).view(B, 81, D, H, W)


def tblock3d_saved_activation_signs(saved, B, C, dims, variant=0, lka_bf16=False):
    D, H, W = (int(v) for v in dims)
    offs = (ctypes.c_size_t * 2)()
    L.check(L.get_lib().dlka_tblock3d_saved_activations_v(B, C, D, H, W, L.DLKA_BF16 if lka_bf16 else L.DLKA_F32, int(variant), offs), "tblock3d_saved_activations")
    n = B * D * H * W * C
    a1 = saved[int(offs[0]):int(offs[0]) + n * 4].view(torch.float32).view(B, D * H * W, C)
    rd = saved[int(offs[1]):int(offs[1]) + n * 4].view(torch.float32).view(B, D * H * W, C)
    return a1 > 0, rd > 0, rd != 0


def lka3d_attention_tokens_backward(x, params, grad_y, saved, dims, variant=0, side_stream=None):
    L.require_device(x, grad_y, saved, *params)
    x, grad_y = x.contiguous(), grad_y.to(x.dtype).contiguous()
# ... 1029 lines not shown
```

include/dlka.h:

```cpp
#ifndef DLKA_H_
#define DLKA_H_

#include <stddef.h>
#include <stdint.h>

#ifdef __cplusplus
extern "C" {
#endif

#define DLKA_ABI_VERSION 1

typedef enum dlka_status {
    DLKA_OK = 0,
    DLKA_ERR_NULL = -1,
    DLKA_ERR_GROUP = -2,
    DLKA_ERR_DEFORM_GROUP = -3,
    DLKA_ERR_SHAPE = -4,
    DLKA_ERR_IM2COL_STEP = -5,
    DLKA_ERR_DTYPE = -6,
    DLKA_ERR_WORKSPACE = -7,
    DLKA_ERR_UNSUPPORTED = -8,
    DLKA_ERR_LAUNCH = -9
} dlka_status;

// ... 93 lines not shown
    const void *conv0_offset_w, *conv0_offset_b;
    const void *conv0_w;
    const void *conv_spatial_offset_w, *conv_spatial_offset_b;
    const void *conv_spatial_w;
    const void *conv1_w, *conv1_b;
    const void *proj_2_w, *proj_2_b;
} dlka_lka2d_params;

typedef struct dlka_lka2d_grads {
    void *proj_1_w, *proj_1_b, *conv0_offset_w, *conv0_offset_b, *conv0_w,
         *conv_spatial_offset_w, *conv_spatial_offset_b, *conv_spatial_w, *conv1_w, *conv1_b, *proj_2_w, *proj_2_b;
} dlka_lka2d_grads;

size_t dlka_lka2d_saved_bytes(int B, int C, int H, int W, int dtype);
size_t dlka_lka2d_workspace_bytes(int B, int C, int H, int W, int dtype);
int dlka_lka2d_attention_forward(const void *x, const dlka_lka2d_params *p, void *y,
                                 void *saved, size_t saved_bytes, void *workspace, size_t workspace_bytes,
                                 int B, int C, int H, int W, int dtype, void *stream);
int dlka_lka2d_force_general(int on);
int dlka_lka2d_saved_offsets(int B, int C, int H, int W, int dtype, size_t byte_offsets[2], int *elem_bytes);
int dlka_lka2d_attention_backward(const void *x, const dlka_lka2d_params *p, const void *grad_y,
                                  const void *saved, size_t saved_bytes,
                                  void *grad_x, const dlka_lka2d_grads *grads,
                                  void *workspace, size_t workspace_bytes,
                                  int B, int C, int H, int W, int dtype, void *stream);



size_t dlka_conv3d_cl_workspace(const dlka_conv_geom *g, int dtype, int backward);
int dlka_conv3d_forward_cl(const void *x, const void *weight, const void *bias, void *out, int out_planar,
                           void *workspace, size_t workspace_bytes, const dlka_conv_geom *g, int dtype, void *stream);
int dlka_conv3d_backward_cl(const void *x, const void *weight, const void *grad_out, int grad_out_planar,
                            void *grad_x, void *grad_weight, void *grad_bias,
                            void *workspace, size_t workspace_bytes, const dlka_conv_geom *g, int dtype, void *stream);

size_t dlka_deform_conv3d_cl_workspace(const dlka_conv_geom *g, int dtype, int backward);
int dlka_deform_conv3d_forward_cl(const void *x, const void *offset, const void *weight, const void *bias, void *out,
                                  void *workspace, size_t workspace_bytes, const dlka_conv_geom *g, int dtype, void *stream);
int dlka_deform_conv3d_backward_cl(const void *x, const void *offset, const void *weight, const void *grad_out,
                                   void *grad_x, void *grad_offset, void *grad_weight, void *grad_bias,
                                   void *workspace, size_t workspace_bytes, const dlka_conv_geom *g, int dtype, void *stream);

int dlka_ncdhw_to_ndhwc(const void *src, void *dst, int B, int C, int N, int dtype, void *stream);
int dlka_ndhwc_to_ncdhw(const void *src, void *dst, int B, int C, int N, int dtype, void *stream);

int    dlka_lka3d_tokens_supported(int B, int C, int D, int H, int W, int dtype);
size_t dlka_lka3d_tokens_saved_bytes(int B, int C, int D, int H, int W, int dtype);
size_t dlka_lka3d_tokens_workspace_bytes(int B, int C, int D, int H, int W, int dtype);
int dlka_lka3d_attention_tokens_forward(const void *x, const dlka_lka3d_params *p, void *y,
                                        void *saved, size_t saved_bytes, void *workspace, size_t workspace_bytes,
                                        int B, int C, int D, int H, int W, int dtype, void *stream);
size_t dlka_lka3d_tokens_prepare_plan_bytes(int nblocks);
int dlka_lka3d_tokens_prepare_plan(int nblocks, const dlka_lka3d_params *params, void *const *saved, const size_t *saved_bytes,
                                   const int *dims5, int dtype, void *plan_host, size_t plan_bytes);
int dlka_lka3d_tokens_prepare_run(const void *plan_device, const void *plan_host, int nblocks, void *stream);
int dlka_lka3d_tokens_prepare_run_range(const void *plan_device, const void *plan_host, int nblocks, int block_lo, int block_hi, void *stream);
int dlka_lka3d_attention_tokens_forward_prepared(const void *x, const dlka_lka3d_params *p, void *y,
                                                 void *saved, size_t saved_bytes, void *workspace, size_t workspace_bytes,
                                                 int B, int C, int D, int H, int W, int dtype, void *stream);
int dlka_lka3d_attention_tokens_backward(const void *x, const dlka_lka3d_params *p, const void *grad_y,
                                         const void *saved, size_t saved_bytes,
                                         void *grad_x, const dlka_lka3d_grads *grads,
                                         void *workspace, size_t workspace_bytes,
                                         int B, int C, int D, int H, int W, int dtype, void *stream);
size_t dlka_lka3d_tokens_partials_bytes_v(int B, int C, int D, int H, int W, int dtype, int variant);
size_t dlka_wgrad_finalize_plan_bytes(int nblocks);
int dlka_wgrad_finalize_plan_init(void *plan_host, size_t plan_bytes, int nblocks);
int dlka_lka3d_attention_tokens_backward_deferred_v(const void *x, const dlka_lka3d_params *p, const void *grad_y,
                                                    const void *saved, size_t saved_bytes,
                                                    void *grad_x, const dlka_lka3d_grads *grads,
                                                    void *workspace, size_t workspace_bytes,
                                                    void *partials, size_t partials_bytes, void *plan_host, int plan_slot,
                                                    int B, int C, int D, int H, int W, int dtype, int variant, void *stream);
int dlka_lka3d_attention_tokens_backward_phase_v(const void *x, const dlka_lka3d_params *p, const void *grad_y,
                                                 const void *saved, size_t saved_bytes,
                                                 void *grad_x, const dlka_lka3d_grads *grads,
                                                 void *workspace, size_t workspace_bytes,
                                                 void *partials, size_t partials_bytes, void *plan_host, int plan_slot, int phase,
                                                 int B, int C, int D, int H, int W, int dtype, int variant, void *stream);
int dlka_wgrad_finalize_run_slot(const void *plan_host, int plan_slot, void *stream);
int dlka_wgrad_finalize_plan_seal(void *plan_host);
int dlka_wgrad_finalize_run(const void *plan_device, const void *plan_host, int block_lo, int block_hi, void *stream);


int dlka_layernorm_tokens_forward(const void *x, int x_planar, const void *pos, const void *w, const void *b, void *xt, void *xn,
                                  void *stats, int B, int N, int C, float eps, int dtype, void *stream);
int dlka_layernorm_tokens_backward(const void *g_xn, const void *g_res, const void *xt, const void *stats, const void *w, void *gxt,
                                   void *gw, void *gb, void *gpos, int B, int N, int C, int dtype, void *stream);
int dlka_scale_residual_forward(const void *xt, const void *e, const void *gamma, void *out, int64_t M, int C, int dtype, void *stream);
int dlka_scale_residual_backward(const void *g, const void *e, const void *gamma, void *ge, void *ggamma, int64_t M, int C, int dtype,
                                 void *stream);
int dlka_batchnorm_cl_forward(const void *x, const void *res, const void *w, const void *b, void *stats, int training, void *y,
                              void *scratch, int64_t M, int C, float eps, float slope, int dtype, void *stream);
int dlka_batchnorm_cl_backward(const void *g, const void *x, const void *y, const void *w, const void *stats, int training, void *gx,
                               void *gres, void *gw, void *gb, void *scratch, int64_t M, int C, float slope, int dtype, void *stream);
int dlka_channel_scale(const void *x, const void *mask, void *y, int B, int64_t N, int C, int dtype, void *stream);

int dlka_batchnorm_planar_forward(const void *x, const void *w, const void *b, void *stats, void *y, void *scratch,
                                  int B, int C, int64_t N, float eps, void *stream);
int dlka_batchnorm_planar_backward(const void *g, const void *x, const void *w, const void *stats, void *gx, void *gw, void *gb,
                                   void *scratch, int B, int C, int64_t N, void *stream);
int dlka_pointwise_planar_forward(const void *x, const void *w, const void *bias, void *y, int B, int Cin, int Cout, int64_t N, void *stream);
int dlka_pointwise_planar_backward(const void *x, const void *w, const void *g, void *gx, void *gw, void *gb,
                                   int B, int Cin, int Cout, int64_t N, void *stream);

typedef struct dlka_tblock3d_params {
    const void *norm_w, *norm_b;
    const void *gamma;
    const void *pos_embed;
    const void *conv51_conv1_w, *conv51_conv2_w;
    const void *conv51_norm1_w, *conv51_norm1_b;
    const void *conv51_norm2_w, *conv51_norm2_b;
    const void *conv8_w, *conv8_b;
} dlka_tblock3d_params;

typedef struct dlka_tblock3d_grads {
    void *norm_w, *norm_b, *gamma, *pos_embed, *conv51_conv1_w, *conv51_conv2_w, *conv51_norm1_w, *conv51_norm1_b,
         *conv51_norm2_w, *conv51_norm2_b, *conv8_w, *conv8_b;
} dlka_tblock3d_grads;

int dlka_tblock3d_supported(int B, int C, int D, int H, int W, int dtype);
size_t dlka_tblock3d_saved_bytes(int B, int C, int D, int H, int W, int dtype);
size_t dlka_tblock3d_workspace_bytes(int B, int C, int D, int H, int W, int dtype);
int dlka_tblock3d_forward(const void *x, int x_planar, const dlka_tblock3d_params *p, const dlka_lka3d_params *lka,
                          const void *drop_mask, int training, void *bn_stats, void *y,
                          void *saved, size_t saved_bytes, void *workspace, size_t workspace_bytes,
                          int B, int C, int D, int H, int W, float ln_eps, float bn_eps, int dtype, void *stream);
int dlka_tblock3d_backward(const dlka_tblock3d_params *p, const dlka_lka3d_params *lka, const void *drop_mask, int training,
                           const void *bn_stats, const void *grad_y, const void *saved, size_t saved_bytes, void *grad_x,
                           const dlka_tblock3d_grads *grads, const dlka_lka3d_grads *lka_grads,
                           void *workspace, size_t workspace_bytes, int B, int C, int D, int H, int W, int dtype, void *stream);

int dlka_deform_conv2d_sample_index_path(const void *offset, int32_t *idx, uint8_t *mask,
                                         const dlka_conv_geom *g, int dtype, int path, void *stream);

size_t dlka_deform_dwconv2d_cl_workspace(const dlka_conv_geom *g, int dtype, int backward);
int dlka_deform_dwconv2d_forward_cl(const void *x, const void *offset, const void *weight, void *out,
                                    void *workspace, size_t workspace_bytes, const dlka_conv_geom *g, int dtype, void *stream);
int dlka_deform_dwconv2d_backward_cl(const void *x, const void *offset, const void *weight, const void *grad_out,
                                     void *grad_x, void *grad_offset, void *grad_weight,
                                     void *workspace, size_t workspace_bytes, const dlka_conv_geom *g, int dtype, void *stream);

typedef enum dlka_lka3d_variant { DLKA_LKA3D_SYNAPSE = 0, DLKA_LKA3D_ACDC = 1 } dlka_lka3d_variant;
int    dlka_lka3d_tokens_supported_v(int B, int C, int D, int H, int W, int dtype, int variant);
size_t dlka_lka3d_tokens_saved_bytes_v(int B, int C, int D, int H, int W, int dtype, int variant);
int dlka_lka3d_force_wgrad_gather(int on);
int  dlka_fork_stats(int device, int64_t *contexts, int64_t *leases);
void dlka_env_refresh(void);
long dlka_dwconv_lds_launch_count(void);
long dlka_conv_brick_launch_count(void);
long dlka_dwpair_launch_count(void);
long dlka_pw_chain_launch_count(void);
long dlka_conv_kw_launch_count(void);
int dlka_conv_kw_applies(int amode, int omode, int split_bf16, int K, int epi, int NP, int act_bf16, int volume);
long dlka_dwconv_2p_launch_count(void);
size_t dlka_lka3d_tokens_workspace_bytes_v(int B, int C, int D, int H, int W, int dtype, int variant);
int dlka_lka3d_attention_tokens_forward_v(const void *x, const dlka_lka3d_params *p, void *y, void *saved, size_t saved_bytes,
                                          void *workspace, size_t workspace_bytes, int B, int C, int D, int H, int W, int dtype, int variant, void *stream);
int dlka_lka3d_attention_tokens_backward_v(const void *x, const dlka_lka3d_params *p, const void *grad_y, const void *saved, size_t saved_bytes,
                                           void *grad_x, const dlka_lka3d_grads *grads, void *workspace, size_t workspace_bytes,
                                           int B, int C, int D, int H, int W, int dtype, int variant, void *stream);
int    dlka_tblock3d_supported_v(int B, int C, int D, int H, int W, int dtype, int variant);
size_t dlka_tblock3d_saved_bytes_v(int B, int C, int D, int H, int W, int dtype, int variant);
int dlka_lka3d_tokens_saved_offsets_v(int B, int C, int D, int H, int W, int dtype, int variant, size_t *byte_offset);
int dlka_tblock3d_saved_offsets_v(int B, int C, int D, int H, int W, int dtype, int variant, size_t *byte_offset);
int dlka_tblock3d_saved_activations_v(int B, int C, int D, int H, int W, int dtype, int variant, size_t byte_offsets[2]);
size_t dlka_tblock3d_workspace_bytes_v(int B, int C, int D, int H, int W, int dtype, int variant);
int dlka_tblock3d_forward_v(const void *x, int x_planar, const dlka_tblock3d_params *p, const dlka_lka3d_params *lka,
                            const void *drop_mask, int training, void *bn_stats, void *y, void *saved, size_t saved_bytes,
                            void *workspace, size_t workspace_bytes, int B, int C, int D, int H, int W, float ln_eps, float bn_eps,
                            int dtype, int variant, void *stream);
int dlka_tblock3d_backward_v(const dlka_tblock3d_params *p, const dlka_lka3d_params *lka, const void *drop_mask, int training,
                             const void *bn_stats, const void *grad_y, const void *saved, size_t saved_bytes, void *grad_x,
                             const dlka_tblock3d_grads *grads, const dlka_lka3d_grads *lka_grads,
                             void *workspace, size_t workspace_bytes, int B, int C, int D, int H, int W, int dtype, int variant, void *stream);
int dlka_tblock3d_backward_phase_v(const dlka_tblock3d_params *p, const dlka_lka3d_params *lka, const void *drop_mask, int training, const void *bn_stats,
                                   const void *grad_y, const void *saved, size_t saved_bytes, void *grad_x, const dlka_tblock3d_grads *grads,
                                   const dlka_lka3d_grads *lka_grads, void *workspace, size_t workspace_bytes, int B, int C, int D, int H, int W, int dtype,
                                   int variant, int phase, void *stream);

#define DLKA_TILES_MAX_T 64
#define DLKA_TILES_K_MAX 32
#define DLKA_TILES_IDENTITY 0
#define DLKA_TILES_SOFTMAX 1
#define DLKA_TILES_SIGMOID 2
int dlka_tiles_gather(const float *x, int C, int X, int Y, int Z, const int *origins, int T, const int *masks, int M, int pd, int ph,
                      int pw, int pad_x, int pad_y, int pad_z, float pad_value, float *out, void *stream);
int dlka_tiles_blend(const void *logits, int dtype, int K, int nonlin, float mirror_scale, const float *gauss, float *score,
                     float *weight, int Xp, int Yp, int Zp, const int *origins, int T, const int *masks, int M, int pd, int ph, int pw,
                     void *stream);
int dlka_tiles_finalize(const float *score, const float *weight, int K, int Xp, int Yp, int Zp, int pad_x, int pad_y, int pad_z, int X,
                        int Y, int Z, float *probs, int64_t *seg, void *stream);
long dlka_tiles_launch_count(void);

#define DLKA_SEG_LOSS_K_MAX 32
#define DLKA_SEG_LOSS_NNUNET 0
#define DLKA_SEG_LOSS_DICE2D 1
#define DLKA_LABEL_F32 0
#define DLKA_LABEL_I64 1
typedef struct dlka_seg_loss_desc {
    int32_t B, K;
    int64_t N;
    int32_t dtype, label_dtype, mode, batch_dice, do_bg;
    float smooth, weight_ce, weight_dice;
    float class_weight[DLKA_SEG_LOSS_K_MAX];
} dlka_seg_loss_desc;
size_t dlka_seg_loss_workspace_bytes(const dlka_seg_loss_desc *d);
int dlka_seg_loss_forward(const void *logits, const void *labels, const dlka_seg_loss_desc *d, void *workspace, size_t workspace_bytes,
                          float *loss, float *dc, float *stats, float *coef, void *stream);
int dlka_seg_loss_backward(const void *logits, const void *labels, const dlka_seg_loss_desc *d, const float *coef, const float *grad_output,
                           void *grad_logits, void *stream);
int dlka_seg_eval_counts(const void *logits, const void *labels, const dlka_seg_loss_desc *d, void *workspace, size_t workspace_bytes,
                         int64_t *counts, void *stream);
long dlka_seg_loss_launch_count(void);

#define DLKA_SD_K_MAX 32
#define DLKA_SD_U8 0
#define DLKA_SD_I16 1
#define DLKA_SD_I32 2
#define DLKA_SD_I64 3
typedef struct dlka_sd_desc {
    int32_t rank, connectivity, label_dtype, K, mask_mode;
    int64_t ext[3];
    double spacing[3];
    int64_t class_id[DLKA_SD_K_MAX];
} dlka_sd_desc;
size_t dlka_sd_stats_workspace_bytes(const dlka_sd_desc *d);
int dlka_sd_label_stats(const void *prediction, const void *label, const dlka_sd_desc *d, void *workspace, size_t workspace_bytes,
                        int64_t *stats, void *stream);
int64_t dlka_sd_distance_cells(const dlka_sd_desc *d, const int64_t *boxes);
int dlka_sd_distances(const void *prediction, const void *label, const dlka_sd_desc *d, const int64_t *boxes, void *workspace,
                      size_t workspace_bytes, double *sqdist, int64_t sqdist_cells, void *stream);
long dlka_sd_launch_count(void);

#define DLKA_CC_K_MAX 32
#define DLKA_CC_IDS_MAX 64
#define DLKA_CC_SUMMARY (1 + 2 * DLKA_CC_K_MAX)
typedef struct dlka_cc_desc {
    int32_t rank, connectivity, label_dtype, K, mask_mode, n_ids, has_min;
    int64_t ext[3];
    int64_t class_id[DLKA_CC_IDS_MAX];
    int32_t entry_of[DLKA_CC_IDS_MAX];
    int64_t min_count[DLKA_CC_K_MAX];
} dlka_cc_desc;
size_t dlka_cc_workspace_bytes(const dlka_cc_desc *d);
int dlka_cc_components(const void *image, const dlka_cc_desc *d, void *workspace, size_t workspace_bytes, int32_t *labels, void *filtered,
                       int32_t *summary, void *stream);
int dlka_cc_component_table(const dlka_cc_desc *d, const void *workspace, size_t workspace_bytes, int64_t capacity, int64_t *sizes,
                            int32_t *owner, void *stream);
long dlka_cc_launch_count(void);

typedef struct dlka_resample_desc {
    int32_t C, dtype;
    int32_t taps[3];
    int64_t in[3], out[3];
} dlka_resample_desc;
int dlka_resample_argmax(const void *x, uint8_t *labels, const dlka_resample_desc *d, const int32_t *idx, const double *w,
                         const int32_t *region_class, void *stream);
int dlka_resample_linear(const void *x, void *y, const dlka_resample_desc *d, const int32_t *idx, const double *w, void *stream);
int dlka_resample_labels(const int32_t *seg, int32_t *out, const dlka_resample_desc *d, const int32_t *idx, const double *w, int strict,
                         void *stream);
int dlka_resample_spline_eval(const double *coef, double *y, const dlka_resample_desc *d, const int32_t *start, const double *w4,
                              const double *lo, const double *hi, int clip_axis, void *stream);
long dlka_resample_launch_count(void);

#define DLKA_RESAMPLE_SPLINE_PAD 12
#define DLKA_SPLINE_REFLECT 0
#define DLKA_SPLINE_MIRROR 1
int dlka_spline_pad(const void *x, double *padded, int dtype, const int64_t *in, const int64_t *pad, void *stream);
int dlka_spline_prefilter(double *coef, const int64_t *ext, int axis, int boundary, void *stream);

#define DLKA_AUG_I16 3
#define DLKA_AUG_CONSTANT 0
#define DLKA_AUG_NEAREST 1
#define DLKA_AUG_RADIUS_MAX 32
#define DLKA_AUG_OPS_MAX 4
enum {
    DLKA_AUG_OP_NONE = 0,
    DLKA_AUG_OP_NOISE = 1,
    DLKA_AUG_OP_SCALE_ADD = 2,
    DLKA_AUG_OP_CONTRAST = 3,
    DLKA_AUG_OP_GAMMA = 4,
    DLKA_AUG_OP_RETAIN = 5,
    DLKA_AUG_OP_REPLACE = 6
};
typedef struct dlka_augment_desc {
    int32_t B, C, dtype, order, mode, pad;
    int64_t src[3], out[3];
    double cval;
} dlka_augment_desc;
int dlka_augment_spatial(const void *x, const double *coef, void *y, const dlka_augment_desc *d, const double *maps, const int32_t *plain,
                         void *stream);
int dlka_augment_spatial_labels(const int32_t *seg, int32_t *out, const dlka_augment_desc *d, const double *maps, const int32_t *plain,
                                void *stream);
int dlka_augment_spatial2d(const void *x, const double *coef, void *y, const dlka_augment_desc *d, const double *maps, const int32_t *plain,
                           void *stream);
int dlka_augment_spatial2d_labels(const int32_t *seg, int32_t *out, const dlka_augment_desc *d, const double *maps, const int32_t *plain,
                                  void *stream);
int dlka_augment_gaussian(const void *x, void *y, int dtype, int64_t channels, const int64_t *ext, int axis, const int32_t *radius,
                          const double *weights, void *stream);
size_t dlka_augment_stats_workspace_bytes(int64_t channels, int64_t cells);
int dlka_augment_channel_stats(const void *x, double *stats, void *workspace, size_t workspace_bytes, int dtype, int64_t channels,
                               int64_t cells, void *stream);
int dlka_augment_pointwise(const void *x, const void *noise, void *y, int dtype, int64_t B, int64_t C, const int64_t *ext, const double *ops,
                           const double *stats0, const double *stats1, const int32_t *flip, void *stream);
long dlka_augment_launch_count(void);
// ... 61 lines not shown
```

Measured before the change: 212.5 volumes/s.

## Add split-K with ticketed last-block reduction to the kw conv kernel

Adds a split-K mode to the cl_conv_kw implicit-GEMM kernel for small-tile cases. Each slice along grid.y writes partials to a slab, and the last block to arrive (tracked by an atomic ticket) reduces them and applies the epilogue. It is wired into the offset-conv forward and backward-data paths of the 3D LKA token blocks, reusing the weight-prep reserve as slab and ticket space. The aim is more parallelism on the small deep-stage volumes, at the cost of extra slab traffic, ticket zeroing and a serial final reduction.

After: 214.0 volumes/s (median of 6 runs). No clear change (+0.7%).

```diff
diff --git a/deformablelka_amd/_lib.py b/deformablelka_amd/_lib.py
--- a/deformablelka_amd/_lib.py
+++ b/deformablelka_amd/_lib.py
@@ -214,6 +214,10 @@
     "dlka_dwconv_2p_launch_count": (ctypes.c_long, []),
     "dlka_conv_kw_launch_count": (ctypes.c_long, []),
     "dlka_conv_kw_applies": (c_int, [c_int] * 8),
+    "dlka_conv_kw_force_ks": (c_int, [c_int]),
+    "dlka_conv_kw_last_ks": (c_int, []),
+    "dlka_conv_kw_pick_ks": (c_int, [c_int] * 3),
+    "dlka_conv3d_kw_split_run": (c_int, [c_int] + [c_void_p] * 6 + [c_size_t, c_void_p, c_size_t, _G, c_int, c_int, c_void_p]),
     "dlka_lka3d_tokens_supported_v": (c_int, [c_int] * 7),
     "dlka_lka3d_tokens_saved_bytes_v": (c_size_t, [c_int] * 7),
     "dlka_lka3d_tokens_workspace_bytes_v": (c_size_t, [c_int] * 7),
diff --git a/deformablelka_amd/csrc/capi_lka3d_tokens.h b/deformablelka_amd/csrc/capi_lka3d_tokens.h
--- a/deformablelka_amd/csrc/capi_lka3d_tokens.h
+++ b/deformablelka_amd/csrc/capi_lka3d_tokens.h
@@ -161,6 +161,16 @@
     return W;
 }
 
+inline KwSplitWs tok_kw_split_ws(float *wp_reserve, const TokGeoms &G)
+{
+    KwSplitWs k = {nullptr, 0, nullptr, 0, 0};
+    const size_t bytes = align256(G.wp_floats() * 4), tick = (size_t)KW_SPLIT_TICKETS * 4;
+    if (!wp_reserve || bytes <= tick) return k;
+    k.ticket = reinterpret_cast<unsigned *>(wp_reserve); k.ticket_words = KW_SPLIT_TICKETS;
+    k.slab = wp_reserve + KW_SPLIT_TICKETS; k.slab_bytes = bytes - tick;
+    return k;
+}
+
 struct TokFwdWs {
     float *wp_reserve, *part_reserve, *gg1_reserve;
     float *a32, *t1_32, *t_32;
diff --git a/deformablelka_amd/csrc/capi_lka3d_tokens.hip b/deformablelka_amd/csrc/capi_lka3d_tokens.hip
--- a/deformablelka_amd/csrc/capi_lka3d_tokens.hip
+++ b/deformablelka_amd/csrc/capi_lka3d_tokens.hip
@@ -111,6 +111,10 @@
     memset(&zb, 0, sizeof(zb));
     if (dense_forward_splits(G.offc_f, 0) > 1) zb.add(off, G.Off);
     if (dense_forward_splits(G.pw, 3) > 1) zb.add(y, G.E);
+    KwSplitWs kws = tok_kw_split_ws(Wf.wp_reserve, G);
+    const bool kw_split = kws.ticket && dense_forward_kw_ks(G.offc_f, 0) > 1;
+    if (kw_split) zb.add(reinterpret_cast<float *>(kws.ticket), KW_SPLIT_TICKETS);
+    if (zb.overflow) return DLKA_ERR_WORKSPACE;
     TokPrep PW;
     const ZeroBatch *ride = nullptr;
     if (prepared) {
@@ -138,7 +142,7 @@
         bk7.blk = blkB; bk7.blk_floats = G.blk_floats(); bk7.in_blocked = chained;
         DLKA_TRY(dw_forward(G.dw7_f, t1_out, N0, (const float *)p->conv_spatial_b, t_out, PW.dw7_f, 0, st, nullptr, nullptr, bf ? t : nullptr, &bk7));
     }
-    DLKA_TRY(dense_forward(G.offc_f, t_out, N0, (const float *)p->offset_b, off, 1, PW.off_f, 0, nullptr, nullptr, st, true));
+    DLKA_TRY(dense_forward(G.offc_f, t_out, N0, (const float *)p->offset_b, off, 1, PW.off_f, 0, nullptr, nullptr, st, true, nullptr, nullptr, kw_split ? &kws : nullptr));
     DLKA_TRY(deform_forward(G.dcn, t, off, N0, (const float *)p->deform_b, f, PW.dcn_f, st, slab));
     const int prc = pointwise_pair(G.pw, 0, f, PW.pw_f[1], (const float *)p->conv1_b, PW.pw_f[2], (const float *)p->proj_2_b, a, x, g1, m, y, st);
     if (prc != DLKA_ERR_UNSUPPORTED) return prc;
@@ -433,6 +437,9 @@
     if (dense_backward_data_splits(G.pw, 3) > 1) zb.add(gx, G.E);
     float *samp_max = (samp && !bf) ? samp + (size_t)G.dcn.K * G.dcn.M * G.dcn.Cin / 2 : nullptr;
     zb.add(samp_max, 1);
+    KwSplitWs kws = tok_kw_split_ws(Wb.wp_reserve, G);
+    const bool kw_split = phase != 2 && kws.ticket && dense_backward_data_kw_ks(G.offc, 3, 1) > 1;
+    if (kw_split) zb.add(reinterpret_cast<float *>(kws.ticket), KW_SPLIT_TICKETS);
     if (zb.overflow) return DLKA_ERR_WORKSPACE;
 
 #define DLKA_P1(call) do { if (phase != 2) DLKA_TRY(call); } while (0)
@@ -463,7 +470,7 @@
     if (gx_forked) DLKA_TRY(lease.join(1));
     else
         DLKA_P1(deform_backward(G.dcn, t, off, N0, gf, gta, nullptr, nullptr, nullptr, PW.dcn_b, nullptr, scratch, st, nullptr, true, false, 0, nullptr, PW.dcn_b16));
-    DLKA_P1(dense_backward_data(G.offc, goff, 1, N0, gt, PW.off_b, 3, gta, st, nullptr, nullptr, true, goff_cpad != 0, true, ga2));
+    DLKA_P1(dense_backward_data(G.offc, goff, 1, N0, gt, PW.off_b, 3, gta, st, nullptr, nullptr, true, goff_cpad != 0, true, ga2, nullptr, kw_split ? &kws : nullptr));
     DLKA_P2(dw_backward_weight(G.dw7, t1, gt, (float *)gr->conv_spatial_w, (float *)gr->conv_spatial_b, stage7, st, &fb.j[fb.njobs++]));
     bool chained = false;
     DwBlk bk7, bk5;
diff --git a/deformablelka_amd/csrc/cl_args.h b/deformablelka_amd/csrc/cl_args.h
--- a/deformablelka_amd/csrc/cl_args.h
+++ b/deformablelka_amd/csrc/cl_args.h
@@ -26,6 +26,15 @@
     }
 }
 
+struct KwSplitWs {
+    float *slab;
+    size_t slab_bytes;
+    unsigned *ticket;
+    int ticket_words;
+    int ks;
+};
+constexpr int KW_SPLIT_TICKETS = 1024;
+
 struct IgemmArgs {
     const float *in;
     const float *off;
@@ -49,6 +58,7 @@
     ZeroBatch zero;
     int zero_xblocks;
     int epi;
+    KwSplitWs kws;
 };
 
 struct PwPairArgs {
diff --git a/deformablelka_amd/csrc/cl_conv_kw.hip b/deformablelka_amd/csrc/cl_conv_kw.hip
--- a/deformablelka_amd/csrc/cl_conv_kw.hip
+++ b/deformablelka_amd/csrc/cl_conv_kw.hip
@@ -7,9 +7,30 @@
 
 namespace dlka {
 
+#if defined(HIPEMU)
+static inline void ks_drain() {}
+static inline unsigned ks_publish_and_draw(unsigned *t) { return reinterpret_cast<std::atomic<unsigned> *>(t)->fetch_add(1u, std::memory_order_acq_rel); }
+static inline void ks_acquire() { std::atomic_thread_fence(std::memory_order_acquire); }
+static inline void ks_reset(unsigned *t) { reinterpret_cast<std::atomic<unsigned> *>(t)->store(0u, std::memory_order_release); }
+#else
+__device__ __forceinline__ void ks_drain() { asm volatile("s_waitcnt vmcnt(0)" ::: "memory"); }
+__device__ __forceinline__ unsigned ks_publish_and_draw(unsigned *t)
+{
+    __builtin_amdgcn_fence(__ATOMIC_RELEASE, "agent");
+    asm volatile("s_waitcnt vmcnt(0)" ::: "memory");
+    return __hip_atomic_fetch_add(t, 1u, __ATOMIC_RELAXED, __HIP_MEMORY_SCOPE_AGENT);
+}
+__device__ __forceinline__ void ks_acquire()
+{
+    __builtin_amdgcn_fence(__ATOMIC_ACQUIRE, "agent");
+    asm volatile("s_waitcnt vmcnt(0)" ::: "memory");
+}
+__device__ __forceinline__ void ks_reset(unsigned *t) { __hip_atomic_store(t, 0u, __ATOMIC_RELAXED, __HIP_MEMORY_SCOPE_AGENT); }
+#endif
+
 std::atomic<long> g_conv_kw_launches{0};
 
-template <int AMODE, int OMODE, int SPLIT, int KW, int NT, typename T>
+template <int AMODE, int OMODE, int SPLIT, int KW, int NT, typename T, bool KSP = false>
 __global__ __launch_bounds__(64 * KW) void cl_conv_kw_kernel(IgemmArgs p)
 {
     constexpr bool A16 = AMODE == 0 && sizeof(T) == 2;
@@ -38,9 +59,12 @@
 
     const int nchunk = p.CinP / 32;
     const int units = p.K * nchunk;
-    const int ups = (units + KW - 1) / KW;
-    const int unit_lo = wave * ups;
-    const int unit_hi = min(units, unit_lo + ups);
+    const int per = KSP ? (units + (int)gridDim.y - 1) / (int)gridDim.y : units;
+    const int g_lo = KSP ? min(units, (int)blockIdx.y * per) : 0;
+    const int g_hi = KSP ? min(units, g_lo + per) : units;
+    const int ups = (g_hi - g_lo + KW - 1) / KW;
+    const int unit_lo = g_lo + wave * ups;
+    const int unit_hi = min(g_hi, unit_lo + ups);
     const BufRsrc rin = make_rsrc(p.in, AMODE == 2 ? (size_t)p.B * p.CinReal * p.N * 4 : (size_t)p.M * p.Cin * sizeof(T));
     const BufRsrc rw = make_rsrc(p.wp, (size_t)units * UF * p.NP * 4);
     const unsigned unit_bytes = (unsigned)(UF * p.NP) * 4u, seg_bytes = (unsigned)p.NP * 16u;
@@ -138,6 +162,22 @@
         }
     }
 
+    auto emit = [&](int t, int e, float val) {
+        const int row = OMODE == 1 ? (e & 31) : (e >> 5), col = OMODE == 1 ? (e >> 5) : (e & 31);
+        const int mr = mbase + row, n = n0 + 32 * t + col;
+        if (mr >= p.M || n >= p.Cout) return;
+        if (p.bias) val += p.bias[n];
+        if (OMODE == 1) {
+            const int bb = mr / p.N, vv = mr - bb * p.N;
+            p.out[((long)bb * p.Cout + n) * p.N + vv] = val;
+        } else {
+            const long o = (long)mr * p.Cout + n;
+            if (p.epi == 3) val += (sizeof(T) == 2 && p.aux_f32) ? p.aux[o] : act_load1(reinterpret_cast<const T *>(p.aux), o);
+            act_store1(reinterpret_cast<T *>(p.out), o, val);
+        }
+    };
+    const long tile = (long)blockIdx.z * gridDim.x + blockIdx.x;
+    float *slabs = KSP ? p.kws.slab + tile * (long)gridDim.y * (NT * 1024) : nullptr;
     float *mine = Red[wave];
     wave_sync();
 #pragma unroll
@@ -152,18 +192,30 @@
             float val = 0.f;
 #pragma unroll
             for (int w = 0; w < KW; ++w) val += Red[w][rr * RS + col + 32 * hh];
-            const int mr = mbase + row, n = n0 + 32 * t + col;
-            if (mr >= p.M || n >= p.Cout) continue;
-            if (p.bias) val += p.bias[n];
-            if (OMODE == 1) {
-                const int bb = mr / p.N, vv = mr - bb * p.N;
-                p.out[((long)bb * p.Cout + n) * p.N + vv] = val;
-            } else {
-                const long o = (long)mr * p.Cout + n;
-                if (p.epi == 3) val += (sizeof(T) == 2 && p.aux_f32) ? p.aux[o] : act_load1(reinterpret_cast<const T *>(p.aux), o);
-                act_store1(reinterpret_cast<T *>(p.out), o, val);
-            }
-        }
+            if (KSP) slabs[((long)blockIdx.y * NT + t) * 1024 + e] = val;
+            else emit(t, e, val);
+        }
+    }
+    if (KSP) {
+        const unsigned ks = gridDim.y;
+        ks_drain();
+        __syncthreads();
+        unsigned *flag = reinterpret_cast<unsigned *>(&Red[0][0]);
+        if (tid == 0) {
+            const unsigned tk = ks_publish_and_draw(p.kws.ticket + tile);
+            if (tk == ks - 1) ks_acquire();
+            *flag = tk;
+        }
+        __syncthreads();
+        if (*flag != ks - 1) return;
+#pragma unroll
+        for (int t = 0; t < NT; ++t)
+            for (int e = tid; e < 32 * 32; e += 64 * KW) {
+                float val = 0.f;
+                for (unsigned s = 0; s < ks; ++s) val += slabs[((long)s * NT + t) * 1024 + e];
+                emit(t, e, val);
+            }
+        if (tid == 0) ks_reset(p.kws.ticket + tile);
     }
 }
 
@@ -178,19 +230,81 @@
     return false;
 }
 
-int launch_cl_conv_kw(int amode, int omode, const IgemmArgs &a, hipStream_t st)
-{
+struct KwPlan { int nt, kw, tiles, row_tiles, col_groups; };
+static KwPlan kw_plan(int M, int NP)
+{
+    KwPlan pl;
+    const int nt_total = NP / 32;
+    pl.row_tiles = cdiv(M, 32);
+    pl.nt = 1;
+    for (int c = 4; c > 1; --c)
+        if (nt_total % c == 0 && (long)pl.row_tiles * (nt_total / c) * 4 >= 2048) { pl.nt = c; break; }
+    pl.col_groups = nt_total / pl.nt;
+    pl.tiles = pl.row_tiles * pl.col_groups;
+    pl.kw = (pl.nt > 1 || pl.tiles * 4 >= 1024) ? 4 : 8;
+    return pl;
+}
+
+static std::atomic<int> g_conv_kw_ks{-1};
+static int conv_kw_forced_ks()
+{
+    int v = g_conv_kw_ks.load(std::memory_order_acquire);
+    if (v < 0) {
+        const char *e = getenv("DLKA_CONV_KW_KS");
+        int want = e ? atoi(e) : 0;
+        if (want < 0) want = 0;
+        if (g_conv_kw_ks.compare_exchange_strong(v, want, std::memory_order_acq_rel)) v = want;
+    }
+    return v;
+}
+static std::atomic<int> g_conv_kw_last_ks{0};
+
+static int kw_normalise_ks(int ks, int units)
+{
+    if (ks > units) ks = units;
+    if (ks > 32) ks = 32;
+    if (ks <= 1) return 1;
+    return cdiv(units, cdiv(units, ks));
+}
+
+int cl_conv_kw_pick_ks(int M, int NP, int units, int want)
+{
+    const KwPlan pl = kw_plan(M, NP);
+    if (pl.nt != 1) return 1;
+    if (want <= 0) want = conv_kw_forced_ks();
+    if (want > 0) return kw_normalise_ks(want, units);
+    if (pl.kw != 8) return 1;
+    if (pl.tiles > 64) return 1;
+    int ks = (256 + pl.tiles / 2) / pl.tiles;
+    if (ks > units / (3 * pl.kw)) ks = units / (3 * pl.kw);
+    if (ks > 8) ks = 8;
+    return kw_normalise_ks(ks, units);
+}
+
+int launch_cl_conv_kw(int amode, int omode, const IgemmArgs &a_, hipStream_t st)
+{
+    IgemmArgs a = a_;
     if (!cl_conv_kw_applies(amode, omode, a.split_bf16, a.K, a.epi, a.NP, a.act_bf16 != 0, a.D > 1)) return DLKA_ERR_UNSUPPORTED;
     if ((long)a.K * (a.CinP / 32) * (a.split_bf16 == 3 ? 48 : 32) * a.NP * 4 >= (1l << 31)) return DLKA_ERR_UNSUPPORTED;
-    const int nt_total = a.NP / 32, row_tiles = cdiv(a.M, 32);
-    int nt = 1;
-    for (int c = 4; c > 1; --c)
-        if (nt_total % c == 0 && (long)row_tiles * (nt_total / c) * 4 >= 2048) { nt = c; break; }
-    const int tiles = row_tiles * (nt_total / nt);
-    const int kw = (nt > 1 || tiles * 4 >= 1024) ? 4 : 8;
-    dim3 grid(row_tiles, 1, nt_total / nt), block(64 * kw);
+    const KwPlan pl = kw_plan(a.M, a.NP);
+    const int nt = pl.nt, kw = pl.kw, units = a.K * (a.CinP / 32);
+    int ks = 1;
+    if (a.kws.slab && a.kws.ticket && pl.tiles <= a.kws.ticket_words && nt == 1) {
+        ks = cl_conv_kw_pick_ks(a.M, a.NP, units, a.kws.ks);
+        const size_t fit = a.kws.slab_bytes / ((size_t)pl.tiles * 4096);
+        if ((size_t)ks > fit) ks = kw_normalise_ks((int)fit, units);
+    }
+    g_conv_kw_last_ks.store(ks, std::memory_order_relaxed);
+    dim3 grid(pl.row_tiles, ks, pl.col_groups), block(64 * kw);
     auto go = [&](auto am, auto om, auto sp, auto t) {
         dispatch_int<4, 1, 2, 3>(nt, [&](auto n) { dispatch_bool(kw == 8, [&](auto w8) {
+            if constexpr (DLKA_V(n) == 1) {
+                if (ks > 1) {
+                    auto k = cl_conv_kw_kernel<DLKA_V(am), DLKA_V(om), DLKA_V(sp), DLKA_V(w8) ? 8 : 4, 1, DLKA_T(t), true>;
+                    DLKA_LAUNCH(k, grid, block, 0, st, a);
+                    return;
+                }
+            }
             if constexpr (!DLKA_V(w8) || DLKA_V(n) == 1) {
                 auto k = cl_conv_kw_kernel<DLKA_V(am), DLKA_V(om), DLKA_V(sp), DLKA_V(w8) ? 8 : 4, DLKA_V(n), DLKA_T(t)>;
                 DLKA_LAUNCH(k, grid, block, 0, st, a);
@@ -216,6 +330,14 @@
 
 }
 
+extern "C" int dlka_conv_kw_force_ks(int ks)
+{
+    const int old = dlka::conv_kw_forced_ks();
+    dlka::g_conv_kw_ks.store(ks > 0 ? ks : 0, std::memory_order_release);
+    return old;
+}
+extern "C" int dlka_conv_kw_last_ks(void) { return dlka::g_conv_kw_last_ks.load(std::memory_order_relaxed); }
+extern "C" int dlka_conv_kw_pick_ks(int M, int NP, int units) { return dlka::cl_conv_kw_pick_ks(M, NP, units, 0); }
 extern "C" long dlka_conv_kw_launch_count(void) { return dlka::g_conv_kw_launches.load(std::memory_order_relaxed); }
 extern "C" int dlka_conv_kw_applies(int amode, int omode, int split_bf16, int K, int epi, int NP, int act_bf16, int volume)
 {
diff --git a/deformablelka_amd/csrc/cl_host.h b/deformablelka_amd/csrc/cl_host.h
--- a/deformablelka_amd/csrc/cl_host.h
+++ b/deformablelka_amd/csrc/cl_host.h
@@ -94,10 +94,13 @@
 int dense_forward_splits(const SameConv &s, int epi);
 int dense_backward_data_splits(const SameConv &s, int epi, int gout_planar = -1);
 int dense_forward(const SameConv &s, const float *x, const float *w, const float *bias, float *out, int out_planar, float *wp,
-                  int epi, const float *aux, float *out2, hipStream_t st, bool zeroed = false, const ZeroBatch *ride = nullptr, float *out2_f32 = nullptr);
+                  int epi, const float *aux, float *out2, hipStream_t st, bool zeroed = false, const ZeroBatch *ride = nullptr, float *out2_f32 = nullptr,
+                  const KwSplitWs *kws = nullptr);
+int dense_forward_kw_ks(const SameConv &s, int epi);
+int dense_backward_data_kw_ks(const SameConv &s, int epi, int gout_planar);
 int dense_backward_data(const SameConv &s, const float *gout, int gout_planar, const float *w, float *gx, float *wp, int epi,
                         const float *aux, hipStream_t st, const float *aux2 = nullptr, float *out2 = nullptr, bool zeroed = false, bool g_packed = false,
-                        bool aux_f32 = false, float *acc32 = nullptr, const ZeroBatch *ride = nullptr);
+                        bool aux_f32 = false, float *acc32 = nullptr, const ZeroBatch *ride = nullptr, const KwSplitWs *kws = nullptr);
 size_t dense_wp_floats(const SameConv &s);
 size_t dense_wgrad_pad_bytes(const SameConv &s);
 int dense_backward_weight(const SameConv &s, const float *x, const float *gout, int gout_planar, float *gw, float *gb, float *part, hipStream_t st,
diff --git a/deformablelka_amd/csrc/cl_host_ops.hip b/deformablelka_amd/csrc/cl_host_ops.hip
--- a/deformablelka_amd/csrc/cl_host_ops.hip
+++ b/deformablelka_amd/csrc/cl_host_ops.hip
@@ -74,8 +74,21 @@
     return sp;
 }
 
+int dense_forward_kw_ks(const SameConv &s, int epi)
+{
+    const int units = s.K * (s.Cin / 32), NP = round_up(s.Cout, 32);
+    if (cl_igemm_pick_splits(s.M, units, epi, s.K) <= 1 || dense_forward_splits(s, epi) != 1) return 1;
+    return cl_conv_kw_pick_ks(s.M, NP, units);
+}
+int dense_backward_data_kw_ks(const SameConv &s, int epi, int gout_planar)
+{
+    const int units = s.K * (round_up(s.Cout, 32) / 32);
+    if (cl_igemm_pick_splits(s.M, units, epi, s.K) <= 1 || dense_backward_data_splits(s, epi, gout_planar) != 1) return 1;
+    return cl_conv_kw_pick_ks(s.M, s.Cin, units);
+}
+
 int dense_forward(const SameConv &s, const float *x, const float *w, const float *bias, float *out, int out_planar, float *wp,
-                  int epi, const float *aux, float *out2, hipStream_t st, bool zeroed, const ZeroBatch *ride, float *out2_f32)
+                  int epi, const float *aux, float *out2, hipStream_t st, bool zeroed, const ZeroBatch *ride, float *out2_f32, const KwSplitWs *kws)
 {
     const int NP = round_up(s.Cout, 32);
     const int split = use_split(s, true);
@@ -86,6 +99,7 @@
     a.in = x; a.wp = wp; a.bias = bias; a.out = out; a.out2 = out2; a.aux = aux; a.epi = epi; a.out_zeroed = zeroed ? 1 : 0;
     a.Cin = s.Cin; a.CinReal = s.Cin; a.CinP = s.Cin; a.Cout = s.Cout; a.NP = NP;
     if (ride) a.zero = *ride;
+    if (kws) a.kws = *kws;
     int splits = dense_forward_splits(s, epi);
     if (out_planar && cl_conv_brick3_supported(a)) splits = 1;
     if (out2_f32) {
@@ -97,7 +111,7 @@
 
 int dense_backward_data(const SameConv &s, const float *gout, int gout_planar, const float *w, float *gx, float *wp, int epi,
                         const float *aux, hipStream_t st, const float *aux2, float *out2, bool zeroed, bool g_packed,
-                        bool aux_f32, float *acc32, const ZeroBatch *ride)
+                        bool aux_f32, float *acc32, const ZeroBatch *ride, const KwSplitWs *kws)
 {
     const int KP = round_up(s.Cout, 32), NP = s.Cin;
     if (!(nt_ok(NP) || NP == 192 || NP == 384) || s.Cin % 32) return DLKA_ERR_UNSUPPORTED;
@@ -116,6 +130,7 @@
     }
     a.aux_f32 = aux_f32 ? 1 : 0;
     if (ride) a.zero = *ride;
+    if (kws) a.kws = *kws;
     int splits = dense_backward_data_splits(s, epi, gout_planar);
     const int bsplit = gout_planar ? cl_conv_brick_split(a) : 0;
     bool brick_only = false;
@@ -410,6 +425,46 @@
     fork_env_load();
 }
 
+int dlka_conv3d_kw_split_run(int dir, const void *x, const void *weight, const void *bias, const void *aux, void *out, void *workspace, size_t workspace_bytes,
+                             void *split_ws, size_t split_ws_bytes, const dlka_conv_geom *c, int dtype, int ks, void *stream)
+{
+    if (!x || !weight || !out || !workspace) return DLKA_ERR_NULL;
+    if ((dtype != DLKA_F32 && dtype != DLKA_BF16) || (dir != 0 && dir != 1) || ks < 0) return DLKA_ERR_UNSUPPORTED;
+    SameConv s;
+    DLKA_TRY(make_same_conv(c, s));
+    s.act_bf16 = dtype == DLKA_BF16 ? 1 : 0;
+    if (s.group != 1 || s.Cin % 32 || s.K <= 1 || s.D <= 1) return DLKA_ERR_UNSUPPORTED;
+    hipStream_t st = (hipStream_t)stream;
+    Carver cv(workspace, workspace_bytes);
+    float *wp = (float *)cv.take(dense_wp_floats(s) * 4);
+    if (!cv.ok()) return DLKA_ERR_WORKSPACE;
+    IgemmArgs a;
+    fill_igemm(a, s);
+    const int split = use_split(s, dir == 0);
+    a.split_bf16 = split;
+    a.in = (const float *)x; a.wp = wp; a.out = (float *)out;
+    if (dir == 0) {
+        const int NP = round_up(s.Cout, 32);
+        DLKA_TRY(launch_cl_prep_weight((const float *)weight, wp, s.Cout, s.Cin, s.K, s.Cin, NP, split_mode_flag(split), st));
+        a.bias = (const float *)bias; a.epi = 0;
+        a.Cin = s.Cin; a.CinReal = s.Cin; a.CinP = s.Cin; a.Cout = s.Cout; a.NP = NP;
+    } else {
+        const int KP = round_up(s.Cout, 32), NP = s.Cin;
+        DLKA_TRY(launch_cl_prep_weight((const float *)weight, wp, s.Cout, s.Cin, s.K, KP, NP, 1 | split_mode_flag(split), st));
+        a.pd = s.dd * (s.kd - 1) - s.pd; a.ph = s.dh * (s.kh - 1) - s.ph; a.pw = s.dw * (s.kw - 1) - s.pw;
+        a.aux = (const float *)aux; a.epi = aux ? 3 : 0; a.aux_f32 = 1;
+        a.Cin = s.Cout; a.CinReal = s.Cout; a.CinP = KP; a.Cout = s.Cin; a.NP = NP;
+    }
+    const size_t tick = (size_t)KW_SPLIT_TICKETS * 4;
+    if (split_ws && split_ws_bytes > tick) {
+        a.kws.ticket = (unsigned *)split_ws; a.kws.ticket_words = KW_SPLIT_TICKETS;
+        a.kws.slab = (float *)split_ws + KW_SPLIT_TICKETS; a.kws.slab_bytes = split_ws_bytes - tick;
+        a.kws.ks = ks;
+        DLKA_TRY(launch_zero((float *)split_ws, tick, st));
+    } else if (ks > 1) return DLKA_ERR_WORKSPACE;
+    return launch_cl_conv_kw(dir == 0 ? 0 : 2, dir == 0 ? 1 : 0, a, st);
+}
+
 int dlka_lka3d_force_wgrad_gather(int on)
 {
     const int old = wgrad_gather() ? 1 : 0;
diff --git a/deformablelka_amd/csrc/dlka_kernels.h b/deformablelka_amd/csrc/dlka_kernels.h
--- a/deformablelka_amd/csrc/dlka_kernels.h
+++ b/deformablelka_amd/csrc/dlka_kernels.h
@@ -61,6 +61,7 @@
 int launch_cl_conv_wave(int amode, int omode, const IgemmArgs &a, int splits, hipStream_t st);
 bool cl_conv_kw_applies(int amode, int omode, int split_bf16, int K, int epi, int NP, bool act_bf16, bool volume);
 int launch_cl_conv_kw(int amode, int omode, const IgemmArgs &a, hipStream_t st);
+int cl_conv_kw_pick_ks(int M, int NP, int units, int want = 0);
 bool cl_conv_brick_supported(const IgemmArgs &a);
 int cl_conv_brick_split(const IgemmArgs &a);
 bool cl_conv_brick3_supported(const IgemmArgs &a);
diff --git a/deformablelka_amd/ops.py b/deformablelka_amd/ops.py
--- a/deformablelka_amd/ops.py
+++ b/deformablelka_amd/ops.py
@@ -497,6 +497,34 @@
                                     L.stream_ptr(x))
     L.check(rc, "conv3d_forward_cl")
     return out
+
+
+def conv3d_kw_split_run(direction, x, weight, bias=None, aux=None, ks=0, dtype=None, split_ws=None, out=None):
+    L.require_device(x, weight, bias, aux)
+    x, weight = x.contiguous(), weight.contiguous()
+    Cout, C = int(weight.shape[0]), int(weight.shape[1])
+    if direction == 0:
+        B, D, H, W, _ = x.shape
+        dtype = x.dtype
+        out = torch.empty((B, Cout, D, H, W), dtype=torch.float32, device=x.device) if out is None else out
+        cols = (Cout + 31) // 32
+    else:
+        B, _, D, H, W = x.shape
+        dtype = dtype or torch.float32
+        out = torch.empty((B, D, H, W, C), dtype=dtype, device=x.device) if out is None else out
+        cols = C // 32
+    g = _geom_cl((B, D, H, W, C), Cout, (3, 3, 3), (1, 1, 1), (1, 1, 1), 1)
+    lib = L.get_lib()
+    dt = 1 if dtype == torch.bfloat16 else 0
+    wsb = lib.dlka_conv3d_cl_workspace(byref(g), 0, 0)
+    ws = L.scratch(wsb, x)
+    if split_ws is None:
+        tiles = ((B * D * H * W + 31) // 32) * cols
+        split_ws = torch.empty(4096 + max(ks, 8) * tiles * 4096, dtype=torch.uint8, device=x.device)
+    rc = lib.dlka_conv3d_kw_split_run(int(direction), L.ptr(x), L.ptr(weight), L.ptr(bias), L.ptr(aux), L.ptr(out), L.ptr(ws), wsb, L.ptr(split_ws),
+                                      split_ws.numel(), byref(g), dt, int(ks), L.stream_ptr(x))
+    L.check(rc, "conv3d_kw_split_run")
+    return out, int(lib.dlka_conv_kw_last_ks())
 
 
 def conv3d_backward_cl(x, weight, grad_out, padding=0, dilation=1, groups=1, grad_out_planar=False, need=(True, True, True)):
diff --git a/include/dlka.h b/include/dlka.h
--- a/include/dlka.h
+++ b/include/dlka.h
@@ -269,6 +269,11 @@
 long dlka_dwpair_launch_count(void);
 long dlka_pw_chain_launch_count(void);
 long dlka_conv_kw_launch_count(void);
+int dlka_conv_kw_force_ks(int ks);
+int dlka_conv_kw_last_ks(void);
+int dlka_conv_kw_pick_ks(int M, int NP, int units);
+int dlka_conv3d_kw_split_run(int dir, const void *x, const void *weight, const void *bias, const void *aux, void *out, void *workspace, size_t workspace_bytes,
+                             void *split_ws, size_t split_ws_bytes, const dlka_conv_geom *c, int dtype, int ks, void *stream);
 int dlka_conv_kw_applies(int amode, int omode, int split_bf16, int K, int epi, int NP, int act_bf16, int volume);
 long dlka_dwconv_2p_launch_count(void);
 size_t dlka_lka3d_tokens_workspace_bytes_v(int B, int C, int D, int H, int W, int dtype, int variant);
```
